# cristianpjensen/thesis-pai-reconstruction

Measured on AMD Instinct MI355X. Metric: train images/sec (256x256, bs=64) Pix2Pix step, higher is better.
Workload: dtype bf16; 1 GPU; Pix2Pix generator+PatchGAN GAN step, 256x256x1 pairs, 64 images/GPU (BASELINE configs[1]); global_batch=64, per_gpu_batch=64, loss_type=gan, parallelism=dp1, grad_bucket_dtype=f32

## Files before the change

### include/pai_hip.h

```cpp
#ifndef PAI_HIP_H
#define PAI_HIP_H

#include <stdint.h>

#ifdef __cplusplus
extern "C" {
#endif

#define PAI_F32 0
#define PAI_BF16 1
#define PAI_U8 2

#define PAI_ACT_NONE 0
#define PAI_ACT_LRELU 1
#define PAI_ACT_RELU 2
#define PAI_ACT_TANH 3
#define PAI_ACT_SILU 4

const char* pai_last_error(void);
int pai_version(void);
int pai_build_flags(void);
int pai_device_info(int* cu_count, int* lds_bytes, char* arch_name, int arch_name_len);

#define PAI_TUNABLE_UNSET (-2147483647 - 1)
int pai_set_tunable(const char* name, int value);

typedef struct pai_conv_desc {
    int32_t dtype;
    int32_t transposed;
    int32_t N, H, W;
    int32_t C1, C2;
    int32_t Cout;
    int32_t kernel;
    int32_t stride;
    int32_t pad;
    int32_t relu1, relu2;
    int32_t epilogue_act;
    int32_t groups;
    int32_t pack_flags;
    int32_t hints;
} pai_conv_desc;
#define PAI_HINT_SOLO 1

int pai_conv_out_hw(const pai_conv_desc* d, int* OH, int* OW);
int pai_conv_fwd_stats_rows(const pai_conv_desc* d);
int pai_conv_fwd_stats_rows_max(const pai_conv_desc* d);
int pai_bn_stats_buffer_rows(int rows);

int pai_conv_kernel_id(const pai_conv_desc* d, int op);
int pai_conv_kernel_name(const pai_conv_desc* d, int op, char* name, int name_len);

int pai_create(int device_id, void** handle_out);
int pai_bind(void* handle);
int pai_destroy(void* handle);
int pai_handle_set_workspace(void* handle, void* zeroed_device_memory, int64_t bytes);
int pai_handle_set_scratch(void* handle, void* device_memory, int64_t bytes);
int pai_handle_set_wgrad_workspace(void* handle, void* device_memory, int64_t bytes);

int pai_set_workspace(void* zeroed_device_memory, int64_t bytes);
int64_t pai_conv_workspace_bytes(const pai_conv_desc* d, int op);
int pai_set_scratch(void* device_memory, int64_t bytes);
int64_t pai_conv_scratch_bytes(const pai_conv_desc* d, int op);
int pai_set_wgrad_workspace(void* device_memory, int64_t bytes);
int64_t pai_conv_wgrad_workspace_bytes(const pai_conv_desc* d);

int pai_conv_fwd(const pai_conv_desc* d, const void* x1, const void* x2, const void* w_fwd,
                 const float* bias, void* y_raw, void* y_act, float* y_f32, float* stats,
                 void* stream);

int pai_conv_dgrad(const pai_conv_desc* d, const void* dy, const void* w_dgrad, void* dx1,
                   void* dx2, int only_c2, void* stream);

int pai_conv_dgrad_f32add_ok(const pai_conv_desc* d);
int pai_conv_dgrad_f32add(const pai_conv_desc* d, const void* dy, const void* w_dgrad, const float* addend,
                          float* dx2_f32, void* stream);

int pai_conv_dgrad_act(const pai_conv_desc* d, const void* dy, const void* w_dgrad, void* dx1,
                       void* dx2, const void* a1, int act1, void* stream);

typedef struct pai_bwd_epilogue {
    const void* z;
    const void* add;
    const float* scale;
    const float* shift;
    const float* mean;
    const float* rstd;
    float* partials;
    int32_t act1, act2;
} pai_bwd_epilogue;
int pai_conv_dgrad_bn_rows_max(const pai_conv_desc* d);
int pai_conv_dgrad_bn(const pai_conv_desc* d, const void* dy, const void* w_dgrad, void* dx1,
                      void* dx2, const pai_bwd_epilogue* e, int* partial_rows, void* stream);

typedef struct pai_bn_train {
    const float* gamma;
    const float* beta;
    float eps, momentum;
    int32_t n_updates;
    float* running_mean;
    float* running_var;
    int64_t* num_batches_tracked;
    float *mean, *rstd, *scale, *shift;
} pai_bn_train;
int pai_conv_fwd_bn(const pai_conv_desc* d, const void* x1, const void* x2, const void* w_fwd, const float* bias,
                    void* z, void* a, int act, const pai_bn_train* bn, float* stats, void* stream);
int pai_conv_dgrad_bn_apply(const pai_conv_desc* d, const void* dy, const void* w_dgrad, void* du_scratch, void* dx2,
                            const pai_bwd_epilogue* e, const float* gamma, float* sums, float* dgamma, float* dbeta,
                            void* dz, void* stream);
int pai_conv_bn_fused(const pai_conv_desc* d, int op);

int pai_conv_wgrad(const pai_conv_desc* d, const void* x1, const void* x2, const void* dy,
                   float* dw, float* dbias, void* stream);
int pai_conv_wgrad_overwrite(const pai_conv_desc* d, const void* x1, const void* x2, const void* dy,
                             float* dw, float* dbias, void* stream);
int pai_conv_wgrad_overwrite_w(const pai_conv_desc* d, const void* x1, const void* x2, const void* dy,
                               float* dw, float* dbias, void* stream);

int pai_conv_prologue_ok(const pai_conv_desc* d);
int pai_conv_fwd_pro(const pai_conv_desc* d, const void* x1, const void* w_fwd, const float* bias, void* y_raw,
                     float* stats, const float* pre_scale, const float* pre_shift, int pre_act, void* stream);
int pai_conv_wgrad_pro(const pai_conv_desc* d, const void* x1, const void* dy, float* dw, float* dbias, int overwrite,
                       const float* pre_scale, const float* pre_shift, int pre_act, void* stream);

int pai_pack_weights(int dtype, const float* w_master, int Cout, int taps, int Cin,
                     void* w_fwd_or_null, void* w_dgrad_or_null, void* stream);
int pai_pack_weights_multi(int n, const float* const* w_master, const int32_t* cout, const int32_t* taps,
                           const int32_t* cin, void* const* w_fwd, void* const* w_dgrad, void* stream);

int pai_bn_finalize(const float* stats, int rows, int C, int64_t count, const float* gamma,
                    const float* beta, float eps, float momentum, int n_updates,
                    float* running_mean, float* running_var, int64_t* num_batches_tracked,
                    float* mean, float* rstd, float* scale, float* shift, void* stream);
int pai_bn_eval_coeffs(int C, const float* gamma, const float* beta, const float* running_mean,
                       const float* running_var, float eps, float* scale, float* shift,
                       void* stream);
int pai_bn_apply(int dtype, const void* z, int64_t M, int C, const float* scale,
                 const float* shift, int act, void* out, void* stream);
int pai_bn2_add_act(int dtype, const void* za, const float* scale_a, const float* shift_a, const void* zb,
                    const float* scale_b, const float* shift_b, int64_t M, int C, int act_a, int act, void* out,
                    void* stream);
int pai_bn_bwd_partial_rows(int64_t M);
int pai_bn_bwd_reduce(int dtype, const void* g1, int act1, const void* g2, int act2, const void* a,
                      const void* z, int64_t M, int C, const float* mean, const float* rstd,
                      void* du, float* partials, float* sums, float* dgamma, float* dbeta,
                      void* stream);
int pai_bn_bwd_reduce_affine(int dtype, const void* g1, int act1, const void* g2, int act2, const void* z,
                             int64_t M, int C, const float* scale, const float* shift, const float* mean,
                             const float* rstd, void* du, float* partials, float* sums, float* dgamma,
                             float* dbeta, void* stream);
int pai_bn_bwd_finalize(const float* partials, int rows, int C, float* sums, float* dgamma,
                        float* dbeta, void* stream);
int pai_bn_bwd_apply(int dtype, const void* du, const void* z, int64_t M, int C,
                     const float* mean, const float* rstd, const float* gamma,
                     const float* sums, void* dz, void* stream);
int pai_bn_bwd_apply_affine(int dtype, const void* g1, int act1, const void* z, int64_t M, int C, const float* scale,
                            const float* shift, const float* mean, const float* rstd, const float* gamma,
                            const float* sums, void* dz, void* stream);
int pai_act_bwd(int dtype, const void* g1, int act1, const void* g2, int act2, const void* a,
                int64_t numel, void* du, void* stream);

int pai_dropout2d(int dtype, const void* x, const float* mask, int N, int64_t HW, int C, void* out,
                  void* stream);

int pai_maxpool2(int dtype, const void* x, int N, int H, int W, int C, void* out, unsigned char* idx, void* stream);
int pai_maxpool2_bwd(int dtype, const void* dout, const unsigned char* idx, int N, int H, int W, int C, void* dx,
                     void* stream);
int pai_upsample2(int dtype, const void* x, int N, int H, int W, int C, void* out, void* stream);
int pai_upsample2_bwd(int dtype, const void* dout, int N, int H, int W, int C, void* dx, void* stream);
int pai_add_act(int dtype, const void* a, const void* b, int64_t numel, int act, void* out, void* stream);
int pai_bn2_bwd_reduce(int dtype, const void* d, int act_a, const void* za, const void* zb, int64_t M, int C,
                       const float* scale_a, const float* shift_a, const float* mean_a, const float* rstd_a,
                       const float* mean_b, const float* rstd_b, float* part_a, float* part_b, float* sums_a, float* sums_b,
                       void* stream);
int pai_bn2_bwd_apply(int dtype, const void* d, int act_a, const void* za, const void* zb, int64_t M, int C,
                      const float* scale_a, const float* shift_a, const float* mean_a, const float* rstd_a,
                      const float* gamma_a, const float* sums_a, const float* mean_b, const float* rstd_b,
                      const float* gamma_b, const float* sums_b, void* dza, void* dzb, void* stream);
int pai_instnorm_fwd(int dtype, const void* x, int N, int HW, int C, float eps, int act, void* y, float* mean, float* rstd,
                     void* stream);
int pai_instnorm_bwd(int dtype, const void* g, const void* x, int N, int HW, int C, int act, const float* mean,
                     const float* rstd, void* dx, void* stream);

int pai_layernorm_partial_rows(int64_t M);
int pai_layernorm_fwd(int dtype, const void* x, const void* res, int64_t M, int D, const float* gamma,
                      const float* beta, float eps, const float* post, int P, void* sum_out, void* y,
                      float* mean, float* rstd, void* stream);
int pai_layernorm_bwd(int dtype, const void* dy, const void* xs, int64_t M, int D, const float* gamma,
                      const float* mean, const float* rstd, void* dx, float* dgamma_dbeta, float* partials,
                      void* stream);
int pai_gelu(int dtype, const void* z, int64_t numel, void* out, void* stream);
int pai_gelu_bwd(int dtype, const void* dy, const void* z, int64_t numel, void* dz, void* stream);
int pai_mha_fwd(int dtype, const void* qkv, int S, int B, int heads, int hd, const float* mask, void* out,
                float* probs, void* stream);
int pai_mha_bwd(int dtype, const void* dout, const void* qkv, const float* probs, int S, int B, int heads,
                int hd, const float* mask, void* dqkv, float* ds_workspace, void* stream);
int pai_mha_kernel_name(int dtype, int S, int hd, int op, char* name, int name_len);
int pai_subsample2(int dtype, const void* x, int N, int H, int W, int C, void* out, void* stream);
int pai_subsample2_bwd(int dtype, const void* dout, int N, int H, int W, int C, void* dx, void* stream);
int pai_bn_stats_rows(int64_t M);
int pai_bn_stats(int dtype, const void* z, int64_t M, int C, float* stats, void* stream);
int pai_colsum(int dtype, const void* x, int64_t rows, int C, float* out, void* stream);

int pai_gate_partial_rows(int64_t M);
int pai_gate_hidden(int dtype, const void* ig, const void* sg, int64_t M, int K, const float* scale_i,
                    const float* shift_i, const float* scale_s, const float* shift_s, const float* w_a,
                    const float* b_a, void* h, float* logit, float* partials, void* stream);
int pai_gate_apply(int dtype, const void* x, const float* logit, int64_t M, int C, const float* scale_a,
                   const float* shift_a, void* out, float* att, void* stream);
int pai_gate_apply_bwd(int dtype, const void* dout, const void* x, const float* att, const float* logit,
                       int64_t M, int C, const float* mean_a, const float* rstd_a, void* dx_skip, float* dl,
                       float* partials, int relu_out, void* stream);
int pai_gate_hidden_bwd(int dtype, const float* dl, const float* logit, const void* h, const void* ig,
                        const void* sg, int64_t M, int K, const float* mean_a, const float* rstd_a,
                        const float* gamma_a, const float* sums_a, const float* w_a, const float* mean_i,
                        const float* rstd_i, const float* mean_s, const float* rstd_s, void* dsum,
                        float* partials_i, float* partials_s, float* dw_a, float* db_a, void* stream);

int pai_bce_logits(const float* logits, int64_t numel, float target, float loss_scale,
                   double* loss, float grad_scale, float* grad, void* stream);
int pai_l1(const float* pred, const float* target, int64_t numel, float loss_scale, double* loss,
           float grad_scale, float* grad, void* stream);
int pai_mse(const float* pred, const float* target, int64_t numel, float loss_scale, double* loss,
            float grad_scale, float* grad, void* stream);
int pai_head_loss_ok(const pai_conv_desc* d, int has_bias);
int pai_head_loss(const pai_conv_desc* d, const void* a3, const void* w_fwd, const void* w_dgrad, int n_first,
                  float target_first, float target_rest, float loss_scale, double* loss, float grad_scale,
                  float* logits, void* dl, float* dl_f32, void* du, const void* act_src, int act, void* stream);
int pai_scalar_take(double* acc, float* out, void* stream);
int pai_metrics_take(double* sums, int64_t n_images, int64_t numel, float* out3, void* stream);
int pai_tanh_bwd(int dtype, const float* pred, const float* g_a, const float* g_b, int64_t numel,
                 void* dh, void* stream);
// ... 112 lines not shown
```

### thesis-pai-reconstruction_amd/attention.py

```python
from __future__ import annotations

import torch
import torch.nn as nn

from . import ops
from .engine import GradArena, UnetEngine, _BNState, _Packs, _bn_forward, to_fwd_pack_
from .ops import ACT_LRELU, ACT_NONE, ACT_RELU, ACT_TANH


class _Gate:

    def __init__(self, block: nn.Module, gen):
        self.conv_i, self.bn_i = block.input_gate[0], block.input_gate[1]
        self.conv_s, self.bn_s = block.signal_gate[0], block.signal_gate[1]
        self.conv_a, self.bn_a = block.attention[0], block.attention[1]
        self.C = self.conv_i.weight.shape[1]
        self.K = self.conv_i.weight.shape[0]
        self.pack_i = _Packs(self.conv_i, need_dgrad=True, gen=gen)
        self.pack_s = _Packs(self.conv_s, need_dgrad=True, gen=gen)

    def ordered_params(self):
        return [(self.conv_a.weight, None), (self.conv_a.bias, None), (self.bn_a.weight, None), (self.bn_a.bias, None),
                (self.bn_i.weight, None), (self.bn_i.bias, None), (self.bn_s.weight, None), (self.bn_s.bias, None),
                (self.conv_i.weight, None), (self.conv_i.bias, None), (self.conv_s.weight, None),
                (self.conv_s.bias, None)]


class AttentionUnetEngine(UnetEngine):
    overwrites_weight_grads = True

    def __init__(self, unet: nn.Module):
        super().__init__(unet)
        self.gates = [_Gate(b, self.weights_generation) for b in unet.attention_blocks]
        assert len(self.gates) == self.L - 1

    def all_packs(self):
        return self.enc_packs + self.dec_packs + [pk for g in self.gates for pk in (g.pack_i, g.pack_s)]

    def _gate(self, j):
        return self.gates[j - 1]

    def ordered_params(self):
        out = []
        L = self.L
        for j in range(L - 1, -1, -1):
            if self.dec_bn[j] is not None:
                out += [(self.dec_bn[j].weight, None), (self.dec_bn[j].bias, None)]
            out += [(self.dec_conv[j].weight, self.dec_conv[j]), (self.dec_conv[j].bias, None)]
            if j >= 1:
                out += self._gate(j).ordered_params()
        for i in range(L - 1, -1, -1):
            if self.enc_bn[i] is not None:
                out += [(self.enc_bn[i].weight, None), (self.enc_bn[i].bias, None)]
            out += [(self.enc_conv[i].weight, self.enc_conv[i]), (self.enc_conv[i].bias, None)]
        return out

    def _plan(self, N, H, W, dtype, device):
        key = (N, H, W, dtype, str(device))
        if key in self._plans:
            return self._plans[key]
        P = super()._plan(N, H, W, dtype, device)
        L = self.L
        eh, ew = P["eh"], P["ew"]
        P["dec_desc"] = []
        for j in range(L):
            hin, win = eh[L - 1 - j], ew[L - 1 - j]
            if j == 0:
                c1, c2, r1, r2 = self.enc_c[L - 1], 0, 1, 0
            else:
                c1, c2, r1, r2 = self.dec_c[j - 1], self.enc_c[L - 1 - j], 1, 1
            act = ACT_NONE
            if j == L - 1:
                r1, r2, act = 0, 0, ACT_TANH
            P["dec_desc"].append(ops.make_desc(dtype, 1, N, hin, win, c1, c2, self.dec_c[j], 2, r1, r2, act))
        P["gate_desc"] = [None]
        rows = P["stats"].numel()
        mx = P["bwd_partials"].numel()
        for j in range(1, L):
            g = self._gate(j)
            lvl = L - 1 - j
            d = ops.make_desc(dtype, 0, N, eh[lvl], ew[lvl], g.C, 0, g.K, 1, 0, 0, ACT_NONE, kernel=1)
            P["gate_desc"].append(d)
            M = N * eh[lvl] * ew[lvl]
            rows = max(rows, ops.bn_stats_buffer_rows(ops.conv_fwd_stats_rows_max(d)) * 2 * g.K,
                       ops.bn_stats_buffer_rows(ops.gate_partial_rows(M)) * 2)
            mx = max(mx, ops.gate_partial_rows(M) * 2 * g.K, ops.conv_dgrad_bn_rows_max(d) * 2 * g.C)
        P["stats"] = torch.empty(rows, dtype=torch.float32, device=device)
        P["bwd_partials"] = torch.empty(mx, dtype=torch.float32, device=device)
        P["bwd_partials2"] = torch.empty(mx, dtype=torch.float32, device=device)
        ops.ensure_workspace(max(ops.conv_workspace_bytes(d, op) for d in P["dec_desc"] + P["gate_desc"][1:]
                                 for op in (0, 1)), device)
        ops.ensure_scratch(ops.scratch_bytes_for(P["enc_desc"] + P["dec_desc"]), device)
        ops.ensure_wgrad_workspace(P["enc_desc"] + P["dec_desc"], device)
        return P

    def _new_slot(self, P):
        S = super()._new_slot(P)
        L, N, dt, dev = self.L, P["N"], P["dtype"], P["device"]
        eh, ew = P["eh"], P["ew"]
        S["b"] = [None] + [torch.empty_like(S["z"][i]) if i < L - 1 else None for i in range(1, L)]
        S["gate"] = [None]
        for j in range(1, L):
            g = self._gate(j)
            lvl = L - 1 - j
            M = N * eh[lvl] * ew[lvl]
            f32 = dict(dtype=torch.float32, device=dev)
            S["gate"].append({
                "M": M,
                "ig": torch.empty(M * g.K, dtype=dt, device=dev), "sg": torch.empty(M * g.K, dtype=dt, device=dev),
                "h": torch.empty(M * g.K, dtype=dt, device=dev), "s": torch.empty(M * g.C, dtype=dt, device=dev),
                "logit": torch.empty(M, **f32), "att": torch.empty(M, **f32),
                "bn_i": _BNState(g.K, dev), "bn_s": _BNState(g.K, dev), "bn_a": _BNState(1, dev),
            })
        return S

    def _grad_bufs(self, S):
        if S["grads"] is not None:
            return S["grads"]
        G = super()._grad_bufs(S)
        P = S["P"]
        L, dt, dev = self.L, P["dtype"], P["device"]
        G["gs"] = [None] + [torch.empty_like(S["gate"][j]["s"]) for j in range(1, L)]
        G["gx"] = [None] + [torch.empty_like(S["gate"][j]["s"]) for j in range(1, L)]
        G["dxs"] = [None] + [torch.empty_like(S["gate"][j]["s"]) for j in range(1, L)]
        G["dl"] = [None] + [torch.empty_like(S["gate"][j]["logit"]) for j in range(1, L)]
        G["dsum"] = [None] + [torch.empty_like(S["gate"][j]["h"]) for j in range(1, L)]
        G["dig"] = [None] + [torch.empty_like(S["gate"][j]["h"]) for j in range(1, L)]
        G["dsg"] = [None] + [torch.empty_like(S["gate"][j]["h"]) for j in range(1, L)]
        G["gr_raw"] = [torch.empty_like(t) if t is not None else None for t in G["gr"]]
        return G

    def _skip(self, S, lvl):
        return S["z"][0] if lvl == 0 else S["b"][lvl]

    def _gate_forward(self, S, j, x, signal, training, bn_updates, dtype):
        g, gs, P = self._gate(j), S["gate"][j], S["P"]
        d, M = P["gate_desc"][j], gs["M"]
        for conv, bn, pack, src, dst, st in ((g.conv_i, g.bn_i, g.pack_i, x, gs["ig"], gs["bn_i"]),
                                             (g.conv_s, g.bn_s, g.pack_s, signal, gs["sg"], gs["bn_s"])):
            wf, _ = pack.get(dtype)
            if training:
                rows = ops.conv_fwd_stats_rows(d)
                ops.conv_fwd(d, src, None, wf, conv.bias, y_raw=dst, stats=P["stats"])
                _bn_forward(bn, st, P["stats"], rows, M, True, bn_updates)
            else:
                ops.conv_fwd(d, src, None, wf, conv.bias, y_raw=dst)
                _bn_forward(bn, st, None, 0, M, False, 0)
        bi, bs, ba = gs["bn_i"], gs["bn_s"], gs["bn_a"]
        ops.gate_hidden(dtype, gs["ig"], gs["sg"], M, g.K, bi.scale, bi.shift, bs.scale, bs.shift, g.conv_a.weight,
                        g.conv_a.bias, gs["h"], gs["logit"], P["stats"])
        _bn_forward(g.bn_a, ba, P["stats"] if training else None, ops.gate_partial_rows(M) if training else 0, M,
                    training, bn_updates)
        ops.gate_apply(dtype, x, gs["logit"], M, g.C, ba.scale, ba.shift, gs["s"], gs["att"])
        return gs["s"]

    def forward(self, x: torch.Tensor, training: bool, bn_updates: int, dtype: torch.dtype):
        if not x.is_cuda:
            raise ops.PaiError("AttentionUnet (HIP) needs a HIP device tensor; there is no CPU path")
        N, Ci, H, W = x.shape
# ... 9 lines not shown
        xs = xs.contiguous() if Ci == 1 else xs.permute(0, 2, 3, 1).contiguous()
        if dtype == torch.float32:
            S["x"] = xs.reshape(-1)
        else:
            ops.cast(xs, S["x"])
        eh, ew = P["eh"], P["ew"]
        wf, _ = self.enc_packs[0].get(dtype)
        ops.conv_fwd(P["enc_desc"][0], S["x"], None, wf, self.enc_conv[0].bias, y_raw=S["z"][0], y_act=S["a"][0])
        for i in range(1, L):
            wf, _ = self.enc_packs[i].get(dtype)
            bn, d = self.enc_bn[i], P["enc_desc"][i]
            if bn is None:
                if i < L - 1:
                    raise ops.PaiError("only the last encoder may be norm-free")
                ops.conv_fwd(d, S["a"][i - 1], None, wf, self.enc_conv[i].bias, y_raw=S["z"][i])
                continue
            M = N * eh[i] * ew[i]
            if training:
                rows = ops.conv_fwd_stats_rows(d)
                ops.conv_fwd(d, S["a"][i - 1], None, wf, self.enc_conv[i].bias, y_raw=S["z"][i], stats=P["stats"])
                _bn_forward(bn, S["ebn"][i], P["stats"], rows, M, True, bn_updates)
            else:
                ops.conv_fwd(d, S["a"][i - 1], None, wf, self.enc_conv[i].bias, y_raw=S["z"][i])
                _bn_forward(bn, S["ebn"][i], None, 0, M, False, 0)
            st = S["ebn"][i]
            ops.bn_apply(dtype, S["z"][i], M, self.enc_c[i], st.scale, st.shift, ACT_LRELU, S["a"][i])
            ops.bn_apply(dtype, S["z"][i], M, self.enc_c[i], st.scale, st.shift, ACT_NONE, S["b"][i])
        for j in range(L):
            wf, _ = self.dec_packs[j].get(dtype)
            d = P["dec_desc"][j]
            if j == 0:
                x1, x2 = S["z"][L - 1], None
            else:
                x1 = S["r"][j - 1]
                x2 = self._gate_forward(S, j, self._skip(S, L - 1 - j), x1, training, bn_updates, dtype)
            if j < L - 1:
                bn = self.dec_bn[j]
                M = N * S["dh"][j] * S["dw"][j]
                if training:
                    rows = ops.conv_fwd_stats_rows(d)
                    ops.conv_fwd(d, x1, x2, wf, self.dec_conv[j].bias, y_raw=S["w"][j], stats=P["stats"])
                    _bn_forward(bn, S["dbn"][j], P["stats"], rows, M, True, bn_updates)
                else:
                    ops.conv_fwd(d, x1, x2, wf, self.dec_conv[j].bias, y_raw=S["w"][j])
                    _bn_forward(bn, S["dbn"][j], None, 0, M, False, 0)
                ops.bn_apply(dtype, S["w"][j], M, self.dec_c[j], S["dbn"][j].scale, S["dbn"][j].shift, ACT_NONE,
                             S["r"][j])
                if training and self.dec_drop[j] > 0:
                    self._dropout(S, j, M, self.dec_c[j], dtype)
            else:
                S["pred"] = torch.empty_like(S["pred"])
                ops.conv_fwd(d, x1, x2, wf, self.dec_conv[j].bias, y_f32=S["pred"])
        pred = S["pred"]
        if self.out_ch != 1:
            pred = pred.view(N, H, W, self.out_ch).permute(0, 3, 1, 2)
        return pred, S

    def backward(self, S, gpred: torch.Tensor, fresh: bool = False):
        P = S["P"]
        L, N, dtype = self.L, P["N"], P["dtype"]
        eh, ew = P["eh"], P["ew"]
        G = self._grad_bufs(S)
        A = self.arena()
        hook = self.grad_ready_hook
        if self.out_ch != 1:
            gpred = gpred.permute(0, 2, 3, 1)
        gpred = gpred.contiguous()
        if gpred.dtype != torch.float32:
            gpred = gpred.float()
        side = self._side
        part, part2 = P["bwd_partials"], P["bwd_partials2"]

        def done(p):
            if hook is not None:
                hook(A, A.end_of(p))

        def wgrad(d, x1, x2, dz, conv, with_bias, last=None):
            cin, cout = conv.weight.shape[1], conv.weight.shape[0]
            dense = fresh and conv.weight.shape[2] == 4 and min(cin, cout) > 2
            with torch.cuda.stream(side.fork(d)):
                (ops.conv_wgrad_overwrite_w if dense else ops.conv_wgrad)(
                    d, x1, x2, dz, A.seg(conv.weight), A.seg(conv.bias) if with_bias else None)
                done(last if last is not None else conv.bias)

        def gate_backward(j, relu_out):
            g, gs = self._gate(j), S["gate"][j]
            d, M = P["gate_desc"][j], gs["M"]
            lvl = L - 1 - j
            x, signal = self._skip(S, lvl), S["r"][j - 1]
            ba, bi, bs = gs["bn_a"], gs["bn_i"], gs["bn_s"]
            ops.gate_apply_bwd(dtype, G["gs"][j], x, gs["att"], gs["logit"], M, g.C, ba.mean, ba.rstd, G["dxs"][j],
                               G["dl"][j], part, relu_out)
            ops.bn_bwd_finalize(part, ops.gate_partial_rows(M), 1, ba.sums, A.seg(g.bn_a.weight), A.seg(g.bn_a.bias))
            ops.gate_hidden_bwd(dtype, G["dl"][j], gs["logit"], gs["h"], gs["ig"], gs["sg"], M, g.K, ba.mean, ba.rstd,
                                g.bn_a.weight, ba.sums, g.conv_a.weight, bi.mean, bi.rstd, bs.mean, bs.rstd,
                                G["dsum"][j], part, part2, A.seg(g.conv_a.weight), A.seg(g.conv_a.bias))
            rows = ops.gate_partial_rows(M)
            ops.bn_bwd_finalize(part, rows, g.K, bi.sums, A.seg(g.bn_i.weight), A.seg(g.bn_i.bias))
            ops.bn_bwd_finalize(part2, rows, g.K, bs.sums, A.seg(g.bn_s.weight), A.seg(g.bn_s.bias))
            ops.bn_bwd_apply(dtype, G["dsum"][j], gs["ig"], M, g.K, bi.mean, bi.rstd, g.bn_i.weight, bi.sums, G["dig"][j])
            ops.bn_bwd_apply(dtype, G["dsum"][j], gs["sg"], M, g.K, bs.mean, bs.rstd, g.bn_s.weight, bs.sums, G["dsg"][j])
            wgrad(d, x, None, G["dig"][j], g.conv_i, False)
            wgrad(d, signal, None, G["dsg"][j], g.conv_s, False)
            _, wd_i = g.pack_i.get(dtype)
            _, wd_s = g.pack_s.get(dtype)
            ops.conv_dgrad_bn(d, G["dig"][j], wd_i, G["gx"][j], None, x, ACT_NONE, G["dxs"][j], ACT_NONE)
            pst = S["dbn"][j - 1]
            if (j - 1) in S["drop"]:
                ops.conv_dgrad_bn(d, G["dsg"][j], wd_s, G["gr"][j - 1], None, S["r"][j - 1], ACT_NONE,
                                  G["gr_raw"][j - 1], ACT_RELU if relu_out else ACT_NONE)
                ops.dropout2d(dtype, G["gr"][j - 1], S["drop"][j - 1], N, S["dh"][j - 1] * S["dw"][j - 1],
                              self.dec_c[j - 1], G["gr"][j - 1])
                return None
            return ops.conv_dgrad_bn(d, G["dsg"][j], wd_s, G["gr"][j - 1], None, S["w"][j - 1], ACT_NONE,
                                     G["gr_raw"][j - 1], ACT_RELU if relu_out else ACT_NONE, pst.scale, pst.shift,
                                     pst.mean, pst.rstd, part)

        j = L - 1
        dh = G["dz_head"]
        ops.tanh_bwd(dtype, S["pred"], gpred, None, dh)
        d = P["dec_desc"][j]
        wgrad(d, S["r"][j - 1], S["gate"][j]["s"], dh, self.dec_conv[j], True)
        side.mark_scratch()
        _, wd = self.dec_packs[j].get(dtype)
        ops.conv_dgrad(d, dh, wd, G["gr_raw"][j - 1], G["gs"][j])
        fused_rows = gate_backward(j, relu_out=False)
        for j in range(L - 2, -1, -1):
            bn, st, conv = self.dec_bn[j], S["dbn"][j], self.dec_conv[j]
            M = N * S["dh"][j] * S["dw"][j]
            C = self.dec_c[j]
            dz = G["dz_dec"][j]
            du = G["gr"][j]
            if fused_rows is None:
                du = G["du"][:M * C]
                ops.bn_bwd_reduce(dtype, G["gr"][j], ACT_NONE, None, ACT_NONE, None, S["w"][j], M, C, st.mean, st.rstd,
                                  du, part, st.sums, A.seg(bn.weight), A.seg(bn.bias))
            else:
                ops.bn_bwd_finalize(part, fused_rows, C, st.sums, A.seg(bn.weight), A.seg(bn.bias))
            ops.bn_bwd_apply(dtype, du, S["w"][j], M, C, st.mean, st.rstd, bn.weight, st.sums, dz)
            d = P["dec_desc"][j]
            _, wd = self.dec_packs[j].get(dtype)
            if j == 0:
                wgrad(d, S["z"][L - 1], None, dz, conv, False)
                fused_rows = ops.conv_dgrad_bn(d, dz, wd, G["dz_enc"][L - 1], None, S["z"][L - 1], ACT_RELU)
            else:
                wgrad(d, S["r"][j - 1], S["gate"][j]["s"], dz, conv, False)
                ops.conv_dgrad(d, dz, wd, G["gr_raw"][j - 1], G["gs"][j])
                fused_rows = gate_backward(j, relu_out=True)
        i = L - 1
        dz = G["dz_enc"][i]
        wgrad(P["enc_desc"][i], S["a"][i - 1], None, dz, self.enc_conv[i], True)
        _, wd = self.enc_packs[i].get(dtype)

        def enc_dgrad(i, dz, wd):
            d = P["enc_desc"][i]
            gx = G["gx"][L - 1 - (i - 1)]
            if i - 1 == 0:
                return ops.conv_dgrad_bn(d, dz, wd, G["dz_enc"][0], None, S["z"][0], ACT_LRELU, gx, ACT_NONE)
            pst = S["ebn"][i - 1]
            return ops.conv_dgrad_bn(d, dz, wd, G["ga"][i - 1], None, S["z"][i - 1], ACT_LRELU, gx, ACT_NONE,
                                     pst.scale, pst.shift, pst.mean, pst.rstd, part)

        fused_rows = enc_dgrad(i, dz, wd)
        for i in range(L - 2, 0, -1):
            bn, st, conv = self.enc_bn[i], S["ebn"][i], self.enc_conv[i]
            M = N * eh[i] * ew[i]
            C = self.enc_c[i]
            du, dz = G["ga"][i], G["dz_enc"][i]
            ops.bn_bwd_finalize(part, fused_rows, C, st.sums, A.seg(bn.weight), A.seg(bn.bias))
            ops.bn_bwd_apply(dtype, du, S["z"][i], M, C, st.mean, st.rstd, bn.weight, st.sums, dz)
            wgrad(P["enc_desc"][i], S["a"][i - 1], None, dz, conv, False)
            _, wd = self.enc_packs[i].get(dtype)
            fused_rows = enc_dgrad(i, dz, wd)
        conv0 = self.enc_conv[0]
        with torch.cuda.stream(side.fork_tail()):
            c0_in, c0_out = conv0.weight.shape[1], conv0.weight.shape[0]
            (ops.conv_wgrad_overwrite_w if (fresh and min(c0_in, c0_out) > 2) else ops.conv_wgrad)(
                P["enc_desc"][0], S["x"], None, G["dz_enc"][0], A.seg(conv0.weight), A.seg(conv0.bias))
        side.join()
        done(conv0.bias)
```

### thesis-pai-reconstruction_amd/csrc/api.hip

```cpp
#include <stdarg.h>

#include "common.h"

static thread_local char g_err[512] = "";

void pai_set_error(const char* fmt, ...) {
    va_list ap;
    va_start(ap, fmt);
    vsnprintf(g_err, sizeof(g_err), fmt, ap);
    va_end(ap);
}

extern "C" const char* pai_last_error(void) { return g_err; }
extern "C" int pai_version(void) { return 141; }

extern "C" int pai_build_flags(void) { return 0; }

extern "C" int pai_device_info(int* cu_count, int* lds_bytes, char* arch_name, int arch_name_len) {
    int dev = 0;
    hipError_t e = hipGetDevice(&dev);
    PAI_CHECK(e == hipSuccess, "hipGetDevice: %s", hipGetErrorString(e));
    hipDeviceProp_t p;
    e = hipGetDeviceProperties(&p, dev);
    PAI_CHECK(e == hipSuccess, "hipGetDeviceProperties: %s", hipGetErrorString(e));
// ... 470 lines not shown

extern "C" int64_t pai_conv_workspace_bytes(const pai_conv_desc* d, int op) {
    GG g;
    if (op == 1 ? gg_build_dgrad(d, &g) : gg_build_fwd(d, &g)) return -1;
    return op == 2 ? 0 : pick_fwd(d->dtype, g, query_args(g, op)).workspace_bytes;
}

extern "C" int64_t pai_conv_scratch_bytes(const pai_conv_desc* d, int op) {
    GG g;
    if (op == 1 ? gg_build_dgrad(d, &g) : gg_build_fwd(d, &g)) return -1;
    return op == 2 ? pick_wgrad(d->dtype, g, false, false).scratch_bytes : pick_fwd(d->dtype, g, query_args(g, op)).scratch_bytes;
}

extern "C" int pai_conv_fwd_stats_rows(const pai_conv_desc* d) {
    GG g;
    if (gg_build_fwd(d, &g)) return -1;
    FwdArgs a = query_args(g, 0);
    a.stats = (float*)1;
    return pick_fwd(d->dtype, g, a).rows;
}

extern "C" int pai_conv_kernel_id(const pai_conv_desc* d, int op) {
    GG g;
    if (op == 1 ? gg_build_dgrad(d, &g) : gg_build_fwd(d, &g)) return -1;
    return op == 2 ? pick_wgrad(d->dtype, g, false, false).id : pick_fwd(d->dtype, g, query_args(g, op)).id;
}

extern "C" int pai_conv_kernel_name(const pai_conv_desc* d, int op, char* name, int name_len) {
    GG g;
    if ((op == 1 ? gg_build_dgrad(d, &g) : gg_build_fwd(d, &g)) || !name || name_len <= 0) return -1;
    const char* n = op == 2 ? pick_wgrad(d->dtype, g, false, false).name : pick_fwd(d->dtype, g, query_args(g, op)).name;
    strncpy(name, n, name_len - 1);
    name[name_len - 1] = 0;
    return 0;
}

extern "C" int pai_conv_fwd_stats_rows_max(const pai_conv_desc* d) {
    GG g;
    if (gg_build_fwd(d, &g)) return -1;
    return cdiv(g.M, 16) * g.nphase;
}

extern "C" int pai_conv_fwd(const pai_conv_desc* d, const void* x1, const void* x2,
                            const void* w_fwd, const float* bias, void* y_raw, void* y_act,
                            float* y_f32, float* stats, void* stream) {
    GG g;
    if (gg_build_fwd(d, &g)) return 1;
    PAI_CHECK(x1 && w_fwd, "pai_conv_fwd: null x1 / w");
    PAI_CHECK(d->C2 == 0 || x2, "pai_conv_fwd: C2 > 0 but x2 is null");
    PAI_CHECK(y_raw || y_act || y_f32, "pai_conv_fwd: no output requested");
    FwdArgs a;
    memset(&a, 0, sizeof(a));
    a.x1 = x1; a.x2 = x2; a.w = w_fwd; a.bias = bias;
    a.y1 = y_raw; a.y2 = nullptr; a.yact = y_act; a.yf32 = y_f32; a.stats = stats;
    a.eact = d->epilogue_act;
    return run_fwd(d->dtype, g, a, (hipStream_t)stream);
}

static int conv_wgrad_impl(const pai_conv_desc* d, const void* x1, const void* x2, const void* dy, float* dw,
                           float* dbias, int overwrite, void* stream, const float* pscale = nullptr,
                           const float* pshift = nullptr, int pact = 0);

extern "C" int pai_conv_prologue_ok(const pai_conv_desc* d) {
    GG g;
    if (gg_build_fwd(d, &g)) return 0;
    FwdArgs a = query_args(g, 0);
    a.pscale = a.pshift = (const float*)1;
    a.pact = PAI_ACT_RELU;
    return pick_fwd(d->dtype, g, a).k != FK_NONE && pick_wgrad(d->dtype, g, false, true).k != WK_NONE;
}

extern "C" int pai_conv_fwd_pro(const pai_conv_desc* d, const void* x1, const void* w_fwd, const float* bias, void* y_raw,
                                float* stats, const float* pre_scale, const float* pre_shift, int pre_act, void* stream) {
    GG g;
    if (gg_build_fwd(d, &g)) return 1;
    PAI_CHECK(x1 && w_fwd && y_raw && pre_scale && pre_shift, "pai_conv_fwd_pro: null pointer");
    PAI_CHECK(pre_act == PAI_ACT_NONE || pre_act == PAI_ACT_RELU, "pai_conv_fwd_pro: pre_act=%d (none or ReLU)", pre_act);
    PAI_CHECK(d->C2 == 0, "pai_conv_fwd_pro: one source tensor only");
    FwdArgs a;
    memset(&a, 0, sizeof(a));
    a.x1 = x1; a.w = w_fwd; a.bias = bias;
    a.y1 = y_raw;
    a.stats = stats;
    a.pscale = pre_scale; a.pshift = pre_shift; a.pact = pre_act;
    return run_fwd(d->dtype, g, a, (hipStream_t)stream);
}

extern "C" int pai_conv_wgrad_pro(const pai_conv_desc* d, const void* x1, const void* dy, float* dw, float* dbias,
                                  int overwrite, const float* pre_scale, const float* pre_shift, int pre_act, void* stream) {
    PAI_CHECK(pre_scale && pre_shift, "pai_conv_wgrad_pro: null prologue");
    PAI_CHECK(pre_act == PAI_ACT_NONE || pre_act == PAI_ACT_RELU, "pai_conv_wgrad_pro: pre_act=%d (none or ReLU)", pre_act);
    PAI_CHECK(d->C2 == 0, "pai_conv_wgrad_pro: one source tensor only");
    return conv_wgrad_impl(d, x1, nullptr, dy, dw, dbias, overwrite ? 1 : 0, stream, pre_scale, pre_shift, pre_act);
}

extern "C" int pai_conv_dgrad(const pai_conv_desc* d, const void* dy, const void* w_dgrad,
                              void* dx1, void* dx2, int only_c2, void* stream) {
    GG g;
    if (gg_build_dgrad(d, &g)) return 1;
    PAI_CHECK(dy && w_dgrad, "pai_conv_dgrad: null dy / w");
    PAI_CHECK(only_c2 ? (dx2 && d->C2 > 0) : (dx1 != nullptr), "pai_conv_dgrad: missing output");
    PAI_CHECK(d->C2 == 0 || dx2, "pai_conv_dgrad: C2 > 0 but dx2 is null");
    FwdArgs a;
    memset(&a, 0, sizeof(a));
    a.x1 = dy; a.w = w_dgrad;
    a.y1 = dx1; a.y2 = dx2;
    a.skip_d1 = only_c2;
    return run_fwd(d->dtype, g, a, (hipStream_t)stream);
}

extern "C" int pai_conv_dgrad_f32add_ok(const pai_conv_desc* d) {
    GG g;
    if (!d || gg_build_dgrad(d, &g)) return 0;
    return pai_tunable("head_fused", 1) && thin_up_f32add_ok(d->dtype, g) ? 1 : 0;
}

extern "C" int pai_conv_dgrad_f32add(const pai_conv_desc* d, const void* dy, const void* w_dgrad, const float* addend,
                                     float* dx2_f32, void* stream) {
    GG g;
    if (gg_build_dgrad(d, &g)) return 1;
    PAI_CHECK(dy && w_dgrad && addend && dx2_f32, "pai_conv_dgrad_f32add: null pointer");
    PAI_CHECK(thin_up_f32add_ok(d->dtype, g), "pai_conv_dgrad_f32add: not a bf16 (1 | 1)-channel k4 s2 layer on thin_up_k (ask pai_conv_dgrad_f32add_ok)");
    FwdArgs a;
    memset(&a, 0, sizeof(a));
    a.x1 = dy; a.w = w_dgrad;
    a.yf32 = dx2_f32; a.badd = addend;
    a.skip_d1 = 1;
    return launch_thin_dgrad(g, a, (hipStream_t)stream);
}

extern "C" int pai_conv_dgrad_act(const pai_conv_desc* d, const void* dy, const void* w_dgrad,
                                  void* dx1, void* dx2, const void* a1, int act1, void* stream) {
    GG g;
    if (gg_build_dgrad(d, &g)) return 1;
    PAI_CHECK(dy && w_dgrad && dx1 && a1, "pai_conv_dgrad_act: null pointer");
    PAI_CHECK(d->C2 == 0 || dx2, "pai_conv_dgrad_act: C2 > 0 but dx2 is null");
    PAI_CHECK(act1 == PAI_ACT_LRELU || act1 == PAI_ACT_RELU || act1 == PAI_ACT_NONE, "pai_conv_dgrad_act: act1=%d", act1);
    FwdArgs a;
    memset(&a, 0, sizeof(a));
    a.x1 = dy; a.w = w_dgrad;
    a.y1 = dx1; a.y2 = dx2;
    hipStream_t s = (hipStream_t)stream;
    FwdPick p = pick_fwd(d->dtype, g, a);
    const bool fused = p.fused || p.k == FK_HEAD_DGRAD;
    if (fused) {
        a.bz = a1; a.bact1 = act1;
        p = pick_fwd(d->dtype, g, a);
    }
    int rc = run_fwd(p, d->dtype, g, a, s);
    if (rc || fused || act1 == PAI_ACT_NONE) return rc;
    return pai_act_bwd(d->dtype, dx1, act1, nullptr, PAI_ACT_NONE, a1, (int64_t)g.N * g.OH * g.OW * g.D1, dx1, stream);
}

extern "C" int pai_conv_dgrad_bn_rows_max(const pai_conv_desc* d) {
    GG g;
    if (gg_build_dgrad(d, &g)) return -1;
    int fused = cdiv(g.M, 16) * g.nphase;
    if (pw_rows(g) > fused) fused = pw_rows(g);
    if (pwx_rows(g) > fused) fused = pwx_rows(g);
    const int twopass = pai_bn_bwd_partial_rows((int64_t)g.N * g.OH * g.OW);
    return fused > twopass ? fused : twopass;
}

int bn_bwd_reduce_affine(int dtype, void* g1_du, int act1, const void* g2, int act2, const void* z, int64_t M, int C,
                         const float* scale, const float* shift, const float* mean, const float* rstd,
                         float* partials, hipStream_t s);

extern "C" int pai_conv_dgrad_bn(const pai_conv_desc* d, const void* dy, const void* w_dgrad, void* dx1,
                                 void* dx2, const pai_bwd_epilogue* e, int* partial_rows, void* stream) {
    GG g;
    if (gg_build_dgrad(d, &g)) return 1;
    PAI_CHECK(dy && w_dgrad && dx1 && e && e->z, "pai_conv_dgrad_bn: null pointer");
    PAI_CHECK(d->C2 == 0 || dx2, "pai_conv_dgrad_bn: C2 > 0 but dx2 is null");
    PAI_CHECK((e->scale == nullptr) == (e->shift == nullptr), "pai_conv_dgrad_bn: scale and shift go together");
    PAI_CHECK(!e->partials || (e->mean && e->rstd && partial_rows), "pai_conv_dgrad_bn: partials need mean, rstd and partial_rows");
    for (int act : {e->act1, e->act2})
        PAI_CHECK(act == PAI_ACT_LRELU || act == PAI_ACT_RELU || act == PAI_ACT_NONE, "pai_conv_dgrad_bn: act=%d", act);
    FwdArgs a;
    memset(&a, 0, sizeof(a));
    a.x1 = dy; a.w = w_dgrad;
    a.y1 = dx1; a.y2 = dx2;
    hipStream_t s = (hipStream_t)stream;
    const int64_t M = (int64_t)g.N * g.OH * g.OW;
    const FwdPick plain = pick_fwd(d->dtype, g, a);
    if (plain.fused) {
        a.bz = e->z; a.badd = e->add;
        a.bscale = e->scale; a.bshift = e->shift; a.bmean = e->mean; a.brstd = e->rstd;
        a.bact1 = e->act1; a.bact2 = e->act2;
        a.bpart = e->partials;
        const FwdPick p = pick_fwd(d->dtype, g, a);
        PAI_CHECK(p.fused, "pai_conv_dgrad_bn: no kernel with the fused store takes this epilogue");
        if (partial_rows) *partial_rows = e->partials ? p.rows : 0;
        return run_fwd(p, d->dtype, g, a, s);
    }
    if (e->partials) {
        if (const int rows = thin_fwd_bwd_rows(d->dtype, g, a, e->act1, e->add, e->scale)) {
            a.bz = e->z; a.bmean = e->mean; a.brstd = e->rstd; a.bpart = e->partials; a.bact1 = e->act1;
            *partial_rows = rows;
            return run_fwd(d->dtype, g, a, s);
        }
    }
    int rc = run_fwd(plain, d->dtype, g, a, s);
    if (rc) return rc;
    if (e->partials) {
        *partial_rows = pai_bn_bwd_partial_rows(M);
        return bn_bwd_reduce_affine(d->dtype, dx1, e->act1, e->add, e->act2, e->z, M, g.D1, e->scale, e->shift,
                                    e->mean, e->rstd, e->partials, s);
    }
    if (partial_rows) *partial_rows = 0;
    PAI_CHECK(e->scale == nullptr, "pai_conv_dgrad_bn: affine pre-activation without partial sums is only built for the matrix-core kernels");
    return pai_act_bwd(d->dtype, dx1, e->act1, e->add, e->act2, e->z, M * g.D1, dx1, stream);
}

extern "C" int pai_conv_fwd_bn(const pai_conv_desc* d, const void* x1, const void* x2, const void* w_fwd, const float* bias,
                               void* z, void* a_out, int act, const pai_bn_train* bn, float* stats, void* stream) {
    GG g;
    if (gg_build_fwd(d, &g)) return 1;
    PAI_CHECK(x1 && w_fwd && z && a_out && bn && stats, "pai_conv_fwd_bn: null pointer");
    PAI_CHECK(d->C2 == 0 || x2, "pai_conv_fwd_bn: C2 > 0 but x2 is null");
    PAI_CHECK(bn->mean && bn->rstd && bn->scale && bn->shift, "pai_conv_fwd_bn: mean / rstd / scale / shift outputs are required");
    PAI_CHECK(act == PAI_ACT_NONE || act == PAI_ACT_RELU || act == PAI_ACT_LRELU, "pai_conv_fwd_bn: act=%d", act);
    FwdArgs a;
    memset(&a, 0, sizeof(a));
    a.x1 = x1; a.x2 = x2; a.w = w_fwd; a.bias = bias;
    a.y1 = z; a.stats = stats;
    a.eact = PAI_ACT_NONE;
    hipStream_t s = (hipStream_t)stream;
    const int64_t count = (int64_t)g.N * g.OH * g.OW;
    const FwdPick p = pick_fwd(d->dtype, g, a);
    if (int rc = run_fwd(p, d->dtype, g, a, s)) return rc;
    const int rows = p.rows;
    if (bn_fuse_small_ok(rows, count, g.Cout))
        return launch_bn_fin_apply(d->dtype, stats, rows, g.Cout, count, bn->gamma, bn->beta, bn->eps, bn->momentum,
                                   bn->n_updates, bn->running_mean, bn->running_var, bn->num_batches_tracked, bn->mean,
                                   bn->rstd, bn->scale, bn->shift, z, act, a_out, s);
    if (int rc = pai_bn_finalize(stats, rows, g.Cout, count, bn->gamma, bn->beta, bn->eps, bn->momentum, bn->n_updates,
                                 bn->running_mean, bn->running_var, bn->num_batches_tracked, bn->mean, bn->rstd, bn->scale,
                                 bn->shift, stream)) return rc;
    return pai_bn_apply(d->dtype, z, count, g.Cout, bn->scale, bn->shift, act, a_out, stream);
}

extern "C" int pai_conv_bn_fused(const pai_conv_desc* d, int op) {
    GG g;
    if (op == 1 ? gg_build_dgrad(d, &g) : gg_build_fwd(d, &g)) return -1;
    return 0;
}

extern "C" int pai_conv_dgrad_bn_apply(const pai_conv_desc* d, const void* dy, const void* w_dgrad, void* du_scratch,
                                       void* dx2, const pai_bwd_epilogue* e, const float* gamma, float* sums,
                                       float* dgamma, float* dbeta, void* dz, void* stream) {
    GG g;
    if (gg_build_dgrad(d, &g)) return 1;
    PAI_CHECK(dy && w_dgrad && du_scratch && e && e->z && e->mean && e->rstd && e->partials && sums && dz,
              "pai_conv_dgrad_bn_apply: null pointer");
    PAI_CHECK(d->C2 == 0 || dx2, "pai_conv_dgrad_bn_apply: C2 > 0 but dx2 is null");
    PAI_CHECK((e->scale == nullptr) == (e->shift == nullptr), "pai_conv_dgrad_bn_apply: scale and shift go together");
    FwdArgs a;
    memset(&a, 0, sizeof(a));
    a.x1 = dy; a.w = w_dgrad;
    a.y1 = du_scratch; a.y2 = dx2;
    hipStream_t s = (hipStream_t)stream;
    int rows = 0;
    if (int rc = pai_conv_dgrad_bn(d, dy, w_dgrad, du_scratch, dx2, e, &rows, stream)) return rc;
    const int64_t Mo = (int64_t)g.N * g.OH * g.OW;
    if (bn_fuse_small_ok(rows, Mo, g.D1))
        return launch_bn_bwd_fin_apply(d->dtype, e->partials, rows, g.D1, sums, dgamma, dbeta, du_scratch, e->z, Mo, e->mean,
                                       e->rstd, gamma, dz, s);
    if (int rc = pai_bn_bwd_finalize(e->partials, rows, g.D1, sums, dgamma, dbeta, stream)) return rc;
    return pai_bn_bwd_apply(d->dtype, du_scratch, e->z, Mo, g.D1, e->mean, e->rstd, gamma, sums, dz, stream);
}


extern "C" int pai_conv_wgrad(const pai_conv_desc* d, const void* x1, const void* x2,
                              const void* dy, float* dw, float* dbias, void* stream) {
    return conv_wgrad_impl(d, x1, x2, dy, dw, dbias, 0, stream);
}

extern "C" int pai_conv_wgrad_overwrite(const pai_conv_desc* d, const void* x1, const void* x2,
                                        const void* dy, float* dw, float* dbias, void* stream) {
    return conv_wgrad_impl(d, x1, x2, dy, dw, dbias, 1, stream);
}

extern "C" int pai_conv_wgrad_overwrite_w(const pai_conv_desc* d, const void* x1, const void* x2,
                                          const void* dy, float* dw, float* dbias, void* stream) {
    return conv_wgrad_impl(d, x1, x2, dy, dw, dbias, 2, stream);
}

static int conv_wgrad_impl(const pai_conv_desc* d, const void* x1, const void* x2, const void* dy, float* dw,
                           float* dbias, int overwrite, void* stream, const float* pscale, const float* pshift, int pact) {
    GG g;
    if (gg_build_fwd(d, &g)) return 1;
    PAI_CHECK(x1 && dy && dw, "pai_conv_wgrad: null pointer");
    PAI_CHECK(d->C2 == 0 || x2, "pai_conv_wgrad: C2 > 0 but x2 is null");
    WgradArgs a;
    a.x1 = x1; a.x2 = x2; a.dy = dy; a.dw = dw; a.dbias = dbias; a.overwrite = 0; a.overwrite_bias = 0; a.slab = nullptr;
    a.pscale = pscale; a.pshift = pshift; a.pact = pact;
    hipStream_t s = (hipStream_t)stream;
    const WgradPick p = pick_wgrad(d->dtype, g, dbias != nullptr, pscale != nullptr);
    PAI_CHECK(p.k != WK_NONE, "pai_conv_wgrad_pro: this layer takes no prologue (ask pai_conv_prologue_ok: the grouped 3 x 3 weight "
                              "gradient needs its workspace, pai_set_wgrad_workspace)");
    if (overwrite && p.overwrites) {
        a.overwrite = 1;
        a.overwrite_bias = p.k != WK_GROUPED3 && overwrite == 1;
    } else if (overwrite) {
        hipError_t e = pai::memset_async(dw, 0, (size_t)g.Cout * g.wtaps * g.Cin * sizeof(float), s);
        PAI_CHECK(e == hipSuccess, "pai_conv_wgrad_overwrite: hipMemsetAsync: %s", hipGetErrorString(e));
// ... 18 lines not shown
```

### thesis-pai-reconstruction_amd/csrc/common.h

```cpp
#pragma once
#include <hip/hip_runtime.h>
#include <stdint.h>
#include <stdio.h>
#include <string.h>

#include "../../include/pai_hip.h"
#include "plan.h"

typedef unsigned short bf16_t;

void pai_set_error(const char* fmt, ...);

#define PAI_CHECK(cond, ...)                 \
    do {                                     \
        if (!(cond)) {                       \
            pai_set_error(__VA_ARGS__);      \
            return 1;                        \
        }                                    \
    } while (0)

#define PAI_LAUNCH_CHECK()                                              \
    do {                                                                \
        hipError_t e_ = hipGetLastError();                              \
        if (e_ != hipSuccess) {                                         \
// ... 41 lines not shown
    static __device__ __forceinline__ void ld(const float* p, float* o) {
        float4 a = *(const float4*)p, b = *(const float4*)(p + 4);
        o[0] = a.x; o[1] = a.y; o[2] = a.z; o[3] = a.w; o[4] = b.x; o[5] = b.y; o[6] = b.z; o[7] = b.w;
    }
    static __device__ __forceinline__ void st(float* p, const float* v) {
        *(float4*)p = make_float4(v[0], v[1], v[2], v[3]);
        *(float4*)(p + 4) = make_float4(v[4], v[5], v[6], v[7]);
    }
};
template <> struct V8<bf16_t> {
    static __device__ __forceinline__ void ld(const bf16_t* p, float* o) {
        uint4 v = *(const uint4*)p;
        unsigned u[4] = {v.x, v.y, v.z, v.w};
#pragma unroll
        for (int i = 0; i < 4; ++i) {
            o[2 * i] = __uint_as_float(u[i] << 16);
            o[2 * i + 1] = __uint_as_float(u[i] & 0xffff0000u);
        }
    }
    static __device__ __forceinline__ void st(bf16_t* p, const float* v) {
        unsigned u[4];
#pragma unroll
        for (int i = 0; i < 4; ++i) u[i] = pk2bf(v[2 * i], v[2 * i + 1]);
        *(uint4*)p = make_uint4(u[0], u[1], u[2], u[3]);
    }
};

__device__ __forceinline__ float act_apply(float v, int act) {
    switch (act) {
        case PAI_ACT_LRELU: return v > 0.f ? v : 0.2f * v;
        case PAI_ACT_RELU: return !(v <= 0.f) ? v : 0.f;
        case PAI_ACT_TANH: return tanhf(v);
        default: return v;
    }
}
__device__ __forceinline__ float act_grad(float a, int act) {
    switch (act) {
        case PAI_ACT_LRELU: return a > 0.f ? 1.f : 0.2f;
        case PAI_ACT_RELU: return a > 0.f ? 1.f : 0.f;
        default: return 1.f;
    }
}

__device__ __forceinline__ float wave_sum(float v) {
#pragma unroll
    for (int o = 32; o > 0; o >>= 1) v += __shfl_xor(v, o, 64);
    return v;
}

static inline int cdiv(int64_t a, int64_t b) { return (int)((a + b - 1) / b); }

struct PerDeviceOnce {
    bool done[32] = {};
    bool first() {
        int dev = 0;
        if (hipGetDevice(&dev) != hipSuccess || dev < 0 || dev >= 32) return true;
        if (done[dev]) return false;
        done[dev] = true;
        return true;
    }
};

struct GG {
    int N, H, W;
    int C1, C2, Cin;
    int OHg, OWg;
    int Cout;
    int S;
    int nphase, ntaps;
    int OH, OW, OS;
    int D1, D2;
    int wtaps;
    int relu1, relu2;
    int M;
    int lw, lh;
    int lsw, lsh, ldw, ldh;
    signed char dy[4][16], dx[4][16], wt[4][16];
    signed char poy[4], pox[4];
    int gslice;
    int solo;
};

struct PatchGeo {
    int groups;
    int TY, TX;
    signed char by[4][4], bx[4][4];
    unsigned toff4[4][4];
    unsigned wt4[4][4];
    unsigned wt_lo[4], wt_hi[4], toff2[4];
};

int gg_build_fwd(const pai_conv_desc* d, GG* g);
int gg_build_dgrad(const pai_conv_desc* d, GG* g);

struct FwdArgs {
    const void *x1, *x2, *w;
    const float* bias;
    void *y1, *y2;
    void* yact;
    float* yf32;
    float* stats;
    int eact;
    int skip_d1;
    const void* bz;
    const void* badd;
    const float *bscale, *bshift, *bmean, *brstd;
    int bact1, bact2;
    float* bpart;
    const float *pscale, *pshift;
    int pact;
};
bool bn_fuse_small_ok(int rows, int64_t M, int C);
int launch_bn_fin_apply(int dtype, const float* stats, int rows, int C, int64_t count, const float* gamma, const float* beta,
                        float eps, float momentum, int n_updates, float* running_mean, float* running_var, int64_t* nbt,
                        float* mean, float* rstd, float* scale, float* shift, const void* z, int act, void* out,
                        hipStream_t s);
int launch_bn_bwd_fin_apply(int dtype, const float* partials, int rows, int C, float* sums, float* dgamma, float* dbeta,
                            const void* du, const void* z, int64_t M, const float* mean, const float* rstd,
                            const float* gamma, void* dz, hipStream_t s);
int ew_stream_bn_apply(int dtype, const void* z, int64_t M, int C, const float* scale, const float* shift, int act, void* out,
                       hipStream_t s);
int ew_stream_bn2_add_act(int dtype, const void* za, const float* sca, const float* sha, const void* zb, const float* scb,
                          const float* shb, int64_t M, int C, int act_a, int act, void* out, hipStream_t s);
int ew_stream_add_act(int dtype, const void* a, const void* b, int64_t numel, int act, void* out, hipStream_t s);
int ew_stream_bn_bwd_reduce(int dtype, const void* g, int act, const void* z, int64_t M, int C, const float* scale,
                            const float* shift, const float* mean, const float* rstd, float* partials, int rows, hipStream_t s);
int ew_stream_bn_bwd_apply(int dtype, const void* g, int act, const void* z, int64_t M, int C, const float* scale,
                           const float* shift, const float* mean, const float* rstd, const float* gamma, const float* sums,
                           void* dz, hipStream_t s);
int ew_stream_bn2_bwd_reduce(int dtype, const void* d, int act_a, const void* za, const void* zb, int64_t M, int C,
                             const float* scale_a, const float* shift_a, const float* mean_a, const float* rstd_a,
                             const float* mean_b, const float* rstd_b, float* part_a, float* part_b, int rows, hipStream_t s);
int ew_stream_bn2_bwd_apply(int dtype, const void* d, int act_a, const void* za, const void* zb, int64_t M, int C,
                            const float* scale_a, const float* shift_a, const float* mean_a, const float* rstd_a,
                            const float* gamma_a, const float* sums_a, const float* mean_b, const float* rstd_b,
                            const float* gamma_b, const float* sums_b, void* dza, void* dzb, hipStream_t s);
int launch_fwd_simt(int dtype, const GG& g, const FwdArgs& a, hipStream_t s);
int launch_fwd_rowdot(int dtype, const GG& g, const FwdArgs& a, hipStream_t s);
int pai_tunable(const char* name, int def);
struct MfmaPlan {
    int variant;
    const char* name;
    int bm, bn, db;
    int ksplit, mtiles, ntiles;
    int rows;
    unsigned grid, block;
    size_t lds;
    int64_t workspace_bytes;
    bool overwrites;
    PatchGeo pg;
};
enum WgradMfmaVariant { WG3_128x64 = 1, WG3_64x128, WG3_128x64_8, WGRAD_PATCH128, WGRAD_PATCH64, WGRAD_TILE128, WGRAD_TILE64 };
MfmaPlan fwd_mfma_plan(const GG& g);
int launch_fwd_mfma(const GG& g, const FwdArgs& a, const MfmaPlan& p, hipStream_t s);
MfmaPlan wgrad_mfma_plan(const GG& g, bool has_dbias, bool has_prologue);
bool wgrad_pro_ok(int dtype, const GG& g);
struct pai_handle_s {
    int device;
    float* workspace;
    int64_t workspace_bytes;
    float* scratch;
    int64_t scratch_bytes;
    float* wslab;
    int64_t wslab_bytes;
};
const pai_handle_s* pai_ctx();
int fwd_simt_mtiles(const GG& g);
bool fwd_mfma_ok(int dtype, const GG& g, const FwdArgs& a);
bool pw_ok(int dtype, const GG& g, const FwdArgs& a);
int pw_rows(const GG& g);
int launch_pw(const GG& g, const FwdArgs& a, hipStream_t s);
bool pwx_ok(int dtype, const GG& g, const FwdArgs& a);
int pwx_rows(const GG& g);
int launch_pwx(const GG& g, const FwdArgs& a, hipStream_t s);
const char* pwx_kernel_name(const GG& g);
bool fwd_rowdot_ok(const GG& g, const FwdArgs& a);
bool small_ok(int dtype, const GG& g, const FwdArgs& a);
int small_rows(const GG& g);
int launch_small(const GG& g, const FwdArgs& a, hipStream_t s);
bool grouped3_ok(int dtype, const GG& g, const FwdArgs& a);
int grouped3_rows(const GG& g);
int launch_grouped3(const GG& g, const FwdArgs& a, hipStream_t s);

bool thin_fwd_ok(int dtype, const GG& g, const FwdArgs& a);
bool thin_dgrad_ok(int dtype, const GG& g, const FwdArgs& a);
bool thin_dgrad_shape_ok(int dtype, const GG& g);
int64_t thin_dgrad_scratch_bytes(const GG& g, const FwdArgs& a);
int launch_thin_fwd(const GG& g, const FwdArgs& a, hipStream_t s);
bool head_dgrad_ok(int dtype, const GG& g, const FwdArgs& a);
int launch_head_dgrad(const GG& g, const FwdArgs& a, hipStream_t s);
int thin_fwd_bwd_rows(int dtype, const GG& g, const FwdArgs& a, int act1, const void* add, const float* scale);
int launch_thin_dgrad(const GG& g, const FwdArgs& a, hipStream_t s);
bool thin_up_f32add_ok(int dtype, const GG& g);

struct WgradArgs {
    const void *x1, *x2, *dy;
    float* dw;
    float* dbias;
    int overwrite;
    int overwrite_bias;
    float* slab;
    const float *pscale, *pshift;
    int pact;
};
float* wgrad_slab_acquire(int64_t bytes);
int launch_wgrad_slab_sum(float* dw, const float* slab, int nsplits, int64_t n, int overwrite, hipStream_t s);
bool grouped3_wgrad_ok(int dtype, const GG& g, const float* dbias);
int64_t grouped3_wgrad_part_bytes(const GG& g);
int launch_grouped3_wgrad(const GG& g, const WgradArgs& a, float* part, hipStream_t s);
int launch_eval_planes(const float* pred, const float* target, int NC, int H, int W, int denorm, double* ssim_plane,
                       double* sse_plane, unsigned char* map_u8, const unsigned char* lut_rgb, unsigned char* hot_u8,
                       hipStream_t stream);
const char* eval_planes_kernel_name();
bool wgrad3_ok(const GG& g);
MfmaPlan wgrad3_plan(const GG& g, bool has_dbias);
int launch_wgrad3(const GG& g, const WgradArgs& a, const MfmaPlan& p, hipStream_t s);
int launch_wgrad_simt(int dtype, const GG& g, const WgradArgs& a, hipStream_t s);
int launch_wgrad_rowdot(int dtype, const GG& g, const WgradArgs& a, hipStream_t s);
int launch_wgrad_mfma(const GG& g, const WgradArgs& a, const MfmaPlan& p, hipStream_t s);
bool wgrad_mfma_ok(int dtype, const GG& g);
bool thin_wgrad_conv_ok(int dtype, const GG& g);
bool thin_wgrad_convt_ok(int dtype, const GG& g);
int launch_thin_wgrad_conv(const GG& g, const WgradArgs& a, hipStream_t s);
int launch_thin_wgrad_convt(const GG& g, const WgradArgs& a, hipStream_t s);
bool thin_wgrad_conv1_ok(int dtype, const GG& g);
int launch_thin_wgrad_conv1(const GG& g, const WgradArgs& a, hipStream_t s);
bool thin_wgrad_conv3_ok(int dtype, const GG& g);
int launch_thin_wgrad_conv3(const GG& g, const WgradArgs& a, hipStream_t s);
bool thin_wgrad_conv3t_ok(int dtype, const GG& g);
int launch_thin_wgrad_conv3t(const GG& g, const WgradArgs& a, hipStream_t s);
int64_t thin_wgrad_scratch_bytes(int64_t M, int T, int WC);
```

### thesis-pai-reconstruction_amd/csrc/gg_mfma.hip

```cpp
#include <type_traits>

#include "gg_tile.h"


bool fwd_mfma_ok(int dtype, const GG& g, const FwdArgs& a) {
    if (dtype != PAI_BF16) return false;
    if (g.C1 % 64 || g.C2 % 64) return false;
    if (g.Cout % 64) return false;
    if (g.D2 > 0 && (g.D1 % 64)) return false;
    if (a.yf32) return false;
    if (a.skip_d1) return false;
    if ((a.y1 || a.y2) && a.yact) return false;
    if (a.yact && a.eact != PAI_ACT_NONE && a.eact != PAI_ACT_LRELU && a.eact != PAI_ACT_RELU) return false;
    return true;
}

struct FwdCfg { int bn, ksplit; };

static FwdCfg fwd_cfg(const GG& g) {
    FwdCfg c;
    c.bn = ((g.Cout % 128) == 0 && (g.D2 == 0 || (g.D1 % 128) == 0)) ? 128 : 64;
    c.ksplit = 1;
    const int ntiles = g.Cout / c.bn;
    const int niter = g.ntaps * g.Cin / MBK;
// ... 287 lines not shown
    float bs1[8], bs2[8];
#pragma unroll
    for (int k = 0; k < 8; ++k) bs1[k] = bs2[k] = 0.f;
    constexpr int NP = BM / ORP, NB = NP < 4 ? NP : 4;
    if (bwd) bwd_load_params(a, dcol + oc * 8, BP);
#pragma unroll
    for (int p0 = 0; p0 < NP; p0 += NB) {
        size_t offs[NB];
        uint4 zq[NB], aq[NB];
#pragma unroll
        for (int p = 0; p < NB; ++p) {
            const int m = m0 + orow0 + (p0 + p) * ORP;
            int n, gy, gx;
            decode_row(g, m < g.M ? m : 0, n, gy, gx);
            const size_t pix = (size_t)(n * g.OH + gy * g.OS + g.poy[ph]) * g.OW + gx * g.OS + g.pox[ph];
            offs[p] = pix * dstride + dcol + oc * 8;
            if (bwd) {
                zq[p] = *(const uint4*)(bzp + offs[p]);
                aq[p] = bap ? *(const uint4*)(bap + offs[p]) : make_uint4(0, 0, 0, 0);
            }
        }
#pragma unroll
        for (int p = 0; p < NB; ++p) {
            const int row = orow0 + (p0 + p) * ORP;
            if (m0 + row < g.M) {
                uint4 o = *(const uint4*)(Cs + row * CROW + oc * 16);
                if (bwd)
                    o = bwd_chunk(o, zq[p], aq[p], bap != nullptr, a.bscale != nullptr, bsum, a.bact1, a.bact2, BP, bs1, bs2);
                *(uint4*)(dst + offs[p]) = o;
            }
        }
    }
    if (bsum)
        bwd_write_partials<BN, CPR, NTHR / 64>(sstat, bs1, bs2, tid,
                                               a.bpart + ((size_t)(ph * mtiles + bm) * 2) * g.D1 + n0, g.D1,
                                               a.bmean + n0, a.brstd + n0);
}

constexpr int FIN_COLS = 128;
__global__ __launch_bounds__(256) void splitk_finish_k(GG g, FwdArgs a, const float* ws, int mtiles, int ksplit) {
    __shared__ float red[2][FIN_ROWS][FIN_COLS + 8];
    const int tid = threadIdx.x;
    const int bm = blockIdx.x, ph = blockIdx.y, cb = blockIdx.z;
    const int row = tid >> 4, cgl = tid & 15;
    const int m = bm * FIN_ROWS + row;
    const int c0 = cb * FIN_COLS + cgl * 8;
    const bool valid = m < g.M && c0 < g.Cout;
    const float eslope = act_slope(a.yact ? a.eact : PAI_ACT_NONE);
    float v[8], bs1[8], bs2[8];
#pragma unroll
    for (int k = 0; k < 8; ++k) v[k] = bs1[k] = bs2[k] = 0.f;
    if (valid) {
        const size_t slab = (size_t)g.nphase * g.M * g.Cout;
        const float* src = ws + ((size_t)ph * g.M + m) * g.Cout + c0;
#pragma unroll 4
        for (int s = 0; s < ksplit; ++s) {
            const float4 v0 = *(const float4*)(src + s * slab), v1 = *(const float4*)(src + s * slab + 4);
            v[0] += v0.x; v[1] += v0.y; v[2] += v0.z; v[3] += v0.w;
            v[4] += v1.x; v[5] += v1.y; v[6] += v1.z; v[7] += v1.w;
        }
        if (a.bias) {
#pragma unroll
            for (int k = 0; k < 8; ++k) v[k] += a.bias[c0 + k];
        }
    }
    if (a.stats) {
#pragma unroll
        for (int k = 0; k < 8; ++k) {
            red[0][row][cgl * 8 + k] = v[k];
            red[1][row][cgl * 8 + k] = v[k] * v[k];
        }
    }
    if (valid) {
        unsigned packed[4];
#pragma unroll
        for (int k = 0; k < 8; ++k) v[k] = act_fwd(v[k], eslope);
#pragma unroll
        for (int k = 0; k < 4; ++k) packed[k] = pk2bf(v[2 * k], v[2 * k + 1]);
        int n, gy, gx;
        decode_row(g, m, n, gy, gx);
        const size_t pix = (size_t)(n * g.OH + gy * g.OS + g.poy[ph]) * g.OW + gx * g.OS + g.pox[ph];
        bf16_t* dst;
        if (a.yact) dst = (bf16_t*)a.yact + pix * g.Cout + c0;
        else if (c0 < g.D1) dst = (bf16_t*)a.y1 + pix * g.D1 + c0;
        else dst = (bf16_t*)a.y2 + pix * g.D2 + (c0 - g.D1);
        uint4 o = make_uint4(packed[0], packed[1], packed[2], packed[3]);
        if (a.bz && !a.yact && c0 < g.D1) {
            BwdParams BP;
            bwd_load_params(a, c0, BP);
            const size_t off = pix * g.D1 + c0;
            const bf16_t* bap = (const bf16_t*)a.badd;
            o = bwd_chunk(o, *(const uint4*)((const bf16_t*)a.bz + off),
                          bap ? *(const uint4*)(bap + off) : make_uint4(0, 0, 0, 0), bap != nullptr,
                          a.bscale != nullptr, a.bpart != nullptr, a.bact1, a.bact2, BP, bs1, bs2);
        }
        *(uint4*)dst = o;
    }
    if (a.stats) {
        __syncthreads();
        const int c = cb * FIN_COLS + tid;
        if (tid < FIN_COLS && c < g.Cout) {
            float t1 = 0.f, t2 = 0.f;
#pragma unroll
            for (int r = 0; r < FIN_ROWS; ++r) { t1 += red[0][r][tid]; t2 += red[1][r][tid]; }
            float* dst = a.stats + ((size_t)(ph * mtiles + bm) * 2) * g.Cout + c;
            dst[0] = t1;
            dst[g.Cout] = t2;
        }
    } else if (a.bpart && a.bz) {
#pragma unroll
        for (int k = 0; k < 8; ++k) {
            red[0][row][cgl * 8 + k] = bs1[k];
            red[1][row][cgl * 8 + k] = bs2[k];
        }
        __syncthreads();
        const int c = cb * FIN_COLS + tid;
        if (tid < FIN_COLS && c < g.D1) {
            float t1 = 0.f, t2 = 0.f;
#pragma unroll
            for (int r = 0; r < FIN_ROWS; ++r) { t1 += red[0][r][tid]; t2 += red[1][r][tid]; }
            float* dst = a.bpart + ((size_t)(ph * mtiles + bm) * 2) * g.D1 + c;
            dst[0] = t1;
            dst[g.D1] = a.brstd[c] * (t2 - a.bmean[c] * t1);
        }
    }
}



static int patch_rows(const GG& g, const FwdCfg& c, PatchGeo* pg) {
    const bool no_256 = !pai_tunable("fwd_patch256", 1);
    if (!pai_tunable("fwd_patch", 1) || c.ksplit > 1) return 0;
    if ((int64_t)g.N * g.H * g.W * (g.C1 > g.C2 ? g.C1 : g.C2) * 2 >= (1ll << 31) || (int64_t)g.Cout * g.wtaps * g.Cin * 2 >= (1ll << 31))
        return 0;
    if (!no_256 && c.bn == 128 && (int64_t)(g.M / 256) * (g.Cout / 128) * g.nphase >= 512 && patch_geo(g, 16, pg)) return 256;
    if (!no_256 && c.bn == 64 && g.Cin >= 256 && pai_tunable("fwd_w1", 1) &&
        (int64_t)(g.M / 256) * (g.Cout / 64) * g.nphase >= pai_tunable("fwd_w1_min", 768) && patch_geo(g, 16, pg))
        return 256;
    return patch_geo(g, 8, pg) ? 128 : 0;
}

#ifndef PATCH_ABL
#define PATCH_ABL 0
#endif
#ifndef EPI_ABL
#define EPI_ABL 0
#endif
#ifndef PATCH_COLSWZ_ALL
#define PATCH_COLSWZ_ALL 0
#endif
#ifndef PATCH_SETPRIO
#define PATCH_SETPRIO 1
#endif
template <int BM, int BN, bool DBB, int WN = 2, int WPX = 64, bool COLSWZ = true>
__device__ __forceinline__ void gg_fwd_patch_body(const GG& g, const FwdArgs& a, const PatchGeo& pg, int mtiles, int ntiles) {
    static_assert(WN == 2 || BN == 64, "one wave column: 64 output channels");
    constexpr int abl = PATCH_ABL;
    typedef PatchDims<BM, WN, WPX> PD;
    constexpr int NTHR = PD::NTHR, MT = WPX / 16, NT = BN / (16 * WN);
    constexpr int BNW = BN / WN;
    constexpr int RPP = PD::RPP, PJ = PD::PJ, PATCH_PIX = PD::PIX, PATCH_BYTES = PD::BYTES;
    constexpr int BJ = BN / RPP;
    extern __shared__ __attribute__((aligned(16))) unsigned char smem[];
    unsigned char* Bs = smem + PATCH_BYTES;

    const int tid = threadIdx.x, lane = tid & 63;
    const int wid = __builtin_amdgcn_readfirstlane(tid >> 6);
    const int wm = WN == 2 ? wid >> 1 : wid, wn = WN == 2 ? wid & 1 : 0;
    int bid = xcd_remap(blockIdx.x, gridDim.x);
    const int bn = bid % ntiles;
    bid /= ntiles;
    const int ph = bid % g.nphase;
    const int bm = bid / g.nphase;
    const int n0 = bn * BN;
    const int tpi = pg.TY * pg.TX;
    const int img = bm / tpi, trem = bm - img * tpi;
    const int gy0 = (trem / pg.TX) * PD::TH, gx0 = (trem % pg.TX) * 16;

    constexpr unsigned OOB = 0x80000000u;
    const __amdgpu_buffer_rsrc_t wrs = __builtin_amdgcn_make_buffer_rsrc(
        const_cast<void*>(a.w), 0, (unsigned)(g.Cout * g.wtaps * g.Cin) * 2u, 0x00020000);
    const unsigned xpix = (unsigned)(g.N * g.H * g.W);
    const __amdgpu_buffer_rsrc_t x1rs = __builtin_amdgcn_make_buffer_rsrc(
        const_cast<void*>(a.x1), 0, xpix * (unsigned)g.C1 * 2u, 0x00020000);
    const __amdgpu_buffer_rsrc_t x2rs = __builtin_amdgcn_make_buffer_rsrc(
        const_cast<void*>(a.x2 ? a.x2 : a.x1), 0, a.x2 ? xpix * (unsigned)g.C2 * 2u : 0u, 0x00020000);
    unsigned wby16 = 0, wbx16 = 0;
#pragma unroll
    for (int q = 0; q < 4; ++q) {
        wby16 |= (unsigned)((pg.by[ph][q] + 8) & 15) << (4 * q);
        wbx16 |= (unsigned)((pg.bx[ph][q] + 8) & 15) << (4 * q);
    }
    wby16 = __builtin_amdgcn_readfirstlane(wby16);
    wbx16 = __builtin_amdgcn_readfirstlane(wbx16);
    const unsigned wtlo = __builtin_amdgcn_readfirstlane(pg.wt_lo[ph]);
    const unsigned wthi = __builtin_amdgcn_readfirstlane(pg.wt_hi[ph]);
    const unsigned toff2 = __builtin_amdgcn_readfirstlane(pg.toff2[ph]);
    const unsigned relu_bits = __builtin_amdgcn_readfirstlane((g.relu1 ? 1u : 0u) | (g.relu2 ? 2u : 0u));

    const int sc = lane & 7, sr = wid * 8 + (lane >> 3);
    unsigned pfill[PJ];
#pragma unroll
    for (int j = 0; j < PJ; ++j) {
        const int p = j * RPP + sr;
        const int py = p / PATCH_W, px = p - py * PATCH_W;
        const int y = (gy0 + py) * g.S, x = (gx0 + px) * g.S;
        const int pixb = (img * g.H + y) * g.W + x;
        unsigned m = 0;
        auto inside = [&](int q) {
            const int yy = y + (int)((wby16 >> (4 * q)) & 15u) - 8, xx = x + (int)((wbx16 >> (4 * q)) & 15u) - 8;
            if (p < PATCH_PIX && (unsigned)yy < (unsigned)g.H && (unsigned)xx < (unsigned)g.W) m |= 1u << q;
        };
        inside(0);
        if (pg.groups > 1) {
#pragma unroll
            for (int q = 1; q < 4; ++q) inside(q);
        }
        pfill[j] = ((unsigned)pixb & 0xffffffu) | (m << 24) | ((unsigned)(sc ^ ((COLSWZ ? px : sr) & 6)) << 28);
    }
    const int gchB = (sc ^ ((sr >> 1) & 7)) * 8;
    unsigned wrow[BJ];
#pragma unroll
    for (int j = 0; j < BJ; ++j) {
        const int lr = sr + RPP * j, half = lr / BNW, rho = lr % BNW;
        const int ch = half * BNW + (4 * NT) * ((rho & 15) >> 2) + 4 * (rho >> 4) + (rho & 3);
        wrow[j] = (unsigned)((n0 + ch) * g.wtaps * g.Cin + gchB) * 2u;
    }

    const int fr = lane & 15, fq = lane >> 4;
    unsigned a_addr[2][2];
#pragma unroll
    for (int tx = 0; tx < 2; ++tx)
#pragma unroll
        for (int kk = 0; kk < 2; ++kk) {
            const unsigned px = (unsigned)(fr + tx);
            a_addr[tx][kk] = ((unsigned)(wm * MT * PATCH_W) + px) * 128u + ((((unsigned)(kk * 4 + fq)) ^ (px & 6u)) << 4);
        }
    const int fswz = fr >> 1;
    unsigned b_addr[2];
#pragma unroll
    for (int kk = 0; kk < 2; ++kk)
        b_addr[kk] = (unsigned)(PATCH_BYTES + (wn * BNW + fr) * 128) + (unsigned)(((kk * 4 + fq) ^ fswz) << 4);
    int pbase[MT];
#pragma unroll
    for (int mt = 0; mt < MT; ++mt) pbase[mt] = (wm * MT + mt) * PATCH_W + fr;
    const unsigned b_base = (unsigned)(PATCH_BYTES + (wn * BNW + fr) * 128);
    f4_t acc[MT][NT];
#pragma unroll
    for (int i = 0; i < MT; ++i)
#pragma unroll
        for (int j = 0; j < NT; ++j) acc[i][j] = (f4_t){0.f, 0.f, 0.f, 0.f};

    const int cchunks = g.Cin / MBK;
    const int ngroups = cchunks * pg.groups;
    const int gsh = pg.groups == 4 ? 2 : 0;
#define FP_BLDS16(rs, voff, soff, lptr) \
    __builtin_amdgcn_raw_ptr_buffer_load_lds(rs, (__attribute__((address_space(3))) void*)(lptr), 16, (int)(voff), (int)(soff), 0, 0)
    auto fire_patch = [&](int gi) {
        const int c0 = (gi >> gsh) * MBK, q = gi & (pg.groups - 1);
        const bool second = c0 >= g.C1;
        const int C = second ? g.C2 : g.C1;
        const int cofs = second ? c0 - g.C1 : c0;
        const int dpix = ((int)((wby16 >> (4 * q)) & 15u) - 8) * g.W + (int)((wbx16 >> (4 * q)) & 15u) - 8;
        if (abl & 2) return;
#pragma unroll
        for (int j = 0; j < PJ; ++j) {
            unsigned pf = pfill[j];
            asm volatile("" : "+v"(pf));
            const unsigned vo = ((pf >> (24 + q)) & 1u)
                                    ? (unsigned)(((int)(pf & 0xffffffu) + dpix) * C + cofs + (int)((pf >> 28) & 7u) * 8) * 2u : OOB;
            if (second) FP_BLDS16(x2rs, vo, 0, smem + (j * RPP + wid * 8) * 128);
            else FP_BLDS16(x1rs, vo, 0, smem + (j * RPP + wid * 8) * 128);
        }
    };
    auto fire_b = [&](int gi, int k, int buf) {
        const int c0 = (gi >> gsh) * MBK, q = gi & (pg.groups - 1);
        const unsigned slot = (((q & 2) ? wthi : wtlo) >> (16 * (q & 1) + 4 * k)) & 15u;
        const unsigned woff = (unsigned)((int)slot * g.Cin + c0) * 2u;
        if (abl & 1) return;
#pragma unroll
        for (int j = 0; j < BJ; ++j) FP_BLDS16(wrs, wrow[j], woff, Bs + buf * (BN * 128) + (j * RPP + wid * 8) * 128);
    };
    fire_patch(0);
    fire_b(0, 0, 0);
    if constexpr (COLSWZ) {
        auto step = [&](auto k_tag, int gi, int relu, bool more) {
            constexpr int K = decltype(k_tag)::value;
            constexpr int TY = K >> 1, TX = K & 1;
            constexpr int BUF = DBB ? (K & 1) : 0;
            asm volatile("s_waitcnt vmcnt(0)" ::: "memory");
            __builtin_amdgcn_s_barrier();
            if (DBB) {
                if (K < 3) fire_b(gi, K + 1, BUF ^ 1);
                else if (more) fire_b(gi + 1, 0, BUF ^ 1);
            }
    #pragma unroll
            for (int kk = 0; kk < 2; ++kk) {
                bf8_t af[MT], bfr[NT];
                if (!(abl & 8)) {
                    const unsigned aa = a_addr[TX][kk], ba = b_addr[kk];
#pragma unroll
                    for (int mt = 0; mt < MT; ++mt)
                        af[mt] = *(const bf8_t*)(smem + (aa & 0xffffu) + (mt + TY) * (PATCH_W * 128));
    #pragma unroll
                    for (int nt = 0; nt < NT; ++nt)
                        bfr[nt] = *(const bf8_t*)(smem + (ba & 0x3ffffu) + BUF * (BN * 128) + nt * 16 * 128);
                } else {
    #pragma unroll
                    for (int mt = 0; mt < MT; ++mt) af[mt] = __builtin_bit_cast(bf8_t, make_uint4(a_addr[TX][kk], b_addr[kk], mt, kk));
// ... 68 lines not shown
                    bf8_t af[MT], bfr[NT];
                    if (!(abl & 8)) {
    #pragma unroll
                        for (int mt = 0; mt < MT; ++mt) af[mt] = *(const bf8_t*)(smem + (abase[mt] ^ ca));
    #pragma unroll
                        for (int nt = 0; nt < NT; ++nt) bfr[nt] = *(const bf8_t*)(smem + bb + nt * 16 * 128 + cb);
                    } else {
    #pragma unroll
                        for (int mt = 0; mt < MT; ++mt) af[mt] = __builtin_bit_cast(bf8_t, make_uint4(ca, cb, mt, kk));
    #pragma unroll
                        for (int nt = 0; nt < NT; ++nt) bfr[nt] = __builtin_bit_cast(bf8_t, make_uint4(cb, ca, nt, kk));
                    }
                    if (relu) {
    #pragma unroll
                        for (int mt = 0; mt < MT; ++mt) af[mt] = relu_frag(af[mt]);
                    }
                    if (PATCH_SETPRIO) __builtin_amdgcn_s_setprio(1);
                    if (!(abl & 4)) {
    #pragma unroll
                        for (int mt = 0; mt < MT; ++mt)
    #pragma unroll
                            for (int nt = 0; nt < NT; ++nt)
                                acc[mt][nt] = __builtin_amdgcn_mfma_f32_16x16x32_bf16(bfr[nt], af[mt], acc[mt][nt], 0, 0, 0);
                    } else {
                        acc[0][0][0] += (float)af[0][0] + (float)bfr[0][0];
                    }
                    if (PATCH_SETPRIO) __builtin_amdgcn_s_setprio(0);
                }
                if (DBB) {
                    buf ^= 1;
                    if (k == 3 && more) {
                        asm volatile("s_waitcnt lgkmcnt(0)" ::: "memory");
                        __builtin_amdgcn_s_barrier();
                        fire_patch(gi + 1);
                    }
                } else {
                    asm volatile("s_waitcnt lgkmcnt(0)" ::: "memory");
                    __builtin_amdgcn_s_barrier();
                    if (k < 3) fire_b(gi, k + 1, 0);
                    else if (more) { fire_patch(gi + 1); fire_b(gi + 1, 0, 0); }
                }
            }
        }
    }
    asm volatile("s_waitcnt lgkmcnt(0)" ::: "memory");
    __builtin_amdgcn_s_barrier();
    if (abl & 16) {
        float t = 0.f;
#pragma unroll
        for (int i = 0; i < MT; ++i)
#pragma unroll
            for (int j = 0; j < NT; ++j) {
                t += acc[i][j][0] + acc[i][j][1] + acc[i][j][2] + acc[i][j][3];
            }
        if (t == 123.456f) *(float*)a.y1 = t;
        return;
    }

    constexpr int CROW = BN * 2 + 16;
    constexpr int WM = BM / WPX;
    unsigned char* Cs = smem;
    float* sstat = (float*)(smem + BM * CROW);
    const int eact = a.yact ? a.eact : PAI_ACT_NONE;
    const float eslope = act_slope(eact);
    constexpr int CL = 4 * NT;
    const int col0 = wn * BNW + CL * fq;
    bf16_t* dst;
    int dstride, dcol;
    if (a.yact) { dst = (bf16_t*)a.yact; dstride = g.Cout; dcol = n0; }
    else if (n0 < g.D1) { dst = (bf16_t*)a.y1; dstride = g.D1; dcol = n0; }
    else { dst = (bf16_t*)a.y2; dstride = g.D2; dcol = n0 - g.D1; }
    const bool bwd = a.bz && !a.yact && n0 < g.D1;
    const bf16_t* bzp = (const bf16_t*)a.bz;
    const bf16_t* bap = (const bf16_t*)a.badd;
    const bool bsum = bwd && a.bpart;
    constexpr int CPR = BN / 8;
    constexpr int ORP = NTHR / CPR;
    static_assert(ORP % 16 == 0, "a pass covers whole 16-pixel tile rows");
    const int oc = tid % CPR, orow0 = tid / CPR;
    constexpr int NP = BM / ORP, NB = NP < 4 ? NP : 4, NBATCH = NP / NB;
    const size_t tile0 = ((size_t)(img * g.OH + gy0 * g.OS + g.poy[ph]) * g.OW + gx0 * g.OS + g.pox[ph]) * dstride + dcol;
    const unsigned toff = (unsigned)((((orow0 >> 4) * g.OS * g.OW + (orow0 & 15) * g.OS) * dstride + oc * 8) * 2);
    const unsigned pstep = (unsigned)((ORP / 16) * g.OS * g.OW * dstride * 2);
    const char* zt = (const char*)(bzp + tile0);
    const char* at = (const char*)(bap + tile0);
    char* dt = (char*)(dst + tile0);
    const float sl1 = act_slope(a.bact1), sl2 = act_slope(a.bact2);
    uint4 zq[NB], aq[NB];
    if (bwd && !(EPI_ABL & 1)) {
#pragma unroll
        for (int p = 0; p < NB; ++p) zq[p] = *(const uint4*)(zt + (toff + (unsigned)p * pstep));
    }
    const bool has_bias = a.bias != nullptr, has_stats = a.stats != nullptr;
    auto stage = [&](auto full_tag) {
        constexpr bool FULL = decltype(full_tag)::value;
        float bias_v[FULL ? CL : 1], csum[FULL ? CL : 1], csq[FULL ? CL : 1];
        if (FULL) {
#pragma unroll
            for (int c = 0; c < CL; ++c) { bias_v[c] = has_bias ? a.bias[n0 + col0 + c] : 0.f; csum[c] = csq[c] = 0.f; }
        }
#pragma unroll
        for (int mt = 0; mt < MT; ++mt) {
            const int row = wm * WPX + mt * 16 + fr;
#pragma unroll
            for (int h = 0; h < CL / 8; ++h) {
                float v[8];
#pragma unroll
                for (int c = 0; c < 8; ++c) {
                    v[c] = acc[mt][(8 * h + c) >> 2][c & 3];
                    if (FULL) {
                        v[c] += bias_v[8 * h + c];
                        csum[8 * h + c] += v[c];
                        csq[8 * h + c] = fmaf(v[c], v[c], csq[8 * h + c]);
                    }
                }
                if (eact != PAI_ACT_NONE) {
#pragma unroll
                    for (int c = 0; c < 8; ++c) v[c] = act_fwd(v[c], eslope);
                }
                *(uint4*)(Cs + row * CROW + (col0 + 8 * h) * 2) =
                    make_uint4(pk2bf(v[0], v[1]), pk2bf(v[2], v[3]), pk2bf(v[4], v[5]), pk2bf(v[6], v[7]));
            }
        }
        if (FULL && has_stats) {
#pragma unroll
            for (int c = 0; c < CL; ++c) {
                float s = csum[c], q = csq[c];
                s += __builtin_bit_cast(float, __builtin_amdgcn_update_dpp(0, __builtin_bit_cast(int, s), 0xB1, 0xF, 0xF, false));
                q += __builtin_bit_cast(float, __builtin_amdgcn_update_dpp(0, __builtin_bit_cast(int, q), 0xB1, 0xF, 0xF, false));
                s += __builtin_bit_cast(float, __builtin_amdgcn_update_dpp(0, __builtin_bit_cast(int, s), 0x4E, 0xF, 0xF, false));
                q += __builtin_bit_cast(float, __builtin_amdgcn_update_dpp(0, __builtin_bit_cast(int, q), 0x4E, 0xF, 0xF, false));
                s += __builtin_bit_cast(float, __builtin_amdgcn_update_dpp(0, __builtin_bit_cast(int, s), 0x141, 0xF, 0xF, false));
                q += __builtin_bit_cast(float, __builtin_amdgcn_update_dpp(0, __builtin_bit_cast(int, q), 0x141, 0xF, 0xF, false));
                s += __builtin_bit_cast(float, __builtin_amdgcn_update_dpp(0, __builtin_bit_cast(int, s), 0x140, 0xF, 0xF, false));
                q += __builtin_bit_cast(float, __builtin_amdgcn_update_dpp(0, __builtin_bit_cast(int, q), 0x140, 0xF, 0xF, false));
                if (fr == 0) {
                    sstat[(wm * 2 + 0) * BN + col0 + c] = s;
                    sstat[(wm * 2 + 1) * BN + col0 + c] = q;
                }
            }
        }
    };
    if (has_bias || has_stats) stage(std::true_type{});
    else stage(std::false_type{});
    if (bwd && bap) {
#pragma unroll
        for (int p = 0; p < NB; ++p) aq[p] = *(const uint4*)(at + (toff + (unsigned)p * pstep));
    }
    BwdParams BP;
    float bs1[8], bs2[8];
#pragma unroll
    for (int k = 0; k < 8; ++k) bs1[k] = bs2[k] = 0.f;
    if (bwd) bwd_load_params(a, dcol + oc * 8, BP);
    __syncthreads();
    if (has_stats && tid < BN) {
        float* dst = a.stats + ((size_t)(ph * mtiles + bm) * 2) * g.Cout + n0 + tid;
        float s = 0.f, q = 0.f;
#pragma unroll
        for (int i = 0; i < WM; ++i) { s += sstat[(i * 2 + 0) * BN + tid]; q += sstat[(i * 2 + 1) * BN + tid]; }
        dst[0] = s;
        dst[g.Cout] = q;
    }
    auto store_tile = [&](auto bwd_tag, auto add_tag, auto sum_tag) {
        constexpr bool BWD = decltype(bwd_tag)::value, ADD = decltype(add_tag)::value, SUM = decltype(sum_tag)::value;
        auto request = [&](int pass, int slot) {
            const unsigned off = toff + (unsigned)pass * pstep;
            if (BWD && !(EPI_ABL & 1)) zq[slot] = *(const uint4*)(zt + off);
            if (BWD && ADD) aq[slot] = *(const uint4*)(at + off);
        };
#pragma unroll
        for (int b = 0; b < NBATCH; ++b) {
#pragma unroll
            for (int p = 0; p < NB; ++p) {
                const int pass = b * NB + p;
                uint4 o = *(const uint4*)(Cs + (orow0 + pass * ORP) * CROW + oc * 16);
                if (EPI_ABL & 1) zq[p] = o;
                if (BWD && !(EPI_ABL & 2)) o = bwd_chunk_t<ADD, SUM>(o, zq[p], aq[p], sl1, sl2, BP, bs1, bs2);
                if (BWD && (EPI_ABL & 2)) { o.x ^= zq[p].x; if (ADD) o.y ^= aq[p].y; }
                if (b + 1 < NBATCH) request(pass + NB, p);
                if (!(EPI_ABL & 4) || o.x == 0x12345u) *(uint4*)(dt + (toff + (unsigned)pass * pstep)) = o;
                __builtin_amdgcn_sched_barrier(0);
            }
        }
    };
    typedef std::true_type T_;
    typedef std::false_type F_;
    if (!bwd) store_tile(F_{}, F_{}, F_{});
    else if (bap) { if (bsum) store_tile(T_{}, T_{}, T_{}); else store_tile(T_{}, T_{}, F_{}); }
    else { if (bsum) store_tile(T_{}, F_{}, T_{}); else store_tile(T_{}, F_{}, F_{}); }
    if (bsum)
        bwd_write_partials<BN, CPR, NTHR / 64>(sstat, bs1, bs2, tid,
                                               a.bpart + ((size_t)(ph * mtiles + bm) * 2) * g.D1 + n0, g.D1,
                                               a.bmean + n0, a.brstd + n0);
}

template <int BM, int BN, bool DBB>
__global__ __launch_bounds__(BM * 2, (BM == 128 && DBB) ? (BN == 64 ? 4 : 3) : (BN == 64 ? 5 : 4)) void gg_fwd_patch_k(GG g, FwdArgs a, PatchGeo pg, int mtiles, int ntiles) {
    gg_fwd_patch_body<BM, BN, DBB, 2, 64, PATCH_COLSWZ_ALL || !(BN == 128 && (BM == 256 || !DBB))>(g, a, pg, mtiles, ntiles);
}
template <int BM, int BN, bool DBB>
__global__ __launch_bounds__(BM, 3) void gg_fwd_patch1_k(GG g, FwdArgs a, PatchGeo pg, int mtiles, int ntiles) {
    gg_fwd_patch_body<BM, BN, DBB, 1>(g, a, pg, mtiles, ntiles);
}
static size_t fwd_lds_bytes(int bm, int bn, bool db) {
    const size_t main_loop = (size_t)(db ? 2 : 1) * (bm * 128 + bn * 128);
    const size_t epilogue = bm * (bn * 2 + 16) + (bm / 64 * 2) * 2 * bn * sizeof(float);
    return main_loop > epilogue ? main_loop : epilogue;
}

#define FWD_MFMA_VARIANTS(X)                                         \
    X(FWD_SPLITK128_DB, TILE, gg_fwd_mfma_k, 128, 128, true, true, 64)   \
    X(FWD_SPLITK128, TILE, gg_fwd_mfma_k, 128, 128, true, false, 64)     \
    X(FWD_SPLITK64, TILE, gg_fwd_mfma_k, 128, 64, true, false, 64)       \
    X(FWD_PATCH1_256, PATCH, gg_fwd_patch1_k, 256, 64, false)            \
    X(FWD_PATCH256_DBB, PATCH, gg_fwd_patch_k, 256, 128, true)           \
    X(FWD_PATCH128_DBB, PATCH, gg_fwd_patch_k, 128, 128, true)           \
    X(FWD_PATCH128N, PATCH, gg_fwd_patch_k, 128, 64, false)              \
    X(FWD_TILE128, TILE, gg_fwd_mfma_k, 128, 128, false, false, 64)      \
    X(FWD_TILE64, TILE, gg_fwd_mfma_k, 128, 64, false, false, 64)
#define X(id, form, k, ...) id,
enum FwdMfmaVariant { FWD_MFMA_VARIANTS(X) };
#undef X
#define X(id, form, k, ...) #k "<" #__VA_ARGS__ ">",
static const char* const fwd_mfma_names[] = {FWD_MFMA_VARIANTS(X)};
#undef X

MfmaPlan fwd_mfma_plan(const GG& g) {
    MfmaPlan p = {};
    FwdCfg c = fwd_cfg(g);
    p.workspace_bytes = c.ksplit > 1 ? (int64_t)c.ksplit * g.nphase * g.M * g.Cout * 4 : 0;
    if (c.ksplit > 1 && (pai_ctx()->workspace == nullptr || pai_ctx()->workspace_bytes < p.workspace_bytes)) c.ksplit = 1;
    p.ksplit = c.ksplit;
    p.bm = 128;
    p.bn = c.bn;
    p.mtiles = cdiv(g.M, p.bm);
    p.ntiles = g.Cout / c.bn;
    const int prow = patch_rows(g, c, &p.pg);
    p.rows = c.ksplit > 1 ? cdiv(g.M, FIN_ROWS) : (prow == 256 ? g.M / 256 : p.mtiles);
    int waves = 0;
    bool db = false;
    size_t patch_bytes = 0;
    if (c.ksplit > 1) {
        db = c.bn == 128 && pai_tunable("fwd_splitk_db", 1);
        p.variant = c.bn == 64 ? FWD_SPLITK64 : (db ? FWD_SPLITK128_DB : FWD_SPLITK128);
    } else if (prow == 256 && c.bn == 64) {
        waves = 4; patch_bytes = PatchDims<256, 1>::BYTES;
        p.variant = FWD_PATCH1_256;
    } else if (prow == 256) {
        db = true; waves = 8; patch_bytes = PatchDims<256>::BYTES;
        p.variant = FWD_PATCH256_DBB;
    } else if (prow == 128) {
        db = c.bn == 128; waves = 4; patch_bytes = PatchDims<128>::BYTES;
        p.variant = db ? FWD_PATCH128_DBB : FWD_PATCH128N;
    } else p.variant = c.bn == 128 ? FWD_TILE128 : FWD_TILE64;
    p.db = db;
    p.name = fwd_mfma_names[p.variant];
    if (waves) {
        p.bm = prow;
        p.mtiles = g.M / prow;
        p.block = waves * 64;
        const size_t lds = patch_bytes + (size_t)c.bn * 128 * (db ? 2 : 1);
        const size_t epi = prow * ((size_t)c.bn * 2 + 16) + waves * 2 * c.bn * sizeof(float);
        p.lds = lds > epi ? lds : epi;
    } else {
        p.block = p.bm / 64 * 128;
        p.lds = fwd_lds_bytes(p.bm, c.bn, db);
    }
    p.grid = p.mtiles * p.ntiles * g.nphase * c.ksplit;
    return p;
}

static int fwd_lds_opt_in();
int launch_fwd_mfma(const GG& g, const FwdArgs& a, const MfmaPlan& p, hipStream_t s) {
    float* ws = pai_ctx()->workspace;
    if (p.lds > 64 * 1024 && fwd_lds_opt_in()) return 1;
#define FWD_LAUNCH_TILE(k, ...) PAI_LAUNCH((k<__VA_ARGS__>), p.grid, p.block, p.lds, s, g, a, p.mtiles, p.ntiles, p.ksplit, ws)
#define FWD_LAUNCH_PATCH(k, ...) PAI_LAUNCH((k<__VA_ARGS__>), p.grid, p.block, p.lds, s, g, a, p.pg, p.mtiles, p.ntiles)
#define X(id, form, k, ...) case id: FWD_LAUNCH_##form(k, __VA_ARGS__); break;
    switch (p.variant) { FWD_MFMA_VARIANTS(X) }
#undef X
#undef FWD_LAUNCH_TILE
#undef FWD_LAUNCH_PATCH
    PAI_LAUNCH_CHECK();
    if (p.ksplit > 1)
        PAI_LAUNCH(splitk_finish_k, dim3(p.rows, g.nphase, cdiv(g.Cout, FIN_COLS)), dim3(256), 0, s, g, a, ws, p.rows, p.ksplit);
    PAI_LAUNCH_CHECK();
    return 0;
}
static int fwd_lds_opt_in() {
    static PerDeviceOnce attr_set;
    if (!attr_set.first()) return 0;
    const hipError_t e = hipFuncSetAttribute(reinterpret_cast<const void*>(&gg_fwd_patch_k<256, 128, true>),
                                             hipFuncAttributeMaxDynamicSharedMemorySize, 80 * 1024);
    PAI_CHECK(e == hipSuccess, "hipFuncSetAttribute(max dynamic LDS): %s", hipGetErrorString(e));
    return 0;
}

bool pw_ok(int dtype, const GG& g, const FwdArgs& a) {
    if (dtype != PAI_BF16 || g.ntaps != 1 || g.nphase != 1 || g.C2 != 0 || g.D2 != 0) return false;
    if (!((g.C1 == 64 && g.Cout == 32) || (g.C1 == 32 && g.Cout == 64))) return false;
    if (a.yf32 || a.skip_d1) return false;
    if ((a.y1 != nullptr) == (a.yact != nullptr)) return false;
    if (a.yact && a.eact != PAI_ACT_NONE && a.eact != PAI_ACT_LRELU && a.eact != PAI_ACT_RELU) return false;
    return true;
}

int pw_rows(const GG& g) {
    int64_t b = ((int64_t)g.M + 63) / 64;
    return (int)(b > 2048 ? 2048 : (b < 1 ? 1 : b));
}

template <int CIN, int COUT>
__global__ __launch_bounds__(256) void pw_k(GG g, FwdArgs a, int groups_per_wave) {
    constexpr int KB = CIN / 32, NTT = COUT / 16, CL = COUT / 4, NCH = CL / 8;
    __shared__ float sred[4][2][COUT];
    const int tid = threadIdx.x, lane = tid & 63, wid = tid >> 6;
    const int fr = lane & 15, fq = lane >> 4;
    const bf16_t* x = (const bf16_t*)a.x1;
    const bf16_t* w = (const bf16_t*)a.w;
    bf16_t* y = (bf16_t*)(a.yact ? a.yact : a.y1);
    const float eslope = act_slope(a.yact ? a.eact : PAI_ACT_NONE);
    bf8_t wf[NTT][KB];
#pragma unroll
    for (int nt = 0; nt < NTT; ++nt)
#pragma unroll
        for (int kb = 0; kb < KB; ++kb)
            wf[nt][kb] = *(const bf8_t*)(w + (size_t)(CL * (fr >> 2) + 4 * nt + (fr & 3)) * CIN + kb * 32 + fq * 8);
    const int c0 = CL * fq;
    float bias_v[CL], s1[CL], s2[CL];
#pragma unroll
    for (int c = 0; c < CL; ++c) { bias_v[c] = a.bias ? a.bias[c0 + c] : 0.f; s1[c] = s2[c] = 0.f; }
    const bool bwd = a.bz != nullptr && !a.yact;
    const bool bsum = bwd && a.bpart;
    const bf16_t* bzp = (const bf16_t*)a.bz;
    const bf16_t* bap = (const bf16_t*)a.badd;
    BwdParams BP[NCH];
    if (bwd) {
#pragma unroll
        for (int h = 0; h < NCH; ++h) bwd_load_params(a, c0 + 8 * h, BP[h]);
    }
    const int64_t ngroups = ((int64_t)g.M + 15) / 16;
    const int64_t g0 = ((int64_t)blockIdx.x * 4 + wid) * groups_per_wave;
    for (int64_t gi = g0; gi < g0 + groups_per_wave && gi < ngroups; ++gi) {
        const int64_t pix = gi * 16 + fr;
        const bool valid = pix < g.M;
        const int64_t pc = valid ? pix : 0;
        bf8_t xb[KB];
#pragma unroll
        for (int kb = 0; kb < KB; ++kb) {
            xb[kb] = *(const bf8_t*)(x + pc * CIN + kb * 32 + fq * 8);
            if (g.relu1) xb[kb] = relu_frag(xb[kb]);
        }
        uint4 zq[NCH], aq[NCH];
        if (bwd) {
#pragma unroll
            for (int h = 0; h < NCH; ++h) {
                zq[h] = *(const uint4*)(bzp + pc * COUT + c0 + 8 * h);
                aq[h] = bap ? *(const uint4*)(bap + pc * COUT + c0 + 8 * h) : make_uint4(0, 0, 0, 0);
            }
        }
        f4_t acc[NTT];
#pragma unroll
        for (int nt = 0; nt < NTT; ++nt) {
            acc[nt] = (f4_t){0.f, 0.f, 0.f, 0.f};
#pragma unroll
            for (int kb = 0; kb < KB; ++kb)
                acc[nt] = __builtin_amdgcn_mfma_f32_16x16x32_bf16(wf[nt][kb], xb[kb], acc[nt], 0, 0, 0);
        }
        unsigned pk[CL / 2];
#pragma unroll
        for (int nt = 0; nt < NTT; ++nt) {
            float v[4];
#pragma unroll
            for (int r = 0; r < 4; ++r) {
                v[r] = acc[nt][r] + bias_v[4 * nt + r];
                if (a.stats && valid) { s1[4 * nt + r] += v[r]; s2[4 * nt + r] = fmaf(v[r], v[r], s2[4 * nt + r]); }
                v[r] = act_fwd(v[r], eslope);
            }
            pk[2 * nt] = pk2bf(v[0], v[1]);
            pk[2 * nt + 1] = pk2bf(v[2], v[3]);
        }
#pragma unroll
        for (int h = 0; h < NCH; ++h) {
            uint4 o = make_uint4(pk[4 * h], pk[4 * h + 1], pk[4 * h + 2], pk[4 * h + 3]);
            if (bwd && valid)
                o = bwd_chunk(o, zq[h], aq[h], bap != nullptr, a.bscale != nullptr, bsum, a.bact1, a.bact2, BP[h],
                              s1 + 8 * h, s2 + 8 * h);
            if (valid) *(uint4*)(y + pix * COUT + c0 + 8 * h) = o;
        }
    }
    float* prow = a.stats ? a.stats : (bsum ? a.bpart : nullptr);
    if (prow) {
#pragma unroll
        for (int c = 0; c < CL; ++c) {
            float u = s1[c], q = s2[c];
            u += __builtin_bit_cast(float, __builtin_amdgcn_update_dpp(0, __builtin_bit_cast(int, u), 0xB1, 0xF, 0xF, false));
            q += __builtin_bit_cast(float, __builtin_amdgcn_update_dpp(0, __builtin_bit_cast(int, q), 0xB1, 0xF, 0xF, false));
            u += __builtin_bit_cast(float, __builtin_amdgcn_update_dpp(0, __builtin_bit_cast(int, u), 0x4E, 0xF, 0xF, false));
            q += __builtin_bit_cast(float, __builtin_amdgcn_update_dpp(0, __builtin_bit_cast(int, q), 0x4E, 0xF, 0xF, false));
            u += __builtin_bit_cast(float, __builtin_amdgcn_update_dpp(0, __builtin_bit_cast(int, u), 0x141, 0xF, 0xF, false));
            q += __builtin_bit_cast(float, __builtin_amdgcn_update_dpp(0, __builtin_bit_cast(int, q), 0x141, 0xF, 0xF, false));
            u += __builtin_bit_cast(float, __builtin_amdgcn_update_dpp(0, __builtin_bit_cast(int, u), 0x140, 0xF, 0xF, false));
            q += __builtin_bit_cast(float, __builtin_amdgcn_update_dpp(0, __builtin_bit_cast(int, q), 0x140, 0xF, 0xF, false));
            if (fr == 0) { sred[wid][0][c0 + c] = u; sred[wid][1][c0 + c] = q; }
        }
        __syncthreads();
        if (tid < COUT) {
            float u = 0.f, q = 0.f;
#pragma unroll
            for (int wv = 0; wv < 4; ++wv) { u += sred[wv][0][tid]; q += sred[wv][1][tid]; }
            float* dst = prow + (size_t)blockIdx.x * 2 * COUT;
            dst[tid] = u;
            dst[COUT + tid] = a.stats ? q : a.brstd[tid] * (q - a.bmean[tid] * u);
        }
    }
}

int launch_pw(const GG& g, const FwdArgs& a, hipStream_t s) {
    const int blocks = pw_rows(g);
    const int64_t ngroups = ((int64_t)g.M + 15) / 16;
    const int gpw = (int)((ngroups + (int64_t)blocks * 4 - 1) / ((int64_t)blocks * 4));
    if (g.C1 == 64) PAI_LAUNCH((pw_k<64, 32>), dim3(blocks), dim3(256), 0, s, g, a, gpw);
    else PAI_LAUNCH((pw_k<32, 64>), dim3(blocks), dim3(256), 0, s, g, a, gpw);
    PAI_LAUNCH_CHECK();
    return 0;
}

bool wgrad_mfma_ok(int dtype, const GG& g) {
    if (dtype != PAI_BF16) return false;
    if (g.lsw < 0) return false;
    if (g.ntaps == 1 && g.C2 == 0 && ((g.C1 == 64 && g.Cout == 32) || (g.C1 == 32 && g.Cout == 64))) return true;
    if (g.ntaps == 1 && g.C2 == 0 && g.C1 == 64 && (g.Cout % 64) == 0) return true;
    if (g.nphase == 1 && g.S == 1 && g.C2 == 0 && (g.C1 % 8) == 0 && (g.Cout % 8) == 0 && (g.C1 < 64 || g.Cout < 64))
        return true;
    if (g.C1 % 64 || g.C2 % 64) return false;
// ... 553 lines not shown
```

### thesis-pai-reconstruction_amd/engine.py

```python
from __future__ import annotations

import os
from typing import Callable, List, Optional

import torch
import torch.nn as nn

from . import ops
from .ops import ACT_LRELU, ACT_NONE, ACT_RELU, ACT_TANH

BN_EPS_DEFAULT = 1e-5


def _fwd_pack_strides(mod) -> tuple:
    if isinstance(mod, nn.ConvTranspose2d):
        cin, cout, kh, kw = mod.weight.shape
        return (1, kh * kw * cin, kw * cin, cin)
    cout, cin, kh, kw = mod.weight.shape
    return (kh * kw * cin, 1, kw * cin, cin)


def _strides_match(t: torch.Tensor, want: tuple) -> bool:
    return all(s == w or n == 1 for s, w, n in zip(t.stride(), want, t.shape))

# ... 311 lines not shown
                          for i, c in enumerate(self.enc_conv)]
        self.dec_packs = [_Packs(c, need_dgrad=True, gen=self.weights_generation) for c in self.dec_conv]
        self._plans = {}
        self._arena: Optional[GradArena] = None
        self._side = _SideStream()
        self.grad_ready_hook: Optional[Callable[[GradArena, int], None]] = None
        self.debug_capture: Optional[dict] = None

    def _dbg(self, name, t):
        if self.debug_capture is not None:
            self.debug_capture[name] = t.detach().clone()

    def _dropout(self, S, j, M, C, dtype):
        p = self.dec_drop[j]
        N = S["P"]["N"]
        if self.dropout_mask_fn is not None:
            mask = self.dropout_mask_fn(j, N, C, p, S["r"][j].device).to(torch.float32).contiguous()
        else:
            keep = torch.full((N, C), 1.0 - p, dtype=torch.float32, device=S["r"][j].device)
            mask = torch.bernoulli(keep) / (1.0 - p)
        S["drop"][j] = mask
        ops.dropout2d(dtype, S["r"][j], mask, N, M // N, C, S["r"][j])

    def ordered_params(self):
        out = []
        L = self.L
        for j in range(L - 1, -1, -1):
            if self.dec_bn[j] is not None:
                out += [(self.dec_bn[j].weight, None), (self.dec_bn[j].bias, None)]
            out += [(self.dec_conv[j].weight, self.dec_conv[j]), (self.dec_conv[j].bias, None)]
        for i in range(L - 1, -1, -1):
            if self.enc_bn[i] is not None:
                out += [(self.enc_bn[i].weight, None), (self.enc_bn[i].bias, None)]
            out += [(self.enc_conv[i].weight, self.enc_conv[i]), (self.enc_conv[i].bias, None)]
        return out

    def arena(self) -> GradArena:
        dev = self.enc_conv[0].weight.device
        if self._arena is None or self._arena.flat.device != dev:
            for c in self.enc_conv + self.dec_conv:
                to_fwd_pack_(c)
            self._arena = GradArena(self.ordered_params(), dev)
        return self._arena

    def pack_targets(self):
        arena = self.arena()
        if getattr(self, "_pt_cache", (None, None))[0] is not arena:
            self._pt_cache = (arena, pack_targets(arena, self.enc_packs + self.dec_packs))
        return self._pt_cache[1]

    def all_packs(self):
        return self.enc_packs + self.dec_packs

    def _plan(self, N, H, W, dtype, device):
        key = (N, H, W, dtype, str(device))
        if key in self._plans:
            return self._plans[key]
        L = self.L
        if H % (1 << L) or W % (1 << L):
            raise ops.PaiError(f"input {H}x{W} must be divisible by 2^{L}")
        P = {"N": N, "H": H, "W": W, "dtype": dtype, "device": device, "slots": [], "free": []}
        eh = [H >> (i + 1) for i in range(L)]
        ew = [W >> (i + 1) for i in range(L)]
        P["eh"], P["ew"] = eh, ew
        P["enc_desc"] = []
        cin = self.in_ch
        for i in range(L):
            hin = H >> i
            win = W >> i
            act = ACT_LRELU if i == 0 else ACT_NONE
            P["enc_desc"].append(ops.make_desc(dtype, 0, N, hin, win, cin, 0, self.enc_c[i], 2, 0, 0, act))
            cin = self.enc_c[i]
        P["dec_desc"] = []
        for j in range(L):
            hin, win = eh[L - 1 - j], ew[L - 1 - j]
            if j == 0:
                c1, c2, r1, r2 = self.enc_c[L - 1], 0, 1, 0
            else:
                c1, c2 = self.dec_c[j - 1], self.enc_c[L - 1 - j]
                r1, r2 = 0, 1
            act = ACT_NONE
            if j == L - 1:
                r1, r2, act = 0, 0, ACT_TANH
            P["dec_desc"].append(ops.make_desc(dtype, 1, N, hin, win, c1, c2, self.dec_c[j], 2, r1, r2, act))
        rows = 1
        for i in range(L):
            if self.enc_bn[i] is not None:
                rows = max(rows, ops.bn_stats_buffer_rows(ops.conv_fwd_stats_rows_max(P["enc_desc"][i]))
                           * 2 * self.enc_c[i])
        for j in range(L):
            if self.dec_bn[j] is not None:
                rows = max(rows, ops.bn_stats_buffer_rows(ops.conv_fwd_stats_rows_max(P["dec_desc"][j]))
                           * 2 * self.dec_c[j])
        P["stats"] = torch.empty(rows, dtype=torch.float32, device=device)
        mx = 1
        for i in range(L):
            if self.enc_bn[i] is not None:
                mx = max(mx, ops.bn_bwd_partial_rows(N * eh[i] * ew[i]) * 2 * self.enc_c[i])
        for j in range(L):
            if self.dec_bn[j] is not None:
                mx = max(mx, ops.bn_bwd_partial_rows(N * 4 * eh[L - 1 - j] * ew[L - 1 - j]) * 2 * self.dec_c[j])
        for i in range(2, L):
            if self.enc_bn[i - 1] is not None:
                mx = max(mx, ops.conv_dgrad_bn_rows_max(P["enc_desc"][i]) * 2 * self.enc_c[i - 1])
        for j in range(1, L):
            if self.dec_bn[j - 1] is not None:
                mx = max(mx, ops.conv_dgrad_bn_rows_max(P["dec_desc"][j]) * 2 * self.dec_c[j - 1])
        P["bwd_partials"] = torch.empty(mx, dtype=torch.float32, device=device)
        ops.ensure_workspace(max(ops.conv_workspace_bytes(d, op) for d in P["enc_desc"] + P["dec_desc"]
                                 for op in (0, 1)), device)
        ops.ensure_scratch(ops.scratch_bytes_for(P["enc_desc"] + P["dec_desc"]), device)
        ops.ensure_wgrad_workspace(P["enc_desc"] + P["dec_desc"], device)
        self._plans[key] = P
        return P

    def _new_slot(self, P):
        L, N, dt, dev = self.L, P["N"], P["dtype"], P["device"]
        eh, ew = P["eh"], P["ew"]

        def buf(h, w, c, dtype=dt):
            return torch.empty(N * h * w * c, dtype=dtype, device=dev)

        S = {"P": P}
        S["x"] = buf(P["H"], P["W"], self.in_ch)
        S["z"] = [buf(eh[i], ew[i], self.enc_c[i]) for i in range(L)]
        S["a"] = [buf(eh[i], ew[i], self.enc_c[i]) if i < L - 1 else None for i in range(L)]
        S["ebn"] = [_BNState(self.enc_c[i], dev) if self.enc_bn[i] is not None else None for i in range(L)]
        dh = [eh[L - 1 - j] * 2 for j in range(L)]
        dw = [ew[L - 1 - j] * 2 for j in range(L)]
        S["dh"], S["dw"] = dh, dw
        S["w"] = [buf(dh[j], dw[j], self.dec_c[j]) if j < L - 1 else None for j in range(L)]
        S["r"] = [buf(dh[j], dw[j], self.dec_c[j]) if j < L - 1 else None for j in range(L)]
        S["dbn"] = [_BNState(self.dec_c[j], dev) if self.dec_bn[j] is not None else None for j in range(L)]
        S["pred"] = torch.empty(N, self.out_ch, P["H"], P["W"], dtype=torch.float32, device=dev)
        S["grads"] = None
        return S

    def _grad_bufs(self, S):
        if S["grads"] is not None:
            return S["grads"]
        P = S["P"]
        L, N, dt, dev = self.L, P["N"], P["dtype"], P["device"]
        eh, ew = P["eh"], P["ew"]
        G = {}
        G["ga"] = [torch.empty_like(S["z"][i]) if i < L - 1 else None for i in range(L)]
        G["gskip"] = [torch.empty_like(S["z"][i]) if i < L - 1 else None for i in range(L)]
        G["gz_last"] = torch.empty_like(S["z"][L - 1])
        G["gr"] = [torch.empty_like(S["w"][j]) if j < L - 1 else None for j in range(L)]
        biggest = max([S["z"][i].numel() for i in range(L)] + [S["w"][j].numel() for j in range(L - 1)]
                      + [S["pred"].numel()])
        G["du"] = torch.empty(biggest, dtype=dt, device=dev)
        G["dz_head"] = torch.empty(S["pred"].numel(), dtype=dt, device=dev)
        G["dz_dec"] = [torch.empty_like(S["w"][j]) if j < L - 1 else None for j in range(L)]
        G["dz_enc"] = [torch.empty_like(S["z"][i]) for i in range(L)]
        S["grads"] = G
        return G

    def acquire(self, N, H, W, dtype, device):
        P = self._plan(N, H, W, dtype, device)
        if P["free"]:
            return P["free"].pop()
        S = self._new_slot(P)
        P["slots"].append(S)
        return S

    def release(self, S):
        S["P"]["free"].append(S)

    def forward(self, x: torch.Tensor, training: bool, bn_updates: int, dtype: torch.dtype):
        if not x.is_cuda:
            raise ops.PaiError("Unet (HIP) needs a HIP device tensor; there is no CPU path")
        N, Ci, H, W = x.shape
        if Ci != self.in_ch:
            raise ops.PaiError(f"expected {self.in_ch} input channels, got {Ci}")
        L = self.L
        S = self.acquire(N, H, W, dtype, x.device)
        P = S["P"]
        S["drop"] = {}
        xs = x.to(torch.float32)
        xs = xs.contiguous() if Ci == 1 else xs.permute(0, 2, 3, 1).contiguous()
        if dtype == torch.float32:
            S["x"] = xs.reshape(-1)
        else:
            ops.cast(xs, S["x"])
        eh, ew = P["eh"], P["ew"]
        refresh_packs(self.enc_packs + self.dec_packs, dtype)

        wf, _ = self.enc_packs[0].get(dtype)
        ops.conv_fwd(P["enc_desc"][0], S["x"], None, wf, self.enc_conv[0].bias, y_raw=S["z"][0],
                     y_act=S["a"][0] if L > 1 else None)
        for i in range(1, L):
            wf, _ = self.enc_packs[i].get(dtype)
            bn = self.enc_bn[i]
            d = P["enc_desc"][i]
            if bn is not None:
                M = N * eh[i] * ew[i]
                if training:
                    _conv_bn_train(d, S["a"][i - 1], None, wf, self.enc_conv[i].bias, S["z"][i], S["a"][i], ACT_LRELU,
                                   bn, S["ebn"][i], bn_updates, P["stats"])
                else:
                    ops.conv_fwd(d, S["a"][i - 1], None, wf, self.enc_conv[i].bias, y_raw=S["z"][i])
                    _bn_forward(bn, S["ebn"][i], None, 0, M, False, 0)
                    ops.bn_apply(dtype, S["z"][i], M, self.enc_c[i], S["ebn"][i].scale, S["ebn"][i].shift,
                                 ACT_LRELU, S["a"][i])
            else:
                ops.conv_fwd(d, S["a"][i - 1], None, wf, self.enc_conv[i].bias, y_raw=S["z"][i])
                if i < L - 1:
                    raise ops.PaiError("only the last encoder may be norm-free")
        for j in range(L):
            wf, _ = self.dec_packs[j].get(dtype)
            d = P["dec_desc"][j]
            if j == 0:
                x1, x2 = S["z"][L - 1], None
            else:
                x1 = S["r"][j - 1]
                skip = L - 1 - j
                x2 = S["a"][skip] if skip > 0 else S["z"][0]
                if j == L - 1:
                    x2 = S["z"][0]
            if j < L - 1:
                bn = self.dec_bn[j]
                M = N * S["dh"][j] * S["dw"][j]
                act = ACT_RELU if j < L - 2 else ACT_NONE
                if training:
                    _conv_bn_train(d, x1, x2, wf, self.dec_conv[j].bias, S["w"][j], S["r"][j], act, bn, S["dbn"][j],
                                   bn_updates, P["stats"])
                else:
                    ops.conv_fwd(d, x1, x2, wf, self.dec_conv[j].bias, y_raw=S["w"][j])
                    _bn_forward(bn, S["dbn"][j], None, 0, M, False, 0)
                    ops.bn_apply(dtype, S["w"][j], M, self.dec_c[j], S["dbn"][j].scale, S["dbn"][j].shift, act,
                                 S["r"][j])
                if training and self.dec_drop[j] > 0:
                    self._dropout(S, j, M, self.dec_c[j], dtype)
            else:
                S["pred"] = torch.empty_like(S["pred"])
                ops.conv_fwd(d, x1, x2, wf, self.dec_conv[j].bias, y_f32=S["pred"])
        if L == 1:
            raise ops.PaiError("Unet needs at least two levels")
        pred = S["pred"]
        if self.out_ch != 1:
            pred = pred.view(N, H, W, self.out_ch).permute(0, 3, 1, 2)
        return pred, S

    def backward(self, S, gpred: torch.Tensor, fresh: bool = False):
        P = S["P"]
        L, N, dtype = self.L, P["N"], P["dtype"]
        eh, ew = P["eh"], P["ew"]
        G = self._grad_bufs(S)
        A = self.arena()
        hook = self.grad_ready_hook
        if self.out_ch != 1:
            gpred = gpred.permute(0, 2, 3, 1)
        gpred = gpred.contiguous()
        if gpred.dtype != torch.float32:
            gpred = gpred.float()

        def done(p):
            if hook is not None:
                hook(A, A.end_of(p))

        side = self._side

        conv_wgrad = ops.conv_wgrad_overwrite_w if fresh else ops.conv_wgrad

        batch_n = int(os.environ.get("PAI_WGRAD_BATCH", "3"))
        held = []

        def flush_held():
            if held:
                with torch.cuda.stream(side.fork()):
                    for run in held:
                        run()
                held.clear()

        def wgrad(d, x1, x2, dz, conv, with_bias):
            def run():
                thin = min(_cin_cout(conv)) <= 2
                fn = ops.conv_wgrad if thin else conv_wgrad
                fn(d, x1, x2, dz, A.seg(conv.weight), A.seg(conv.bias) if with_bias else None)
                if thin:
                    side.mark_scratch()
                done(conv.bias)
            if batch_n > 1 and dz.numel() // max(1, conv.weight.shape[1] if isinstance(conv, nn.ConvTranspose2d) else conv.weight.shape[0]) <= int(os.environ.get("PAI_WGRAD_BATCH_PIX", "1024")):
                held.append(run)
                if len(held) >= batch_n:
                    flush_held()
                return
            flush_held()
            with torch.cuda.stream(side.fork(d)):
                run()

        j = L - 1
        dh = G["dz_head"]
        ops.tanh_bwd(dtype, S["pred"], gpred, None, dh)
        d = P["dec_desc"][j]
        x1 = S["r"][j - 1]
        x2 = S["z"][0]
        wgrad(d, x1, x2, dh, self.dec_conv[j], True)
        _, wd = self.dec_packs[j].get(dtype)
        part = P["bwd_partials"]
        fused_rows = None
        if (j - 1) in S["drop"] or self.dec_bn[j - 1] is None:
            ops.conv_dgrad(d, dh, wd, G["gr"][j - 1], G["gskip"][0])
            if (j - 1) in S["drop"]:
                ops.dropout2d(dtype, G["gr"][j - 1], S["drop"][j - 1], N, S["dh"][j - 1] * S["dw"][j - 1], self.dec_c[j - 1],
                              G["gr"][j - 1])
        else:
            pst, pbn = S["dbn"][j - 1], self.dec_bn[j - 1]
            ops.conv_dgrad_bn_apply(d, dh, wd, G["gr"][j - 1], G["gskip"][0], S["w"][j - 1], ACT_NONE, None, ACT_NONE,
                                    None, None, pst.mean, pst.rstd, part, pbn.weight, pst.sums, A.seg(pbn.weight),
                                    A.seg(pbn.bias), G["dz_dec"][j - 1])
            fused_rows = -1
        for j in range(L - 2, -1, -1):
            bn, st, conv = self.dec_bn[j], S["dbn"][j], self.dec_conv[j]
            M = N * S["dh"][j] * S["dw"][j]
            C = self.dec_c[j]
            n = M * C
            act = ACT_RELU if j < L - 2 else ACT_NONE
            dz = G["dz_dec"][j]
            if fused_rows is None:
                du = G["du"][:n] if act != ACT_NONE else G["gr"][j]
                ops.bn_bwd_reduce(dtype, G["gr"][j], act, None, ACT_NONE, S["r"][j] if act != ACT_NONE else None,
                                  S["w"][j], M, C, st.mean, st.rstd, du if act != ACT_NONE else None, part, st.sums,
                                  A.seg(bn.weight), A.seg(bn.bias))
                ops.bn_bwd_apply(dtype, du, S["w"][j], M, C, st.mean, st.rstd, bn.weight, st.sums, dz)
            self._dbg(f"dec{j}.dz", dz)
            d = P["dec_desc"][j]
            if j == 0:
                x1, x2 = S["z"][L - 1], None
            else:
                skip = L - 1 - j
                x1, x2 = S["r"][j - 1], (S["a"][skip] if skip > 0 else S["z"][0])
            wgrad(d, x1, x2, dz, conv, False)
            _, wd = self.dec_packs[j].get(dtype)
            if j == 0:
                fused_rows = ops.conv_dgrad_bn(d, dz, wd, G["dz_enc"][L - 1], None, S["z"][L - 1], ACT_RELU)
            elif (j - 1) in S["drop"]:
                ops.conv_dgrad(d, dz, wd, G["gr"][j - 1], G["gskip"][L - 1 - j])
                ops.dropout2d(dtype, G["gr"][j - 1], S["drop"][j - 1], N, S["dh"][j - 1] * S["dw"][j - 1],
                              self.dec_c[j - 1], G["gr"][j - 1])
                fused_rows = None
            else:
                pst, pbn = S["dbn"][j - 1], self.dec_bn[j - 1]
                ops.conv_dgrad_bn_apply(d, dz, wd, G["gr"][j - 1], G["gskip"][L - 1 - j], S["w"][j - 1], ACT_RELU, None,
                                        ACT_NONE, pst.scale, pst.shift, pst.mean, pst.rstd, part, pbn.weight, pst.sums,
                                        A.seg(pbn.weight), A.seg(pbn.bias), G["dz_dec"][j - 1])
                fused_rows = -1
        i = L - 1
        conv = self.enc_conv[i]
        dz = G["dz_enc"][i]
        d = P["enc_desc"][i]
        wgrad(d, S["a"][i - 1], None, dz, conv, True)
        _, wd = self.enc_packs[i].get(dtype)

        def enc_dgrad(i, dz, wd):
            d = P["enc_desc"][i]
            if i - 1 == 0:
                return ops.conv_dgrad_bn(d, dz, wd, G["dz_enc"][0], None, S["z"][0], ACT_LRELU, G["gskip"][0], ACT_NONE)
            pst, pbn = S["ebn"][i - 1], self.enc_bn[i - 1]
            ops.conv_dgrad_bn_apply(d, dz, wd, G["ga"][i - 1], None, S["z"][i - 1], ACT_LRELU, G["gskip"][i - 1], ACT_RELU,
                                    pst.scale, pst.shift, pst.mean, pst.rstd, part, pbn.weight, pst.sums,
                                    A.seg(pbn.weight), A.seg(pbn.bias), G["dz_enc"][i - 1])
            return -1

        fused_rows = enc_dgrad(i, dz, wd)
        for i in range(L - 2, 0, -1):
            bn, st, conv = self.enc_bn[i], S["ebn"][i], self.enc_conv[i]
            M = N * eh[i] * ew[i]
            C = self.enc_c[i]
            dz = G["dz_enc"][i]
            d = P["enc_desc"][i]
            wgrad(P["enc_desc"][i], S["a"][i - 1], None, dz, conv, False)
            _, wd = self.enc_packs[i].get(dtype)
            fused_rows = enc_dgrad(i, dz, wd)
        conv0 = self.enc_conv[0]
        flush_held()
        with torch.cuda.stream(side.fork_tail()):
            (ops.conv_wgrad if min(_cin_cout(conv0)) <= 2 else conv_wgrad)(
                P["enc_desc"][0], S["x"], None, G["dz_enc"][0], A.seg(conv0.weight), A.seg(conv0.bias))
        side.join()
        done(conv0.bias)


class DiscEngine:
    def __init__(self, disc: nn.Module):
        seq = disc.discriminator
        self.convs = [seq[i].block[0] for i in range(4)] + [seq[4]]
        self.in_ch = self.convs[0].weight.shape[1] // 2
        self.chans = [c.weight.shape[0] for c in self.convs]
        self.weights_generation = [0]
        self.packs = [_Packs(c, need_dgrad=True, gen=self.weights_generation) for c in self.convs]
        self._plans = {}
        self._arena = None
        self._side = _SideStream()
        self.grad_ready_hook = None

    def ordered_params(self):
        out = [(self.convs[4].weight, self.convs[4])]
        for k in range(3, -1, -1):
            out += [(self.convs[k].weight, self.convs[k]), (self.convs[k].bias, None)]
        return out

    def arena(self) -> GradArena:
        dev = self.convs[0].weight.device
        if self._arena is None or self._arena.flat.device != dev:
            for c in self.convs:
                to_fwd_pack_(c)
            self._arena = GradArena(self.ordered_params(), dev)
        return self._arena

    def pack_targets(self):
        arena = self.arena()
        if getattr(self, "_pt_cache", (None, None))[0] is not arena:
            self._pt_cache = (arena, pack_targets(arena, self.packs))
        return self._pt_cache[1]

    def all_packs(self):
        return self.packs

    def _plan(self, N, H, W, dtype, device):
        key = (N, H, W, dtype, str(device))
        if key in self._plans:
            return self._plans[key]
        if H % 16 or W % 16 or H < 32 or W < 32:
            raise ops.PaiError(f"discriminator input {H}x{W} must be a multiple of 16 and >= 32")
        P = {"N": N, "H": H, "W": W, "dtype": dtype, "device": device, "free": [], "desc": []}
        c = self.in_ch
        P["desc"].append(ops.make_desc(dtype, 0, N, H, W, c, c, self.chans[0], 2, 0, 0, ACT_LRELU))
        for k in range(1, 4):
            P["desc"].append(ops.make_desc(dtype, 0, N, H >> k, W >> k, self.chans[k - 1], 0, self.chans[k], 2, 0, 0,
                                           ACT_LRELU))
        P["desc"].append(ops.make_desc(dtype, 0, N, H >> 4, W >> 4, self.chans[3], 0, 1, 1, 0, 0, ACT_NONE))
        P["oh"], P["ow"] = (H >> 4) - 1, (W >> 4) - 1
        ops.ensure_workspace(max(ops.conv_workspace_bytes(d, op) for d in P["desc"] for op in (0, 1)), device)
        ops.ensure_scratch(ops.scratch_bytes_for(P["desc"]), device)
        ops.ensure_wgrad_workspace(P["desc"], device)
        self._plans[key] = P
        return P

    def acquire(self, N, H, W, dtype, device):
        P = self._plan(N, H, W, dtype, device)
        if P["free"]:
            return P["free"].pop()
        S = {"P": P}
        S["x"] = torch.empty(N * H * W * self.in_ch, dtype=dtype, device=device)
        S["y"] = torch.empty(N * H * W * self.in_ch, dtype=dtype, device=device)
        S["a"] = [torch.empty(N * (H >> (k + 1)) * (W >> (k + 1)) * self.chans[k], dtype=dtype, device=device)
                  for k in range(4)]
        S["logits"] = torch.empty(N, 1, P["oh"], P["ow"], dtype=torch.float32, device=device)
        S["grads"] = None
        return S

    def release(self, S):
        S["P"]["free"].append(S)

    def _to_nhwc(self, t, dst, dtype):
        t = t.to(torch.float32)
        t = t.contiguous() if t.shape[1] == 1 else t.permute(0, 2, 3, 1).contiguous()
        if dtype == torch.float32:
            return t.reshape(-1)
        ops.cast(t, dst)
        return dst

    def forward(self, x, y, dtype, y2=None, head: bool = True):
        if not (x.is_cuda and y.is_cuda):
            raise ops.PaiError("Discriminator (HIP) needs HIP device tensors; there is no CPU path")
        N, C, H, W = x.shape
        if C != self.in_ch or y.shape != x.shape or (y2 is not None and y2.shape != x.shape):
            raise ops.PaiError(f"Discriminator expects [N,{self.in_ch},H,W] tensors of one shape, got {tuple(x.shape)} "
                               f"and {tuple(y.shape)}")
        reps = 1 if y2 is None else 2
        S = self.acquire(N * reps, H, W, dtype, x.device)
        P = S["P"]
        if y2 is None and dtype != torch.float32 and C == 1:
            ops.cast_multi([(x.detach().to(torch.float32).contiguous().reshape(-1), S["x"]),
                            (y.detach().to(torch.float32).contiguous().reshape(-1), S["y"])])
            S["xin"], S["yin"] = S["x"], S["y"]
        elif y2 is None:
            S["xin"] = self._to_nhwc(x, S["x"], dtype)
            S["yin"] = self._to_nhwc(y, S["y"], dtype)
        else:
            half = N * H * W * C
            pairs = []
            for src, dst in ((x, S["x"][:half]), (x, S["x"][half:]), (y, S["y"][:half]), (y2, S["y"][half:])):
                t = src.detach().to(torch.float32)
                t = t.contiguous() if C == 1 else t.permute(0, 2, 3, 1).contiguous()
                pairs.append((t.reshape(-1), dst))
            ops.cast_multi(pairs)
            S["xin"], S["yin"] = S["x"], S["y"]
        refresh_packs(self.packs, dtype)
        wf, _ = self.packs[0].get(dtype)
        ops.conv_fwd(P["desc"][0], S["xin"], S["yin"], wf, self.convs[0].bias, y_act=S["a"][0])
        for k in range(1, 4):
            wf, _ = self.packs[k].get(dtype)
            ops.conv_fwd(P["desc"][k], S["a"][k - 1], None, wf, self.convs[k].bias, y_act=S["a"][k])
        S["head_done"] = False
        if not head:
            return None, S
        wf, _ = self.packs[4].get(dtype)
        S["logits"] = torch.empty_like(S["logits"])
        ops.conv_fwd(P["desc"][4], S["a"][3], None, wf, None, y_f32=S["logits"])
        return S["logits"], S

    @staticmethod
    def fused_enabled() -> bool:
        return os.environ.get("PAI_HEAD_FUSED", "1") not in ("", "0")

    def head_fused_ok(self, dtype) -> bool:
        return dtype == torch.bfloat16 and self.fused_enabled() and self.convs[4].bias is None

    def _grads(self, S):
        if S["grads"] is None:
            P = S["P"]
            S["grads"] = {"du": [torch.empty_like(a) for a in S["a"]],
                          "dl": torch.empty(S["logits"].numel(), dtype=P["dtype"], device=P["device"]),
                          "dl32": torch.empty(S["logits"].numel(), dtype=torch.float32, device=P["device"]),
                          "dy": torch.empty(P["N"] * P["H"] * P["W"] * self.in_ch, dtype=P["dtype"], device=P["device"])}
        return S["grads"]

    def forward_loss(self, x, y, dtype, y2, n_first, target_first, target_rest, acc, need_grad: bool):
        if not (x.is_cuda and y.is_cuda):
            raise ops.PaiError("Discriminator (HIP) needs HIP device tensors; there is no CPU path")
        N = x.shape[0] * (1 if y2 is None else 2)
        P = self._plan(N, x.shape[2], x.shape[3], dtype, x.device)
        if not ops.head_loss_ok(P["desc"][4], self.convs[4].bias is not None):
            return None
        _, S = self.forward(x, y, dtype, y2=y2, head=False)
        wf, wd = self.packs[4].get(dtype)
        G = self._grads(S) if need_grad else None
        ops.head_loss(P["desc"][4], S["a"][3], wf, wd if need_grad else None, n_first, target_first, target_rest, 1.0, acc, 1.0,
                      S["logits"], G["dl"] if need_grad else None, G["dl32"] if need_grad else None,
                      G["du"][3] if need_grad else None, ACT_LRELU)
        S["head_done"] = need_grad
        return S

    def _wgrad_desc(self, P, k):
        if os.environ.get("PAI_D_WGRAD_SOLO", "1") in ("", "0"):
            return P["desc"][k]
        solo = P.setdefault("desc_solo", {})
        if k not in solo:
            import copy
            d = copy.copy(P["desc"][k])
            d.hints = 1
            solo[k] = d
        return solo[k]

    def backward(self, S, glogits, need_params: bool, need_dy: bool, fresh: bool = False, head_done: bool = False,
                 addend=None):
        conv_wgrad = ops.conv_wgrad_overwrite_w if fresh else ops.conv_wgrad
        P = S["P"]
        N, H, W, dtype, dev = P["N"], P["H"], P["W"], P["dtype"], P["device"]
        G = self._grads(S)
        A = self.arena() if need_params else None
        hook = self.grad_ready_hook
        if head_done:
            if not S.get("head_done"):
                raise ops.PaiError("DiscEngine.backward(head_done=True) without a forward_loss that kept its gradients")
            dl = G["dl"]
        else:
            glogits = glogits.contiguous().float()
            if dtype == torch.float32:
                dl = glogits.reshape(-1)
            else:
                ops.cast(glogits, G["dl"])
                dl = G["dl"]
        d = P["desc"][4]
        side = self._side
        gy = None
        if need_params:
            with torch.cuda.stream(side.fork(d)):
                ops.conv_wgrad(d, S["a"][3], None, dl, A.seg(self.convs[4].weight), None)
                if hook is not None:
                    hook(A, A.end_of(self.convs[4].weight))
            side.mark_scratch()
        _, wd = self.packs[4].get(dtype)
        if not head_done:
            ops.conv_dgrad_act(d, dl, wd, G["du"][3], None, S["a"][3], ACT_LRELU)
        for k in range(3, -1, -1):
            conv = self.convs[k]
            d = P["desc"][k]
            if need_params and k == 0:
                with torch.cuda.stream(side.fork_tail()):
                    (ops.conv_wgrad if min(_cin_cout(conv)) <= 2 else conv_wgrad)(
                        d, S["xin"], S["yin"], G["du"][0], A.seg(conv.weight), A.seg(conv.bias))
            elif need_params:
                with torch.cuda.stream(side.fork(d)):
                    conv_wgrad(self._wgrad_desc(P, k), S["a"][k - 1], None, G["du"][k], A.seg(conv.weight), A.seg(conv.bias))
                    if hook is not None:
                        hook(A, A.end_of(conv.bias))
            if k > 0:
                _, wd = self.packs[k].get(dtype)
                ops.conv_dgrad_act(d, G["du"][k], wd, G["du"][k - 1], None, S["a"][k - 1], ACT_LRELU)
            elif need_dy:
                _, wd = self.packs[0].get(dtype)
                if addend is not None and self.in_ch == 1 and self.fused_enabled() and addend.dtype == torch.float32 \
                        and addend.is_contiguous() and addend.numel() == N * H * W and ops.conv_dgrad_f32add_ok(d):
                    gy = torch.empty(N * H * W, dtype=torch.float32, device=dev)
                    ops.conv_dgrad_f32add(d, G["du"][0], wd, addend, gy)
                else:
                    ops.conv_dgrad(d, G["du"][0], wd, None, G["dy"], only_c2=True)
        side.join()
        if need_params and hook is not None:
            hook(A, A.end_of(self.convs[0].bias))
        if not need_dy:
            return None
        if gy is not None:
            return gy.view(N, 1, H, W)
        gy = torch.empty(N * H * W * self.in_ch, dtype=torch.float32, device=dev)
        ops.cast(G["dy"], gy)
        gy = gy.view(N, 1, H, W) if self.in_ch == 1 else gy.view(N, H, W, self.in_ch).permute(0, 3, 1, 2)
        if addend is not None:
            if gy.is_contiguous() and gy.numel() % 8 == 0:
                ops.add_act(torch.float32, gy, addend, ops.ACT_NONE, gy)
            else:
                gy = gy + addend
        return gy
```

### thesis-pai-reconstruction_amd/lib.py

```python
from __future__ import annotations

import ctypes as C
import os

HERE = os.path.dirname(os.path.abspath(__file__))
LIB_PATH = os.environ.get("PAI_HIP_LIB") or os.path.join(HERE, "libpai_hip.so")

F32, BF16 = 0, 1
U8 = 2
ACT_NONE, ACT_LRELU, ACT_RELU, ACT_TANH = 0, 1, 2, 3
ACT_SILU = 4
HINT_SOLO = 1


class PaiError(RuntimeError):
    pass


class ConvDesc(C.Structure):
    _fields_ = [("dtype", C.c_int32), ("transposed", C.c_int32),
                ("N", C.c_int32), ("H", C.c_int32), ("W", C.c_int32),
                ("C1", C.c_int32), ("C2", C.c_int32), ("Cout", C.c_int32),
                ("kernel", C.c_int32), ("stride", C.c_int32), ("pad", C.c_int32),
                ("relu1", C.c_int32), ("relu2", C.c_int32), ("epilogue_act", C.c_int32),
                ("groups", C.c_int32), ("pack_flags", C.c_int32), ("hints", C.c_int32)]


class BwdEpilogue(C.Structure):
    _fields_ = [("z", C.c_void_p), ("add", C.c_void_p), ("scale", C.c_void_p), ("shift", C.c_void_p),
                ("mean", C.c_void_p), ("rstd", C.c_void_p), ("partials", C.c_void_p),
                ("act1", C.c_int32), ("act2", C.c_int32)]


class BnTrain(C.Structure):
    _fields_ = [("gamma", C.c_void_p), ("beta", C.c_void_p), ("eps", C.c_float), ("momentum", C.c_float),
                ("n_updates", C.c_int32), ("running_mean", C.c_void_p), ("running_var", C.c_void_p),
                ("num_batches_tracked", C.c_void_p), ("mean", C.c_void_p), ("rstd", C.c_void_p),
                ("scale", C.c_void_p), ("shift", C.c_void_p)]


_P = C.c_void_p
_I = C.c_int
_L = C.c_int64
_F = C.c_float
_D = C.POINTER(ConvDesc)

SIGNATURES = {
    "pai_last_error": (C.c_char_p, []),
    "pai_version": (_I, []),
    "pai_device_info": (_I, [C.POINTER(_I), C.POINTER(_I), C.c_char_p, _I]),
    "pai_set_tunable": (_I, [C.c_char_p, _I]),
    "pai_create": (_I, [_I, C.POINTER(C.c_void_p)]),
    "pai_bind": (_I, [C.c_void_p]),
    "pai_destroy": (_I, [C.c_void_p]),
    "pai_handle_set_workspace": (_I, [C.c_void_p, C.c_void_p, C.c_int64]),
    "pai_handle_set_scratch": (_I, [C.c_void_p, C.c_void_p, C.c_int64]),
    "pai_handle_set_wgrad_workspace": (_I, [C.c_void_p, C.c_void_p, C.c_int64]),
    "pai_conv_out_hw": (_I, [_D, C.POINTER(_I), C.POINTER(_I)]),
    "pai_conv_fwd_stats_rows": (_I, [_D]),
    "pai_conv_fwd_stats_rows_max": (_I, [_D]),
    "pai_bn_stats_buffer_rows": (_I, [_I]),
    "pai_conv_kernel_id": (_I, [_D, _I]),
    "pai_conv_kernel_name": (_I, [_D, _I, C.c_char_p, _I]),
    "pai_set_workspace": (_I, [_P, _L]),
    "pai_conv_workspace_bytes": (_L, [_D, _I]),
    "pai_set_scratch": (_I, [_P, _L]),
    "pai_conv_scratch_bytes": (_L, [_D, _I]),
    "pai_set_wgrad_workspace": (_I, [_P, _L]),
    "pai_conv_wgrad_workspace_bytes": (_L, [_D]),
    "pai_conv_fwd": (_I, [_D, _P, _P, _P, _P, _P, _P, _P, _P, _P]),
    "pai_conv_dgrad": (_I, [_D, _P, _P, _P, _P, _I, _P]),
    "pai_conv_dgrad_act": (_I, [_D, _P, _P, _P, _P, _P, _I, _P]),
    "pai_conv_dgrad_f32add_ok": (_I, [_D]),
    "pai_conv_dgrad_f32add": (_I, [_D, _P, _P, _P, _P, _P]),
    "pai_head_loss_ok": (_I, [_D, _I]),
    "pai_head_loss": (_I, [_D, _P, _P, _P, _I, _F, _F, _F, _P, _F, _P, _P, _P, _P, _P, _I, _P]),
    "pai_conv_dgrad_bn_rows_max": (_I, [_D]),
    "pai_conv_dgrad_bn": (_I, [_D, _P, _P, _P, _P, C.POINTER(BwdEpilogue), C.POINTER(_I), _P]),
    "pai_bn_bwd_finalize": (_I, [_P, _I, _I, _P, _P, _P, _P]),
    "pai_conv_fwd_bn": (_I, [_D, _P, _P, _P, _P, _P, _P, _I, C.POINTER(BnTrain), _P, _P]),
    "pai_conv_dgrad_bn_apply": (_I, [_D, _P, _P, _P, _P, C.POINTER(BwdEpilogue), _P, _P, _P, _P, _P, _P]),
    "pai_conv_bn_fused": (_I, [_D, _I]),
    "pai_conv_wgrad": (_I, [_D, _P, _P, _P, _P, _P, _P]),
    "pai_conv_wgrad_overwrite": (_I, [_D, _P, _P, _P, _P, _P, _P]),
    "pai_conv_wgrad_overwrite_w": (_I, [_D, _P, _P, _P, _P, _P, _P]),
    "pai_conv_prologue_ok": (_I, [_D]),
    "pai_conv_fwd_pro": (_I, [_D, _P, _P, _P, _P, _P, _P, _P, _I, _P]),
    "pai_conv_wgrad_pro": (_I, [_D, _P, _P, _P, _P, _I, _P, _P, _I, _P]),
    "pai_pack_weights": (_I, [_I, _P, _I, _I, _I, _P, _P, _P]),
    "pai_build_flags": (_I, []),
    "pai_pack_weights_multi": (_I, [_I, _P, _P, _P, _P, _P, _P, _P]),
    "pai_bn_finalize": (_I, [_P, _I, _I, _L, _P, _P, _F, _F, _I, _P, _P, _P, _P, _P, _P, _P, _P]),
    "pai_bn_eval_coeffs": (_I, [_I, _P, _P, _P, _P, _F, _P, _P, _P]),
    "pai_bn_apply": (_I, [_I, _P, _L, _I, _P, _P, _I, _P, _P]),
    "pai_bn2_add_act": (_I, [_I, _P, _P, _P, _P, _P, _P, _L, _I, _I, _I, _P, _P]),
    "pai_bn_bwd_partial_rows": (_I, [_L]),
    "pai_bn_bwd_reduce": (_I, [_I, _P, _I, _P, _I, _P, _P, _L, _I, _P, _P, _P, _P, _P, _P, _P, _P]),
    "pai_bn_bwd_reduce_affine": (_I, [_I, _P, _I, _P, _I, _P, _L, _I, _P, _P, _P, _P, _P, _P, _P, _P, _P, _P]),
    "pai_bn_bwd_apply": (_I, [_I, _P, _P, _L, _I, _P, _P, _P, _P, _P, _P]),
    "pai_bn_bwd_apply_affine": (_I, [_I, _P, _I, _P, _L, _I, _P, _P, _P, _P, _P, _P, _P, _P]),
    "pai_act_bwd": (_I, [_I, _P, _I, _P, _I, _P, _L, _P, _P]),
    "pai_maxpool2": (_I, [_I, _P, _I, _I, _I, _I, _P, _P, _P]),
    "pai_maxpool2_bwd": (_I, [_I, _P, _P, _I, _I, _I, _I, _P, _P]),
    "pai_upsample2": (_I, [_I, _P, _I, _I, _I, _I, _P, _P]),
    "pai_upsample2_bwd": (_I, [_I, _P, _I, _I, _I, _I, _P, _P]),
    "pai_add_act": (_I, [_I, _P, _P, _L, _I, _P, _P]),
    "pai_bn2_bwd_reduce": (_I, [_I, _P, _I, _P, _P, _L, _I, _P, _P, _P, _P, _P, _P, _P, _P, _P, _P, _P]),
    "pai_bn2_bwd_apply": (_I, [_I, _P, _I, _P, _P, _L, _I, _P, _P, _P, _P, _P, _P, _P, _P, _P, _P, _P, _P, _P]),
    "pai_instnorm_fwd": (_I, [_I, _P, _I, _I, _I, _F, _I, _P, _P, _P, _P]),
    "pai_instnorm_bwd": (_I, [_I, _P, _P, _I, _I, _I, _I, _P, _P, _P, _P]),
    "pai_dropout2d": (_I, [_I, _P, _P, _I, _L, _I, _P, _P]),
    "pai_layernorm_partial_rows": (_I, [_L]),
    "pai_layernorm_fwd": (_I, [_I, _P, _P, _L, _I, _P, _P, _F, _P, _I, _P, _P, _P, _P, _P]),
    "pai_layernorm_bwd": (_I, [_I, _P, _P, _L, _I, _P, _P, _P, _P, _P, _P, _P]),
    "pai_gelu": (_I, [_I, _P, _L, _P, _P]),
    "pai_gelu_bwd": (_I, [_I, _P, _P, _L, _P, _P]),
    "pai_mha_fwd": (_I, [_I, _P, _I, _I, _I, _I, _P, _P, _P, _P]),
    "pai_mha_bwd": (_I, [_I, _P, _P, _P, _I, _I, _I, _I, _P, _P, _P, _P]),
    "pai_mha_kernel_name": (_I, [_I, _I, _I, _I, C.c_char_p, _I]),
    "pai_subsample2": (_I, [_I, _P, _I, _I, _I, _I, _P, _P]),
    "pai_subsample2_bwd": (_I, [_I, _P, _I, _I, _I, _I, _P, _P]),
    "pai_bn_stats_rows": (_I, [_L]),
    "pai_bn_stats": (_I, [_I, _P, _L, _I, _P, _P]),
    "pai_colsum": (_I, [_I, _P, _L, _I, _P, _P]),
    "pai_gate_partial_rows": (_I, [_L]),
    "pai_gate_hidden": (_I, [_I, _P, _P, _L, _I, _P, _P, _P, _P, _P, _P, _P, _P, _P, _P]),
    "pai_gate_apply": (_I, [_I, _P, _P, _L, _I, _P, _P, _P, _P, _P]),
    "pai_gate_apply_bwd": (_I, [_I, _P, _P, _P, _P, _L, _I, _P, _P, _P, _P, _P, _I, _P]),
    "pai_gate_hidden_bwd": (_I, [_I, _P, _P, _P, _P, _P, _L, _I] + [_P] * 15),
    "pai_bce_logits": (_I, [_P, _L, _F, _F, _P, _F, _P, _P]),
    "pai_l1": (_I, [_P, _P, _L, _F, _P, _F, _P, _P]),
    "pai_mse": (_I, [_P, _P, _L, _F, _P, _F, _P, _P]),
    "pai_scalar_take": (_I, [_P, _P, _P]),
    "pai_metrics_take": (_I, [_P, _L, _L, _P, _P]),
    "pai_tanh_bwd": (_I, [_I, _P, _P, _P, _L, _P, _P]),
    "pai_denormalize": (_I, [_P, _P, _L, _P, _P]),
    "pai_ssim_sse": (_I, [_P, _P, _I, _I, _I, _I, _P, _P, _P, _P]),
    "pai_ssim_psnr_bwd": (_I, [_P, _P, _I, _I, _I, _I, _F, _F, _P, _P, _P, _P]),
    "pai_ssim_bwd_workspace_floats": (_L, [_I, _I, _I]),
    "pai_eval_planes": (_I, [_P, _P, _I, _I, _I, _I, _P, _P, _P, _P, _P, _P]),
    "pai_eval_kernel_name": (_I, [_I, C.c_char_p, _I]),
    "pai_cast": (_I, [_I, _P, _I, _P, _L, _P]),
    "pai_reduce_rows": (_I, [_P, _I, _I, _P, _I, _P]),
    "pai_adam": (_I, [_P, _P, _P, _P, _L, _F, _F, _F, _F, _I, _P]),
    "pai_adam_dev": (_I, [_P, _P, _P, _P, _L, _F, _F, _F, _F, _P, _P, _P]),
    "pai_adam_pack": (_I, [_P, _P, _P, _P, _L, _L, _I, _I, _I, _P, _P, _F, _F, _F, _F, _I, _P]),
    "pai_comm_unique_id": (_I, [_P]),
    "pai_comm_init": (_I, [_P, _I, _I, C.POINTER(_P)]),
    "pai_allreduce": (_I, [_P, _P, _L, _I, _P]),
    "pai_comm_destroy": (_I, [_P]),
    "pai_adam_multi": (_I, [_I, _P, _P, _P, _P, _P, _F, _F, _F, _F, _I, _P]),
    "pai_adam_multi_dev": (_I, [_I, _P, _P, _P, _P, _P, _F, _F, _F, _F, _P, _P, _P]),
    "pai_plan_create": (_I, [C.POINTER(_P)]),
    "pai_plan_destroy": (_I, [_P]),
    "pai_plan_begin": (_I, [_P]),
    "pai_plan_end": (_I, [_P]),
    "pai_plan_run": (_I, [_P, _L]),
    "pai_plan_info": (_I, [_P, C.POINTER(_I), C.POINTER(_I), C.POINTER(_I), C.POINTER(_L)]),
    "pai_stream_wait": (_I, [_P, _P]),
    "pai_stream_wait_last": (_I, [_P, _P]),
    "pai_event_create": (_I, [C.POINTER(_P)]),
    "pai_event_destroy": (_I, [_P]),
    "pai_event_record": (_I, [_P, _P]),
    "pai_event_create_timing": (_I, [C.POINTER(_P)]),
    "pai_event_elapsed_ms": (_I, [_P, _P, C.POINTER(_F)]),
    "pai_profile_arm": (_I, [_P, _P]),
    "pai_stream_wait_event": (_I, [_P, _P]),
    "pai_zero_multi": (_I, [_I, _P, _P, _P]),
    "pai_lerp_multi": (_I, [_I, _P, _P, _P, _F, _P]),
    "pai_scale": (_I, [_P, _L, _F, _P]),
    "pai_cast_multi": (_I, [_I, _I, _P, _I, _P, _P, _P]),
    "pai_filter_to_dense": (_I, [_P, _I, _I, _I, _I, _P, _P]),
    "pai_filter_grad_from_dense": (_I, [_P, _I, _I, _I, _I, _P, _P]),
    "pai_swap_mid": (_I, [_I, _P, C.c_int64, _I, _I, C.c_int64, _P, _P]),
    "pai_resize_aa_u8": (_I, [_P, _I, _I, _I, _I, _P, _P, _I, _P, _P, _I, _P, _P, _P]),
    "pai_batch_gather": (_I, [_I, _P, _P, _L, _L, _P, _I, _P, _P, _P, _P]),
    "pai_data_kernel_name": (_I, [_I, _I, C.c_char_p, _I]),
    "pai_sattn_fwd": (_I, [_I, _P, _I, _I, _I, _I, _P, _P]),
    "pai_sattn_fwd_lse": (_I, [_I, _P, _I, _I, _I, _I, _P, _P, _P]),
    "pai_sattn_bwd": (_I, [_I, _P, _P, _P, _P, _I, _I, _I, _I, _P, _P, _P]),
    "pai_sattn_kernel_name": (_I, [_I, _I, _I, C.c_char_p, _I]),
    "pai_affine_act": (_I, [_I, _P, _L, _I, _I, _P, _P, _I, _I, _P, _P]),
    "pai_film_coeffs": (_I, [_I, _I, _I, _P, _P, _P, _L, _P, _P, _P]),
    "pai_avgpool2": (_I, [_I, _P, _I, _I, _I, _I, _P, _P]),
    "pai_avgpool2_bwd": (_I, [_I, _P, _I, _I, _I, _I, _P, _P]),
    "pai_silu_bwd": (_I, [_I, _P, _P, _L, _P, _P]),
    "pai_gamma_embedding": (_I, [_I, _P, _I, _I, _P, _P]),
    "pai_palette_step": (_I, [_I, _P, _P, _P, _L, _I, _I, _I, _F, _F, _F, _F, _F, _F, _P, _P, _P]),
    "pai_film_norm_slabs": (_I, [_L]),
    "pai_film_norm_ws_floats": (_L, [_I, _L, _I]),
    "pai_film_norm_fwd": (_I, [_I, _P, _L, _I, _I, _P, _P, _P, _P, _P, _L, _P, _F, _I, _P, _P]),
    "pai_film_norm_bwd": (_I, [_I, _P, _P, _L, _I, _I, _P, _P, _P, _P, _P, _L, _P, _F, _I, _P, _P, _P, _P, _P, _P]),
    "pai_palette_noise": (_I, [_P, _P, _P, _P, _P, _P, _I, _I, _L, _I, _P, _P, _P, _P]),
    "pai_palette_objective_slabs": (_I, [_L]),
    "pai_palette_objective_ws_floats": (_L, [_I, _L]),
    "pai_palette_objective": (_I, [_P, _P, _P, _P, _P, _P, _I, _I, _L, _I, _I, _F, _P, _P, _P, _P]),
}

_lib = None


def load() -> C.CDLL:
    global _lib
    if _lib is not None:
        return _lib
    if not os.path.exists(LIB_PATH):
        raise PaiError(
            f"{LIB_PATH} is missing: build it with `python __graft_entry__.py` "
            "(hipcc --offload-arch=gfx950).  There is no fallback path.")
    lib = C.CDLL(LIB_PATH)
    for name, (res, args) in SIGNATURES.items():
        fn = getattr(lib, name)
        fn.restype = res
        fn.argtypes = args
    _lib = lib
    return lib


def check(rc: int, what: str):
    if rc != 0:
        msg = load().pai_last_error()
        raise PaiError(f"{what} failed ({rc}): {msg.decode() if msg else '?'}")


def ptr(t):
# ... 2 lines not shown
```

### thesis-pai-reconstruction_amd/ops.py

```python
from __future__ import annotations

import ctypes as C

import threading
from typing import Optional

import torch

from . import lib as L
from .lib import ACT_LRELU, ACT_NONE, ACT_RELU, ACT_SILU, ACT_TANH, BF16, F32, U8, ConvDesc, PaiError


def code_of(dtype: torch.dtype) -> int:
    if dtype == torch.float32:
        return F32
    if dtype == torch.bfloat16:
        return BF16
    raise PaiError(f"unsupported storage dtype {dtype}")


_TLS = threading.local()


def _stream():
# ... 133 lines not shown
class _TimedBytes:
    def __init__(self, family, nbytes):
        self.on = PROFILE_HBM is not None
        if self.on:
            self.family, self.nbytes = family, int(nbytes)
            self.e0 = torch.cuda.Event(enable_timing=True)
            self.e1 = torch.cuda.Event(enable_timing=True)

    def __enter__(self):
        if self.on:
            self.e0.record()

    def __exit__(self, *exc):
        if self.on:
            self.e1.record()
            PROFILE_HBM.append((self.family, self.nbytes, self.e0, self.e1))
        return False


def _es(dtype) -> int:
    return 4 if dtype == torch.float32 else 2


class Handle:

    def __init__(self, device):
        dev = torch.device(device)
        self.device = torch.device("cuda", dev.index if dev.index is not None else torch.cuda.current_device())
        self._h = C.c_void_p()
        L.check(L.load().pai_create(self.device.index, C.byref(self._h)), "pai_create")
        self.workspace = None
        self.scratch = None
        self.wgrad_workspace = None
        self.epoch = 0

    def bind(self):
        L.check(L.load().pai_bind(self._h), "pai_bind")
        return self

    def ensure_workspace(self, nbytes: int) -> None:
        if nbytes <= 0:
            return
        if self.workspace is None or self.workspace.numel() * 4 < nbytes:
            self.workspace = torch.zeros((nbytes + 3) // 4, dtype=torch.float32, device=self.device)
            self.epoch += 1
            L.check(L.load().pai_handle_set_workspace(self._h, self.workspace.data_ptr(), self.workspace.numel() * 4),
                    "pai_handle_set_workspace")

    def ensure_scratch(self, nbytes: int) -> None:
        if nbytes <= 0:
            return
        if self.scratch is None or self.scratch.numel() * 4 < nbytes:
            self.scratch = torch.empty((nbytes + 3) // 4, dtype=torch.float32, device=self.device)
            self.epoch += 1
            L.check(L.load().pai_handle_set_scratch(self._h, self.scratch.data_ptr(), self.scratch.numel() * 4),
                    "pai_handle_set_scratch")

    def ensure_wgrad_workspace(self, nbytes: int) -> None:
        if nbytes <= 0:
            return
        if self.wgrad_workspace is None or self.wgrad_workspace.numel() * 4 < nbytes:
            if self.wgrad_workspace is not None:
                torch.cuda.synchronize(self.device)
            self.wgrad_workspace = torch.empty((nbytes + 3) // 4, dtype=torch.float32, device=self.device)
            self.epoch += 1
            L.check(L.load().pai_handle_set_wgrad_workspace(self._h, self.wgrad_workspace.data_ptr(),
                                                           self.wgrad_workspace.numel() * 4),
                    "pai_handle_set_wgrad_workspace")

    def close(self):
        if self._h:
            L.check(L.load().pai_destroy(self._h), "pai_destroy")
            self._h = C.c_void_p()
            _HANDLES.pop(self.device.index, None) if _HANDLES.get(self.device.index) is self else None


_HANDLES = {}


def handle_for(device) -> Handle:
    dev = torch.device(device)
    idx = dev.index if dev.index is not None else torch.cuda.current_device()
    h = _HANDLES.get(idx)
    if h is None:
        h = _HANDLES[idx] = Handle(torch.device("cuda", idx))
    return h


def conv_workspace_bytes(d: ConvDesc, op: int) -> int:
    return L.load().pai_conv_workspace_bytes(C.byref(d), op)


def ensure_workspace(nbytes: int, device) -> None:
    handle_for(device).ensure_workspace(nbytes)


def conv_scratch_bytes(d: ConvDesc, op: int) -> int:
    return L.load().pai_conv_scratch_bytes(C.byref(d), op)


def scratch_bytes_for(descs) -> int:
    head = max((conv_scratch_bytes(d, op) for d in descs for op in (0, 1)), default=0)
    tail = max((conv_scratch_bytes(d, 2) for d in descs), default=0)
    return head + tail


def ensure_scratch(nbytes: int, device) -> None:
    handle_for(device).ensure_scratch(nbytes)


def conv_wgrad_workspace_bytes(d: ConvDesc) -> int:
    return L.load().pai_conv_wgrad_workspace_bytes(C.byref(d))


def ensure_wgrad_workspace(descs, device) -> None:
    handle_for(device).ensure_wgrad_workspace(max((conv_wgrad_workspace_bytes(d) for d in descs), default=0))


def conv_fwd(d, x1, x2, w, bias, y_raw=None, y_act=None, y_f32=None, stats=None):
    with _Timed(d, 0):
        L.check(L.load().pai_conv_fwd(C.byref(d), _p(x1), _p(x2), _p(w), _p(bias, torch.float32), _p(y_raw),
                                      _p(y_act), _p(y_f32, torch.float32), _p(stats, torch.float32),
                                      _stream()), "pai_conv_fwd")


def conv_prologue_ok(d) -> bool:
    return bool(L.load().pai_conv_prologue_ok(C.byref(d)))


def conv_fwd_pro(d, x1, w, bias, y_raw, stats, pre_scale, pre_shift, pre_act):
    with _Timed(d, 0):
        L.check(L.load().pai_conv_fwd_pro(C.byref(d), _p(x1), _p(w), _p(bias, torch.float32), _p(y_raw),
                                          _p(stats, torch.float32), _p(pre_scale, torch.float32), _p(pre_shift, torch.float32),
                                          int(pre_act), _stream()), "pai_conv_fwd_pro")


def conv_wgrad_pro(d, x1, dy, dw, dbias, overwrite, pre_scale, pre_shift, pre_act):
    with _Timed(d, 2):
        L.check(L.load().pai_conv_wgrad_pro(C.byref(d), _p(x1), _p(dy), _p(dw, torch.float32), _p(dbias, torch.float32),
                                            int(overwrite), _p(pre_scale, torch.float32), _p(pre_shift, torch.float32),
                                            int(pre_act), _stream()), "pai_conv_wgrad_pro")


def conv_dgrad(d, dy, w_dgrad, dx1, dx2=None, only_c2=False):
    with _Timed(d, 1):
        L.check(L.load().pai_conv_dgrad(C.byref(d), _p(dy), _p(w_dgrad), _p(dx1), _p(dx2), int(only_c2),
                                        _stream()), "pai_conv_dgrad")


def conv_dgrad_act(d, dy, w_dgrad, dx1, dx2, a1, act1):
    with _Timed(d, 1):
        L.check(L.load().pai_conv_dgrad_act(C.byref(d), _p(dy), _p(w_dgrad), _p(dx1), _p(dx2), _p(a1), int(act1),
                                            _stream()), "pai_conv_dgrad_act")


def conv_dgrad_f32add_ok(d) -> bool:
    return bool(L.load().pai_conv_dgrad_f32add_ok(C.byref(d)))


def conv_dgrad_f32add(d, dy, w_dgrad, addend, dx2_f32):
    with _Timed(d, 1):
        L.check(L.load().pai_conv_dgrad_f32add(C.byref(d), _p(dy), _p(w_dgrad), _p(addend, torch.float32),
                                               _p(dx2_f32, torch.float32), _stream()), "pai_conv_dgrad_f32add")


def head_loss_ok(d, has_bias: bool = False) -> bool:
    return bool(L.load().pai_head_loss_ok(C.byref(d), int(bool(has_bias))))


def head_loss(d, a3, w_fwd, w_dgrad, n_first, target_first, target_rest, loss_scale, loss, grad_scale, logits, dl=None,
              dl_f32=None, du=None, act=ACT_LRELU):
    L.check(L.load().pai_head_loss(C.byref(d), _p(a3, torch.bfloat16), _p(w_fwd), _p(w_dgrad), int(n_first),
                                   float(target_first), float(target_rest), float(loss_scale), _p(loss, torch.float64),
                                   float(grad_scale), _p(logits, torch.float32), _p(dl, torch.bfloat16),
                                   _p(dl_f32, torch.float32), _p(du, torch.bfloat16), _p(a3) if du is not None else None,
                                   int(act), _stream()), "pai_head_loss")


def conv_dgrad_bn_rows_max(d) -> int:
    return L.load().pai_conv_dgrad_bn_rows_max(C.byref(d))


def conv_dgrad_bn(d, dy, w_dgrad, dx1, dx2, z, act1, add=None, act2=ACT_NONE, scale=None, shift=None,
                  mean=None, rstd=None, partials=None) -> int:
    e = L.BwdEpilogue(_p(z), _p(add), _p(scale, torch.float32), _p(shift, torch.float32), _p(mean, torch.float32),
                      _p(rstd, torch.float32), _p(partials, torch.float32), int(act1), int(act2))
    rows = C.c_int(0)
    with _Timed(d, 1):
        L.check(L.load().pai_conv_dgrad_bn(C.byref(d), _p(dy), _p(w_dgrad), _p(dx1), _p(dx2), C.byref(e),
                                           C.byref(rows), _stream()), "pai_conv_dgrad_bn")
    return rows.value


def conv_fwd_bn(d, x1, x2, w, bias, z, a, act, gamma, beta, eps, momentum, n_updates, running_mean, running_var,
                num_batches_tracked, mean, rstd, scale, shift, stats):
    f32 = torch.float32
    bn = L.BnTrain(_p(gamma, f32), _p(beta, f32), float(eps), float(momentum), int(n_updates), _p(running_mean, f32),
                   _p(running_var, f32), _p(num_batches_tracked, torch.int64), _p(mean, f32), _p(rstd, f32),
                   _p(scale, f32), _p(shift, f32))
    with _Timed(d, 0):
        L.check(L.load().pai_conv_fwd_bn(C.byref(d), _p(x1), _p(x2), _p(w), _p(bias, f32), _p(z), _p(a), int(act),
                                         C.byref(bn), _p(stats, f32), _stream()), "pai_conv_fwd_bn")


def conv_bn_fused(d, op: int) -> bool:
    return L.load().pai_conv_bn_fused(C.byref(d), op) == 1


def conv_dgrad_bn_apply(d, dy, w_dgrad, du_scratch, dx2, z, act1, add, act2, scale, shift, mean, rstd, partials, gamma,
                        sums, dgamma, dbeta, dz):
    f32 = torch.float32
    e = L.BwdEpilogue(_p(z), _p(add), _p(scale, f32), _p(shift, f32), _p(mean, f32), _p(rstd, f32), _p(partials, f32),
                      int(act1), int(act2))
    with _Timed(d, 1):
        L.check(L.load().pai_conv_dgrad_bn_apply(C.byref(d), _p(dy), _p(w_dgrad), _p(du_scratch), _p(dx2), C.byref(e),
                                                 _p(gamma, f32), _p(sums, f32), _p(dgamma, f32), _p(dbeta, f32), _p(dz),
                                                 _stream()), "pai_conv_dgrad_bn_apply")


def bn_bwd_finalize(partials, rows, C_, sums, dgamma, dbeta):
    L.check(L.load().pai_bn_bwd_finalize(_p(partials, torch.float32), rows, C_, _p(sums, torch.float32),
                                         _p(dgamma, torch.float32), _p(dbeta, torch.float32), _stream()),
            "pai_bn_bwd_finalize")


def conv_wgrad(d, x1, x2, dy, dw, dbias=None):
    with _Timed(d, 2):
        L.check(L.load().pai_conv_wgrad(C.byref(d), _p(x1), _p(x2), _p(dy), _p(dw, torch.float32),
                                        _p(dbias, torch.float32), _stream()), "pai_conv_wgrad")


def conv_wgrad_overwrite(d, x1, x2, dy, dw, dbias=None):
    with _Timed(d, 2):
        L.check(L.load().pai_conv_wgrad_overwrite(C.byref(d), _p(x1), _p(x2), _p(dy), _p(dw, torch.float32),
                                                  _p(dbias, torch.float32), _stream()), "pai_conv_wgrad_overwrite")


def conv_wgrad_overwrite_w(d, x1, x2, dy, dw, dbias=None):
    with _Timed(d, 2):
        L.check(L.load().pai_conv_wgrad_overwrite_w(C.byref(d), _p(x1), _p(x2), _p(dy), _p(dw, torch.float32),
                                                    _p(dbias, torch.float32), _stream()), "pai_conv_wgrad_overwrite_w")


def pack_weights(dtype, w_master, Cout, taps, Cin, w_fwd=None, w_dgrad=None):
    L.check(L.load().pai_pack_weights(code_of(dtype), _p(w_master, torch.float32), Cout, taps, Cin, _p(w_fwd),
                                      _p(w_dgrad), _stream()), "pai_pack_weights")


TUNABLE_UNSET = -2147483648


def set_tunable(name: str, value: int = TUNABLE_UNSET) -> None:
    L.check(L.load().pai_set_tunable(name.encode(), int(value)), "pai_set_tunable")


def pack_weights_multi(items):
    import ctypes as C
    n = len(items)
    if n == 0:
        return
    ptrs = lambda k: (C.c_void_p * n)(*[_p(it[k]) if k == 0 else (_p(it[k]) if it[k] is not None else None) for it in items])
    ints = lambda k: (C.c_int32 * n)(*[int(it[k]) for it in items])
    for it in items:
        if it[0].dtype != torch.float32:
            raise PaiError("pack_weights_multi: fp32 master weights expected")
    L.check(L.load().pai_pack_weights_multi(n, ptrs(0), ints(1), ints(2), ints(3), ptrs(4), ptrs(5), _stream()),
            "pai_pack_weights_multi")


def bn_finalize(stats, rows, C_, count, gamma, beta, eps, momentum, n_updates, running_mean, running_var,
                nbt, mean, rstd, scale, shift):
    L.check(L.load().pai_bn_finalize(_p(stats), rows, C_, count, _p(gamma), _p(beta), eps, momentum, n_updates,
                                     _p(running_mean), _p(running_var), _p(nbt, torch.int64), _p(mean),
                                     _p(rstd), _p(scale), _p(shift), _stream()), "pai_bn_finalize")


def bn_eval_coeffs(C_, gamma, beta, running_mean, running_var, eps, scale, shift):
    L.check(L.load().pai_bn_eval_coeffs(C_, _p(gamma), _p(beta), _p(running_mean), _p(running_var), eps,
                                        _p(scale), _p(shift), _stream()), "pai_bn_eval_coeffs")


def bn_apply(dtype, z, M, C_, scale, shift, act, out):
    with _TimedBytes("bn_passes", 2 * M * C_ * _es(dtype)):
        L.check(L.load().pai_bn_apply(code_of(dtype), _p(z), M, C_, _p(scale), _p(shift), act, _p(out), _stream()),
                "pai_bn_apply")


def bn2_add_act(dtype, za, scale_a, shift_a, zb, scale_b, shift_b, M, C_, act_a, act, out):
    with _TimedBytes("bn_passes", 3 * M * C_ * _es(dtype)):
        L.check(L.load().pai_bn2_add_act(code_of(dtype), _p(za), _p(scale_a, torch.float32), _p(shift_a, torch.float32), _p(zb),
                                         _p(scale_b, torch.float32), _p(shift_b, torch.float32), M, C_, act_a, act, _p(out),
                                         _stream()), "pai_bn2_add_act")


def bn_bwd_partial_rows(M) -> int:
    return L.load().pai_bn_bwd_partial_rows(M)


def bn_bwd_reduce(dtype, g1, act1, g2, act2, a, z, M, C_, mean, rstd, du, partials, sums, dgamma, dbeta):
    streams = 2 + (g2 is not None) + (a is not None and z is not None and a.data_ptr() != z.data_ptr()) + (du is not None)
    with _TimedBytes("bn_passes", streams * M * C_ * _es(dtype)):
        L.check(L.load().pai_bn_bwd_reduce(code_of(dtype), _p(g1), act1, _p(g2), act2, _p(a), _p(z), M, C_, _p(mean),
                                           _p(rstd), _p(du), _p(partials), _p(sums), _p(dgamma), _p(dbeta),
                                           _stream()), "pai_bn_bwd_reduce")


# ... 683 lines not shown
```

Measured before the change: 11440 images/s.

## Fuse first-layer weight gradient into second-layer input-gradient kernel

Adds a fused kernel that computes the second conv's input gradient with activation backward and, in the same tile, the weight and bias gradients of the thin first conv (1-2 input channels to 64). It reads the raw input patch into LDS, runs MFMA for the weight gradient, and accumulates into fp32 slabs that a small reduction kernel sums afterwards. The goal is to skip writing and rereading the full-resolution first-layer activation gradient and to drop the separate thin wgrad launch in the generator encoder and the discriminator. In exchange the path adds slab memset and atomic traffic, a reduce launch, higher LDS use in the dgrad kernel, and loses the side-stream overlap of the old wgrad.

```diff
diff --git a/include/pai_hip.h b/include/pai_hip.h
--- a/include/pai_hip.h
+++ b/include/pai_hip.h
@@ -77,6 +77,13 @@
 
 int pai_conv_dgrad_act(const pai_conv_desc* d, const void* dy, const void* w_dgrad, void* dx1,
                        void* dx2, const void* a1, int act1, void* stream);
+
+int pai_conv_dgrad_act_wthin_ok(const pai_conv_desc* d, const pai_conv_desc* d_thin, int need_dx);
+int64_t pai_conv_dgrad_act_wthin_slab_bytes(const pai_conv_desc* d, const pai_conv_desc* d_thin);
+int pai_conv_dgrad_act_wthin_kernel_name(const pai_conv_desc* d, const pai_conv_desc* d_thin, char* name, int name_len);
+int pai_conv_dgrad_act_wthin(const pai_conv_desc* d, const void* dy, const void* w_dgrad, const void* a1, int act1,
+                             const void* add, int act2, const pai_conv_desc* d_thin, const void* x1, const void* x2,
+                             float* dw, float* dbias, int overwrite, float* slabs, int64_t slab_bytes, void* stream);
 
 typedef struct pai_bwd_epilogue {
     const void* z;
diff --git a/thesis-pai-reconstruction_amd/attention.py b/thesis-pai-reconstruction_amd/attention.py
--- a/thesis-pai-reconstruction_amd/attention.py
+++ b/thesis-pai-reconstruction_amd/attention.py
@@ -4,7 +4,7 @@
 import torch.nn as nn
 
 from . import ops
-from .engine import GradArena, UnetEngine, _BNState, _Packs, _bn_forward, to_fwd_pack_
+from .engine import GradArena, UnetEngine, _BNState, _Packs, _bn_forward, to_fwd_pack_, wthin_slabs
 from .ops import ACT_LRELU, ACT_NONE, ACT_RELU, ACT_TANH
 
 
@@ -320,10 +320,19 @@
         wgrad(P["enc_desc"][i], S["a"][i - 1], None, dz, self.enc_conv[i], True)
         _, wd = self.enc_packs[i].get(dtype)
 
+        enc0_fused = ops.conv_dgrad_act_wthin_ok(P["enc_desc"][1], P["enc_desc"][0], False)
+
         def enc_dgrad(i, dz, wd):
             d = P["enc_desc"][i]
             gx = G["gx"][L - 1 - (i - 1)]
+            if i - 1 == 0 and enc0_fused:
+                c0, d0 = self.enc_conv[0], P["enc_desc"][0]
+                ops.conv_dgrad_act_wthin(d, dz, wd, S["z"][0], ACT_LRELU, gx, ACT_NONE, d0, S["x"], None,
+                                         A.seg(c0.weight), A.seg(c0.bias), wthin_slabs(P, d, d0))
+                return 0
             if i - 1 == 0:
+                if G["dz_enc"][0] is None:
+                    G["dz_enc"][0] = torch.empty_like(S["z"][0])
                 return ops.conv_dgrad_bn(d, dz, wd, G["dz_enc"][0], None, S["z"][0], ACT_LRELU, gx, ACT_NONE)
             pst = S["ebn"][i - 1]
             return ops.conv_dgrad_bn(d, dz, wd, G["ga"][i - 1], None, S["z"][i - 1], ACT_LRELU, gx, ACT_NONE,
@@ -341,9 +350,10 @@
             _, wd = self.enc_packs[i].get(dtype)
             fused_rows = enc_dgrad(i, dz, wd)
         conv0 = self.enc_conv[0]
-        with torch.cuda.stream(side.fork_tail()):
-            c0_in, c0_out = conv0.weight.shape[1], conv0.weight.shape[0]
-            (ops.conv_wgrad_overwrite_w if (fresh and min(c0_in, c0_out) > 2) else ops.conv_wgrad)(
-                P["enc_desc"][0], S["x"], None, G["dz_enc"][0], A.seg(conv0.weight), A.seg(conv0.bias))
+        if not enc0_fused:
+            with torch.cuda.stream(side.fork_tail()):
+                c0_in, c0_out = conv0.weight.shape[1], conv0.weight.shape[0]
+                (ops.conv_wgrad_overwrite_w if (fresh and min(c0_in, c0_out) > 2) else ops.conv_wgrad)(
+                    P["enc_desc"][0], S["x"], None, G["dz_enc"][0], A.seg(conv0.weight), A.seg(conv0.bias))
         side.join()
         done(conv0.bias)
diff --git a/thesis-pai-reconstruction_amd/csrc/api.hip b/thesis-pai-reconstruction_amd/csrc/api.hip
--- a/thesis-pai-reconstruction_amd/csrc/api.hip
+++ b/thesis-pai-reconstruction_amd/csrc/api.hip
@@ -646,6 +646,83 @@
     return pai_act_bwd(d->dtype, dx1, act1, nullptr, PAI_ACT_NONE, a1, (int64_t)g.N * g.OH * g.OW * g.D1, dx1, stream);
 }
 
+struct WthinPick {
+    GG g, gt;
+    FwdPick p;
+    int T;
+};
+static const char* pick_wthin(const pai_conv_desc* d, const pai_conv_desc* dt, WthinPick* o) {
+    if (!d || !dt) return "null descriptor";
+    if (gg_build_dgrad(d, &o->g) || gg_build_fwd(dt, &o->gt)) return "invalid descriptor";
+    const GG &g = o->g, &gt = o->gt;
+    if (d->dtype != PAI_BF16 || dt->dtype != PAI_BF16) return "bf16 storage only";
+    if (d->transposed || dt->transposed || d->kernel != 4 || dt->kernel != 4 || d->stride != 2 || dt->stride != 2)
+        return "both layers are k4 s2 convolutions";
+    if (!thin_wgrad_conv_ok(dt->dtype, gt) || gt.Cout != 64) return "the thin layer is (1 | 1) -> 64 channels";
+    if (g.D1 != 64 || g.D2 != 0 || g.relu1) return "the next layer reads the thin layer's 64 channels, one tensor";
+    if (gt.N != g.N || gt.OH != g.OH || gt.OW != g.OW) return "the thin layer's output is not the next layer's input";
+    FwdArgs a = query_args(g, 1);
+    a.bz = (const void*)1;
+    o->p = pick_fwd(d->dtype, g, a);
+    o->T = gt.C1 + gt.C2;
+    if (o->p.k != FK_MFMA || !fwd_mfma_wthin(&o->p.mfma, o->T)) return "the input gradient does not run on 8 x 16-pixel, 64-channel patch tiles";
+    o->p.name = o->p.mfma.name;
+    return nullptr;
+}
+
+extern "C" int pai_conv_dgrad_act_wthin_ok(const pai_conv_desc* d, const pai_conv_desc* d_thin, int need_dx) {
+    WthinPick w;
+    return !need_dx && pai_tunable("dgrad_wthin", 1) && pick_wthin(d, d_thin, &w) == nullptr ? 1 : 0;
+}
+
+extern "C" int64_t pai_conv_dgrad_act_wthin_slab_bytes(const pai_conv_desc* d, const pai_conv_desc* d_thin) {
+    WthinPick w;
+    if (pick_wthin(d, d_thin, &w)) return -1;
+    int S = pai_tunable("wthin_slabs", 128);
+    S = S < 1 ? 1 : (S > 4096 ? 4096 : S);
+    return (int64_t)S * wthin_slab_floats(w.T) * sizeof(float);
+}
+
+extern "C" int pai_conv_dgrad_act_wthin_kernel_name(const pai_conv_desc* d, const pai_conv_desc* d_thin, char* name, int name_len) {
+    WthinPick w;
+    if (pick_wthin(d, d_thin, &w) || !name || name_len <= 0) return -1;
+    strncpy(name, w.p.name, name_len - 1);
+    name[name_len - 1] = 0;
+    return 0;
+}
+
+extern "C" int pai_conv_dgrad_act_wthin(const pai_conv_desc* d, const void* dy, const void* w_dgrad, const void* a1, int act1,
+                                        const void* add, int act2, const pai_conv_desc* d_thin, const void* x1, const void* x2,
+                                        float* dw, float* dbias, int overwrite, float* slabs, int64_t slab_bytes, void* stream) {
+    WthinPick w;
+    const char* why = pick_wthin(d, d_thin, &w);
+    PAI_CHECK(!why, "pai_conv_dgrad_act_wthin: %s (ask pai_conv_dgrad_act_wthin_ok)", why);
+    PAI_CHECK(dy && w_dgrad && a1 && x1 && dw && slabs, "pai_conv_dgrad_act_wthin: null pointer");
+    PAI_CHECK((w.T == 2) == (x2 != nullptr), "pai_conv_dgrad_act_wthin: x2 goes with the thin layer's second channel");
+    PAI_CHECK(((uintptr_t)x1 & 15) == 0 && ((uintptr_t)x2 & 15) == 0, "pai_conv_dgrad_act_wthin: the thin inputs are read in 16-B chunks");
+    for (int act : {act1, act2})
+        PAI_CHECK(act == PAI_ACT_LRELU || act == PAI_ACT_RELU || act == PAI_ACT_NONE, "pai_conv_dgrad_act_wthin: act=%d", act);
+    PAI_CHECK(overwrite >= 0 && overwrite <= 2, "pai_conv_dgrad_act_wthin: overwrite=%d", overwrite);
+    const int64_t per = (int64_t)wthin_slab_floats(w.T) * sizeof(float);
+    int S = pai_tunable("wthin_slabs", 128);
+    S = S < 1 ? 1 : (S > 4096 ? 4096 : S);
+    if ((int64_t)S * per > slab_bytes) S = (int)(slab_bytes / per);
+    PAI_CHECK(S >= 1, "pai_conv_dgrad_act_wthin: the slab buffer holds no slab (pai_conv_dgrad_act_wthin_slab_bytes)");
+    hipStream_t s = (hipStream_t)stream;
+    FwdArgs a;
+    memset(&a, 0, sizeof(a));
+    a.x1 = dy; a.w = w_dgrad;
+    a.y1 = (void*)a1;
+    a.bz = a1; a.bact1 = act1;
+    a.badd = add; a.bact2 = act2;
+    WThin wt;
+    wt.x1 = x1; wt.x2 = x2; wt.slab = slabs; wt.S = S; wt.TH = w.gt.H; wt.TW = w.gt.W;
+    hipError_t e = pai::memset_async(slabs, 0, (size_t)S * per, s);
+    PAI_CHECK(e == hipSuccess, "pai_conv_dgrad_act_wthin: hipMemsetAsync: %s", hipGetErrorString(e));
+    if (int rc = launch_fwd_mfma(w.g, a, w.p.mfma, s, &wt)) return rc;
+    return launch_wthin_reduce(slabs, S, w.T, dw, dbias, overwrite != 0, overwrite == 1, s);
+}
+
 extern "C" int pai_conv_dgrad_bn_rows_max(const pai_conv_desc* d) {
     GG g;
     if (gg_build_dgrad(d, &g)) return -1;
diff --git a/thesis-pai-reconstruction_amd/csrc/common.h b/thesis-pai-reconstruction_amd/csrc/common.h
--- a/thesis-pai-reconstruction_amd/csrc/common.h
+++ b/thesis-pai-reconstruction_amd/csrc/common.h
@@ -217,7 +217,15 @@
 };
 enum WgradMfmaVariant { WG3_128x64 = 1, WG3_64x128, WG3_128x64_8, WGRAD_PATCH128, WGRAD_PATCH64, WGRAD_TILE128, WGRAD_TILE64 };
 MfmaPlan fwd_mfma_plan(const GG& g);
-int launch_fwd_mfma(const GG& g, const FwdArgs& a, const MfmaPlan& p, hipStream_t s);
+struct WThin {
+    const void *x1, *x2;
+    float* slab;
+    int S, TH, TW;
+};
+static inline int wthin_slab_floats(int T) { return (16 * T + 1) * 64; }
+bool fwd_mfma_wthin(MfmaPlan* p, int T);
+int launch_fwd_mfma(const GG& g, const FwdArgs& a, const MfmaPlan& p, hipStream_t s, const WThin* wt = nullptr);
+int launch_wthin_reduce(const float* slab, int S, int T, float* dw, float* dbias, int overwrite_w, int overwrite_bias, hipStream_t s);
 MfmaPlan wgrad_mfma_plan(const GG& g, bool has_dbias, bool has_prologue);
 bool wgrad_pro_ok(int dtype, const GG& g);
 struct pai_handle_s {
diff --git a/thesis-pai-reconstruction_amd/csrc/gg_mfma.hip b/thesis-pai-reconstruction_amd/csrc/gg_mfma.hip
--- a/thesis-pai-reconstruction_amd/csrc/gg_mfma.hip
+++ b/thesis-pai-reconstruction_amd/csrc/gg_mfma.hip
@@ -463,9 +463,13 @@
 #ifndef PATCH_SETPRIO
 #define PATCH_SETPRIO 1
 #endif
-template <int BM, int BN, bool DBB, int WN = 2, int WPX = 64, bool COLSWZ = true>
-__device__ __forceinline__ void gg_fwd_patch_body(const GG& g, const FwdArgs& a, const PatchGeo& pg, int mtiles, int ntiles) {
+constexpr int WTH_XROW = 160;
+constexpr int WTH_XPLANE = 32 * WTH_XROW + 16;
+template <int BM, int BN, bool DBB, int WN = 2, int WPX = 64, bool COLSWZ = true, int WT = 0>
+__device__ __forceinline__ void gg_fwd_patch_body(const GG& g, const FwdArgs& a, const PatchGeo& pg, int mtiles, int ntiles,
+                                                  const WThin& wt = WThin{}) {
     static_assert(WN == 2 || BN == 64, "one wave column: 64 output channels");
+    static_assert(WT == 0 || (BM == 128 && BN == 64 && WN == 2 && WPX == 64), "the weight-gradient store: 8 x 16 pixels, 64 channels");
     constexpr int abl = PATCH_ABL;
     typedef PatchDims<BM, WN, WPX> PD;
     constexpr int NTHR = PD::NTHR, MT = WPX / 16, NT = BN / (16 * WN);
@@ -840,7 +844,73 @@
 #pragma unroll
     for (int k = 0; k < 8; ++k) bs1[k] = bs2[k] = 0.f;
     if (bwd) bwd_load_params(a, dcol + oc * 8, BP);
+    unsigned char* Xs = smem + BM * CROW + (NTHR / 64) * 2 * BN * sizeof(float);
+    if constexpr (WT > 0) {
+        const int iy0 = 4 * gy0 + 2 * g.poy[ph] - 1, ix0 = 4 * gx0 - 8;
+#pragma unroll
+        for (int i = 0; i < (320 * WT + NTHR - 1) / NTHR; ++i) {
+            const int q = tid + NTHR * i;
+            if (q < 320 * WT) {
+                const int t = q / 320, rem = q - t * 320, r = rem / 10, c = rem - r * 10;
+                const int iy = iy0 + r, ix = ix0 + 8 * c;
+                uint4 v = make_uint4(0u, 0u, 0u, 0u);
+                if ((unsigned)iy < (unsigned)wt.TH && (unsigned)ix < (unsigned)wt.TW)
+                    v = *(const uint4*)((const bf16_t*)(t ? wt.x2 : wt.x1) + ((size_t)(img * wt.TH + iy) * wt.TW + ix));
+                *(uint4*)(Xs + t * WTH_XPLANE + r * WTH_XROW + c * 16) = v;
+            }
+        }
+    }
     __syncthreads();
+    if constexpr (WT > 0) {
+#pragma unroll
+        for (int p = 0; p < NP; ++p) {
+            static_assert(NP == NB, "every producer chunk was requested up front");
+            uint4* cp = (uint4*)(Cs + (orow0 + p * ORP) * CROW + oc * 16);
+            *cp = bap ? bwd_chunk_t<true, false>(*cp, zq[p], aq[p], sl1, sl2, BP, bs1, bs2)
+                      : bwd_chunk_t<false, false>(*cp, zq[p], aq[p], sl1, sl2, BP, bs1, bs2);
+        }
+        __syncthreads();
+        const int tq = fr >> 2, tp = fr & 3;
+        const unsigned char* xb[WT];
+#pragma unroll
+        for (int tt = 0; tt < WT; ++tt) {
+            const int k = 16 * tt + fr, tap = k / WT, t = k - tap * WT, th = tap >> 2, tw = tap & 3;
+            xb[tt] = Xs + t * WTH_XPLANE + (4 * (fq >> 1) + th) * WTH_XROW + (7 + 2 * g.pox[ph] + tw + 32 * (fq & 1)) * 2;
+        }
+        const unsigned char* cb = Cs + (fq * 8 + tq) * CROW + (wid * 16 + 4 * tp) * 2;
+        const unsigned one2 = fr == 0 ? 0x3f803f80u : 0u;
+        const bf8_t ones = __builtin_bit_cast(bf8_t, make_uint4(one2, one2, one2, one2));
+        f4_t wacc[WT], bacc = (f4_t){0.f, 0.f, 0.f, 0.f};
+#pragma unroll
+        for (int tt = 0; tt < WT; ++tt) wacc[tt] = (f4_t){0.f, 0.f, 0.f, 0.f};
+#pragma unroll
+        for (int ks = 0; ks < BM / 32; ++ks) {
+            bf8_t bfr;
+#pragma unroll
+            for (int h = 0; h < 2; ++h) {
+                const bf4_t v = __builtin_amdgcn_ds_read_tr16_b64_v4bf16(
+                    (bf4_t __attribute__((address_space(3)))*)(cb + (ks * 32 + h * 4) * CROW));
+#pragma unroll
+                for (int e = 0; e < 4; ++e) bfr[h * 4 + e] = v[e];
+            }
+#pragma unroll
+            for (int tt = 0; tt < WT; ++tt) {
+                typedef __attribute__((ext_vector_type(8))) unsigned short us8_t;
+                us8_t pv;
+#pragma unroll
+                for (int j = 0; j < 8; ++j) pv[j] = *(const unsigned short*)(xb[tt] + ks * 8 * WTH_XROW + j * 8);
+                wacc[tt] = __builtin_amdgcn_mfma_f32_16x16x32_bf16(__builtin_bit_cast(bf8_t, pv), bfr, wacc[tt], 0, 0, 0);
+            }
+            bacc = __builtin_amdgcn_mfma_f32_16x16x32_bf16(ones, bfr, bacc, 0, 0, 0);
+        }
+        float* slab = wt.slab + (size_t)(blockIdx.x % (unsigned)wt.S) * ((16 * WT + 1) * 64);
+#pragma unroll
+        for (int tt = 0; tt < WT; ++tt)
+#pragma unroll
+            for (int r = 0; r < 4; ++r) unsafeAtomicAdd(slab + ((wid * WT + tt) * 4 + r) * 64 + lane, wacc[tt][r]);
+        if (fq == 0) unsafeAtomicAdd(slab + 16 * WT * 64 + wid * 16 + fr, bacc[0]);
+        return;
+    }
     if (has_stats && tid < BN) {
         float* dst = a.stats + ((size_t)(ph * mtiles + bm) * 2) * g.Cout + n0 + tid;
         float s = 0.f, q = 0.f;
@@ -890,6 +960,46 @@
 __global__ __launch_bounds__(BM, 3) void gg_fwd_patch1_k(GG g, FwdArgs a, PatchGeo pg, int mtiles, int ntiles) {
     gg_fwd_patch_body<BM, BN, DBB, 1>(g, a, pg, mtiles, ntiles);
 }
+template <int T>
+__global__ __launch_bounds__(256, 5) void gg_dgrad_wthin_k(GG g, FwdArgs a, PatchGeo pg, int mtiles, int ntiles, WThin wt) {
+    gg_fwd_patch_body<128, 64, false, 2, 64, true, T>(g, a, pg, mtiles, ntiles, wt);
+}
+__global__ __launch_bounds__(256) void wthin_reduce_k(const float* slab, int S, int T, float* dw, float* dbias, int ow_w, int ow_b) {
+    __shared__ float red[4][64];
+    const int n = (16 * T + 1) * 64;
+    const int e = blockIdx.x * 64 + (threadIdx.x & 63), slice = threadIdx.x >> 6;
+    const int per = (S + 3) / 4, b0 = slice * per, b1 = min(S, b0 + per);
+    float sum = 0.f;
+    if (e < n) {
+        const float* src = slab + e;
+        int b = b0;
+        for (; b + 8 <= b1; b += 8) {
+            float t[8];
+#pragma unroll
+            for (int u = 0; u < 8; ++u) t[u] = src[(size_t)(b + u) * n];
+            sum += ((t[0] + t[1]) + (t[2] + t[3])) + ((t[4] + t[5]) + (t[6] + t[7]));
+        }
+        for (; b < b1; ++b) sum += src[(size_t)b * n];
+    }
+    red[slice][threadIdx.x & 63] = sum;
+    __syncthreads();
+    if (slice == 0 && e < n) {
+        sum = (red[0][threadIdx.x] + red[1][threadIdx.x]) + (red[2][threadIdx.x] + red[3][threadIdx.x]);
+        if (e < 16 * T * 64) {
+            const int lane = e & 63, q = e >> 6, r = q & 3, tt = (q >> 2) % T, wave = (q >> 2) / T;
+            float* dst = dw + (16 * wave + (lane & 15)) * 16 * T + 16 * tt + 4 * (lane >> 4) + r;
+            *dst = ow_w ? sum : *dst + sum;
+        } else if (dbias) {
+            float* dst = dbias + (e - 16 * T * 64);
+            *dst = ow_b ? sum : *dst + sum;
+        }
+    }
+}
+int launch_wthin_reduce(const float* slab, int S, int T, float* dw, float* dbias, int overwrite_w, int overwrite_bias, hipStream_t s) {
+    PAI_LAUNCH(wthin_reduce_k, dim3(cdiv(wthin_slab_floats(T), 64)), dim3(256), 0, s, slab, S, T, dw, dbias, overwrite_w, overwrite_bias);
+    PAI_LAUNCH_CHECK();
+    return 0;
+}
 static size_t fwd_lds_bytes(int bm, int bn, bool db) {
     const size_t main_loop = (size_t)(db ? 2 : 1) * (bm * 128 + bn * 128);
     const size_t epilogue = bm * (bn * 2 + 16) + (bm / 64 * 2) * 2 * bn * sizeof(float);
@@ -904,6 +1014,8 @@
     X(FWD_PATCH256_DBB, PATCH, gg_fwd_patch_k, 256, 128, true)           \
     X(FWD_PATCH128_DBB, PATCH, gg_fwd_patch_k, 128, 128, true)           \
     X(FWD_PATCH128N, PATCH, gg_fwd_patch_k, 128, 64, false)              \
+    X(FWD_WTHIN1, WTHIN, gg_dgrad_wthin_k, 1)                            \
+    X(FWD_WTHIN2, WTHIN, gg_dgrad_wthin_k, 2)                            \
     X(FWD_TILE128, TILE, gg_fwd_mfma_k, 128, 128, false, false, 64)      \
     X(FWD_TILE64, TILE, gg_fwd_mfma_k, 128, 64, false, false, 64)
 #define X(id, form, k, ...) id,
@@ -958,17 +1070,31 @@
     return p;
 }
 
+bool fwd_mfma_wthin(MfmaPlan* p, int T) {
+    if (p->variant != FWD_PATCH128N || p->ntiles != 1 || (T != 1 && T != 2)) return false;
+    p->variant = T == 1 ? FWD_WTHIN1 : FWD_WTHIN2;
+    p->name = fwd_mfma_names[p->variant];
+    const size_t epi = 128 * (64 * 2 + 16) + 4 * 2 * 64 * sizeof(float) + (size_t)T * WTH_XPLANE;
+    if (epi > p->lds) p->lds = epi;
+    return true;
+}
+
 static int fwd_lds_opt_in();
-int launch_fwd_mfma(const GG& g, const FwdArgs& a, const MfmaPlan& p, hipStream_t s) {
+int launch_fwd_mfma(const GG& g, const FwdArgs& a, const MfmaPlan& p, hipStream_t s, const WThin* wt) {
     float* ws = pai_ctx()->workspace;
+    const bool wthin = p.variant == FWD_WTHIN1 || p.variant == FWD_WTHIN2;
+    PAI_CHECK(wthin == (wt != nullptr), "launch_fwd_mfma: the weight-gradient store and its arguments go together");
+    const WThin wta = wt ? *wt : WThin{};
     if (p.lds > 64 * 1024 && fwd_lds_opt_in()) return 1;
 #define FWD_LAUNCH_TILE(k, ...) PAI_LAUNCH((k<__VA_ARGS__>), p.grid, p.block, p.lds, s, g, a, p.mtiles, p.ntiles, p.ksplit, ws)
 #define FWD_LAUNCH_PATCH(k, ...) PAI_LAUNCH((k<__VA_ARGS__>), p.grid, p.block, p.lds, s, g, a, p.pg, p.mtiles, p.ntiles)
+#define FWD_LAUNCH_WTHIN(k, ...) PAI_LAUNCH((k<__VA_ARGS__>), p.grid, p.block, p.lds, s, g, a, p.pg, p.mtiles, p.ntiles, wta)
 #define X(id, form, k, ...) case id: FWD_LAUNCH_##form(k, __VA_ARGS__); break;
     switch (p.variant) { FWD_MFMA_VARIANTS(X) }
 #undef X
 #undef FWD_LAUNCH_TILE
 #undef FWD_LAUNCH_PATCH
+#undef FWD_LAUNCH_WTHIN
     PAI_LAUNCH_CHECK();
     if (p.ksplit > 1)
         PAI_LAUNCH(splitk_finish_k, dim3(p.rows, g.nphase, cdiv(g.Cout, FIN_COLS)), dim3(256), 0, s, g, a, ws, p.rows, p.ksplit);
diff --git a/thesis-pai-reconstruction_amd/engine.py b/thesis-pai-reconstruction_amd/engine.py
--- a/thesis-pai-reconstruction_amd/engine.py
+++ b/thesis-pai-reconstruction_amd/engine.py
@@ -487,7 +487,7 @@
         G["du"] = torch.empty(biggest, dtype=dt, device=dev)
         G["dz_head"] = torch.empty(S["pred"].numel(), dtype=dt, device=dev)
         G["dz_dec"] = [torch.empty_like(S["w"][j]) if j < L - 1 else None for j in range(L)]
-        G["dz_enc"] = [torch.empty_like(S["z"][i]) for i in range(L)]
+        G["dz_enc"] = [torch.empty_like(S["z"][i]) if i > 0 else None for i in range(L)]
         S["grads"] = G
         return G
 
@@ -688,9 +688,18 @@
         wgrad(d, S["a"][i - 1], None, dz, conv, True)
         _, wd = self.enc_packs[i].get(dtype)
 
+        enc0_fused = ops.conv_dgrad_act_wthin_ok(P["enc_desc"][1], P["enc_desc"][0], False)
+
         def enc_dgrad(i, dz, wd):
             d = P["enc_desc"][i]
+            if i - 1 == 0 and enc0_fused:
+                c0, d0 = self.enc_conv[0], P["enc_desc"][0]
+                ops.conv_dgrad_act_wthin(d, dz, wd, S["z"][0], ACT_LRELU, G["gskip"][0], ACT_NONE, d0, S["x"], None,
+                                         A.seg(c0.weight), A.seg(c0.bias), wthin_slabs(P, d, d0))
+                return 0
             if i - 1 == 0:
+                if G["dz_enc"][0] is None:
+                    G["dz_enc"][0] = torch.empty_like(S["z"][0])
                 return ops.conv_dgrad_bn(d, dz, wd, G["dz_enc"][0], None, S["z"][0], ACT_LRELU, G["gskip"][0], ACT_NONE)
             pst, pbn = S["ebn"][i - 1], self.enc_bn[i - 1]
             ops.conv_dgrad_bn_apply(d, dz, wd, G["ga"][i - 1], None, S["z"][i - 1], ACT_LRELU, G["gskip"][i - 1], ACT_RELU,
@@ -710,11 +719,19 @@
             fused_rows = enc_dgrad(i, dz, wd)
         conv0 = self.enc_conv[0]
         flush_held()
-        with torch.cuda.stream(side.fork_tail()):
-            (ops.conv_wgrad if min(_cin_cout(conv0)) <= 2 else conv_wgrad)(
-                P["enc_desc"][0], S["x"], None, G["dz_enc"][0], A.seg(conv0.weight), A.seg(conv0.bias))
+        if not enc0_fused:
+            with torch.cuda.stream(side.fork_tail()):
+                (ops.conv_wgrad if min(_cin_cout(conv0)) <= 2 else conv_wgrad)(
+                    P["enc_desc"][0], S["x"], None, G["dz_enc"][0], A.seg(conv0.weight), A.seg(conv0.bias))
         side.join()
         done(conv0.bias)
+
+
+def wthin_slabs(P, d, d_thin):
+    if "wthin_slabs" not in P:
+        P["wthin_slabs"] = torch.empty(ops.conv_dgrad_act_wthin_slab_bytes(d, d_thin) // 4, dtype=torch.float32,
+                                       device=P["device"])
+    return P["wthin_slabs"]
 
 
 class DiscEngine:
@@ -847,11 +864,18 @@
     def _grads(self, S):
         if S["grads"] is None:
             P = S["P"]
-            S["grads"] = {"du": [torch.empty_like(a) for a in S["a"]],
+            S["grads"] = {"du": [None] + [torch.empty_like(a) for a in S["a"][1:]],
                           "dl": torch.empty(S["logits"].numel(), dtype=P["dtype"], device=P["device"]),
                           "dl32": torch.empty(S["logits"].numel(), dtype=torch.float32, device=P["device"]),
                           "dy": torch.empty(P["N"] * P["H"] * P["W"] * self.in_ch, dtype=P["dtype"], device=P["device"])}
         return S["grads"]
+
+    @staticmethod
+    def _du0(S):
+        G = S["grads"]
+        if G["du"][0] is None:
+            G["du"][0] = torch.empty_like(S["a"][0])
+        return G["du"][0]
 
     def forward_loss(self, x, y, dtype, y2, n_first, target_first, target_rest, acc, need_grad: bool):
         if not (x.is_cuda and y.is_cuda):
@@ -911,29 +935,37 @@
         _, wd = self.packs[4].get(dtype)
         if not head_done:
             ops.conv_dgrad_act(d, dl, wd, G["du"][3], None, S["a"][3], ACT_LRELU)
+        wthin = need_params and not need_dy and ops.conv_dgrad_act_wthin_ok(P["desc"][1], P["desc"][0], need_dy)
         for k in range(3, -1, -1):
             conv = self.convs[k]
             d = P["desc"][k]
+            if wthin and k == 0:
+                break
             if need_params and k == 0:
                 with torch.cuda.stream(side.fork_tail()):
                     (ops.conv_wgrad if min(_cin_cout(conv)) <= 2 else conv_wgrad)(
-                        d, S["xin"], S["yin"], G["du"][0], A.seg(conv.weight), A.seg(conv.bias))
+                        d, S["xin"], S["yin"], self._du0(S), A.seg(conv.weight), A.seg(conv.bias))
             elif need_params:
                 with torch.cuda.stream(side.fork(d)):
                     conv_wgrad(self._wgrad_desc(P, k), S["a"][k - 1], None, G["du"][k], A.seg(conv.weight), A.seg(conv.bias))
                     if hook is not None:
                         hook(A, A.end_of(conv.bias))
-            if k > 0:
+            if k == 1 and wthin:
+                _, wd = self.packs[1].get(dtype)
+                c0, d0 = self.convs[0], P["desc"][0]
+                ops.conv_dgrad_act_wthin(d, G["du"][1], wd, S["a"][0], ACT_LRELU, None, ACT_NONE, d0, S["xin"], S["yin"],
+                                         A.seg(c0.weight), A.seg(c0.bias), wthin_slabs(P, d, d0))
+            elif k > 0:
                 _, wd = self.packs[k].get(dtype)
-                ops.conv_dgrad_act(d, G["du"][k], wd, G["du"][k - 1], None, S["a"][k - 1], ACT_LRELU)
+                ops.conv_dgrad_act(d, G["du"][k], wd, self._du0(S) if k == 1 else G["du"][k - 1], None, S["a"][k - 1], ACT_LRELU)
             elif need_dy:
                 _, wd = self.packs[0].get(dtype)
                 if addend is not None and self.in_ch == 1 and self.fused_enabled() and addend.dtype == torch.float32 \
                         and addend.is_contiguous() and addend.numel() == N * H * W and ops.conv_dgrad_f32add_ok(d):
                     gy = torch.empty(N * H * W, dtype=torch.float32, device=dev)
-                    ops.conv_dgrad_f32add(d, G["du"][0], wd, addend, gy)
+                    ops.conv_dgrad_f32add(d, self._du0(S), wd, addend, gy)
                 else:
-                    ops.conv_dgrad(d, G["du"][0], wd, None, G["dy"], only_c2=True)
+                    ops.conv_dgrad(d, self._du0(S), wd, None, G["dy"], only_c2=True)
         side.join()
         if need_params and hook is not None:
             hook(A, A.end_of(self.convs[0].bias))
diff --git a/thesis-pai-reconstruction_amd/lib.py b/thesis-pai-reconstruction_amd/lib.py
--- a/thesis-pai-reconstruction_amd/lib.py
+++ b/thesis-pai-reconstruction_amd/lib.py
@@ -71,6 +71,10 @@
     "pai_conv_fwd": (_I, [_D, _P, _P, _P, _P, _P, _P, _P, _P, _P]),
     "pai_conv_dgrad": (_I, [_D, _P, _P, _P, _P, _I, _P]),
     "pai_conv_dgrad_act": (_I, [_D, _P, _P, _P, _P, _P, _I, _P]),
+    "pai_conv_dgrad_act_wthin_ok": (_I, [_D, _D, _I]),
+    "pai_conv_dgrad_act_wthin_slab_bytes": (_L, [_D, _D]),
+    "pai_conv_dgrad_act_wthin_kernel_name": (_I, [_D, _D, C.c_char_p, _I]),
+    "pai_conv_dgrad_act_wthin": (_I, [_D, _P, _P, _P, _I, _P, _I, _D, _P, _P, _P, _P, _I, _P, _L, _P]),
     "pai_conv_dgrad_f32add_ok": (_I, [_D]),
     "pai_conv_dgrad_f32add": (_I, [_D, _P, _P, _P, _P, _P]),
     "pai_head_loss_ok": (_I, [_D, _I]),
diff --git a/thesis-pai-reconstruction_amd/ops.py b/thesis-pai-reconstruction_amd/ops.py
--- a/thesis-pai-reconstruction_amd/ops.py
+++ b/thesis-pai-reconstruction_amd/ops.py
@@ -309,6 +309,54 @@
     with _Timed(d, 1):
         L.check(L.load().pai_conv_dgrad_act(C.byref(d), _p(dy), _p(w_dgrad), _p(dx1), _p(dx2), _p(a1), int(act1),
                                             _stream()), "pai_conv_dgrad_act")
+
+
+def conv_dgrad_act_wthin_ok(d, d_thin, need_dx: bool = False) -> bool:
+    return bool(L.load().pai_conv_dgrad_act_wthin_ok(C.byref(d), C.byref(d_thin), int(bool(need_dx))))
+
+
+def conv_dgrad_act_wthin_slab_bytes(d, d_thin) -> int:
+    n = L.load().pai_conv_dgrad_act_wthin_slab_bytes(C.byref(d), C.byref(d_thin))
+    if n < 0:
+        raise PaiError("pai_conv_dgrad_act_wthin_slab_bytes: not a pair of layers conv_dgrad_act_wthin takes")
+    return n
+
+
+def conv_dgrad_act_wthin_kernel_name(d, d_thin) -> str:
+    buf = C.create_string_buffer(96)
+    if L.load().pai_conv_dgrad_act_wthin_kernel_name(C.byref(d), C.byref(d_thin), buf, 96) != 0:
+        raise PaiError("pai_conv_dgrad_act_wthin_kernel_name: not a pair of layers conv_dgrad_act_wthin takes")
+    return buf.value.decode()
+
+
+class _TimedWthin(_Timed):
+
+    def __init__(self, d, d_thin):
+        super().__init__(d, 1)
+        self.d_thin = d_thin
+
+    def __exit__(self, *exc):
+        if self.on:
+            LaunchTimer.disarm()
+            PROFILE.append((conv_dgrad_act_wthin_kernel_name(self.d, self.d_thin), 1, conv_flops(self.d), self.t, self.t))
+        return False
+
+
+def conv_dgrad_act_wthin(d, dy, w_dgrad, a1, act1, add, act2, d_thin, x1, x2, dw, dbias, slabs, overwrite=0):
+    if not isinstance(d_thin, ConvDesc) or not isinstance(d, ConvDesc):
+        raise PaiError("conv_dgrad_act_wthin: d and d_thin are convolution descriptors (make_desc)")
+    if slabs is None or slabs.dtype != torch.float32 or not slabs.is_contiguous():
+        raise PaiError("conv_dgrad_act_wthin: slabs is a contiguous fp32 tensor")
+    if (x2 is None) != (d_thin.C2 == 0):
+        raise PaiError("conv_dgrad_act_wthin: x2 goes with the thin layer's second channel")
+    if dw.numel() != d_thin.Cout * 16 * (d_thin.C1 + d_thin.C2) or (dbias is not None and dbias.numel() != d_thin.Cout):
+        raise PaiError("conv_dgrad_act_wthin: dw / dbias do not have the thin layer's shape")
+    with _TimedWthin(d, d_thin):
+        L.check(L.load().pai_conv_dgrad_act_wthin(C.byref(d), _p(dy), _p(w_dgrad), _p(a1), int(act1), _p(add), int(act2),
+                                                  C.byref(d_thin), _p(x1, torch.bfloat16), _p(x2, torch.bfloat16),
+                                                  _p(dw, torch.float32), _p(dbias, torch.float32), int(overwrite),
+                                                  _p(slabs, torch.float32), slabs.numel() * 4, _stream()),
+                "pai_conv_dgrad_act_wthin")
 
 
 def conv_dgrad_f32add_ok(d) -> bool:
```

Result: faster. 11590 images/s (median of 6 runs) (+1.3%).
